# mapillary/OpenSfM

Hardware: NVIDIA H100
Metric: BA observations/sec (higher is better)
Workload: dtype f64

## Files before the change

### include/opensfm_b200.h

```cpp
#ifndef OPENSFM_B200_H_
#define OPENSFM_B200_H_

#include <stddef.h>
#include <stdint.h>

#ifdef __cplusplus
extern "C" {
#endif

#define OSFM_OK 0
#define OSFM_ERR_CUDA 1
#define OSFM_ERR_ARG 2
#define OSFM_ERR_RUNTIME 3

const char* osfm_last_error(void);
int osfm_version(void);
int64_t osfm_kernel_launch_count(void);

typedef struct osfm_matcher osfm_matcher;

int osfm_matcher_create(int device, osfm_matcher** out);
int osfm_matcher_destroy(osfm_matcher* m);

int osfm_bf_match_f32(osfm_matcher* m, const float* f1, int n1, const float* f2, int n2, int dim,
// ... 42 lines not shown

enum {
  OSFM_PERSPECTIVE = 0, OSFM_BROWN = 1, OSFM_FISHEYE = 2, OSFM_FISHEYE_OPENCV = 3, OSFM_FISHEYE62 = 4,
  OSFM_FISHEYE624 = 5, OSFM_SPHERICAL = 6, OSFM_DUAL = 7, OSFM_RADIAL = 8, OSFM_SIMPLE_RADIAL = 9
};
enum { OSFM_LOSS_TRIVIAL = 0, OSFM_LOSS_HUBER = 1, OSFM_LOSS_SOFTLONE = 2, OSFM_LOSS_CAUCHY = 3, OSFM_LOSS_ARCTAN = 4,
       OSFM_LOSS_TUKEY = 5  };

int osfm_ba_create(int device, osfm_ba** out);
int osfm_ba_destroy(osfm_ba* ba);
int osfm_camera_num_params(int projection_type);

int osfm_ba_set_cameras(osfm_ba* ba, int n, const int32_t* type, const double* params ,
                        const int32_t* constant, const double* prior , const double* prior_sigma ,
                        const int32_t* prior_log );
int osfm_ba_set_rig_instances(osfm_ba* ba, int n, const double* pose6, const int32_t* constant,
                              const int32_t* has_position_prior, const double* prior_position3,
                              const double* prior_std3);
int osfm_ba_set_rig_cameras(osfm_ba* ba, int n, const double* pose6, const int32_t* constant);
int osfm_ba_set_shots(osfm_ba* ba, int n, const int32_t* rig_instance, const int32_t* camera,
                      const int32_t* rig_camera, const int32_t* use_rig_camera);
int osfm_ba_set_points(osfm_ba* ba, int n, const double* xyz, const int32_t* constant);
int osfm_ba_set_observations(osfm_ba* ba, int64_t n, const int32_t* shot, const int32_t* point,
                             const double* xy, const double* std_deviation);
int osfm_ba_set_observations_async(osfm_ba* ba, int64_t n, const int32_t* shot, const int32_t* point,
                                   const double* xy, const double* std_deviation);

int osfm_ba_set_rig_camera_priors(osfm_ba* ba, const double* prior6, const double* sigma6);
int osfm_ba_set_point_priors(osfm_ba* ba, int n, const int32_t* point, const double* prior3, const double* sigma3,
                             const int32_t* has_altitude);
int osfm_ba_set_ext_blocks(osfm_ba* ba, int n, const int32_t* size, const double* values, const int32_t* constant,
                           const double* lower_bound);
int osfm_ba_get_ext_blocks(osfm_ba* ba, double* values);

enum {
  OSFM_SIDE_UP_VECTOR = 0, OSFM_SIDE_PAN = 1, OSFM_SIDE_TILT = 2, OSFM_SIDE_ROLL = 3, OSFM_SIDE_RELATIVE_MOTION = 4,
  OSFM_SIDE_RELATIVE_ROTATION = 5, OSFM_SIDE_COMMON_POSITION = 6, OSFM_SIDE_LINEAR_MOTION = 7,
  OSFM_SIDE_TRANSLATION_PRIOR = 8, OSFM_SIDE_PARAMETER_BARRIER = 9, OSFM_SIDE_STD_DEVIATION = 10,
  OSFM_SIDE_POSITION_PRIOR = 11,
  OSFM_SIDE_RA_RELATIVE_MOTION = 12, OSFM_SIDE_RA_ABSOLUTE_POSITION = 13, OSFM_SIDE_RA_RELATIVE_ABSOLUTE_POSITION = 14,
  OSFM_SIDE_RA_COMMON_POINT = 15, OSFM_SIDE_RA_COMMON_CAMERA = 16, OSFM_SIDE_NUM_TYPES = 17
};
typedef struct {
  int32_t type, nres, nblocks;
  int32_t kind[6], idx[6];
  int32_t loss;
  double loss_a;
  int32_t cofs;
  int32_t aux[4];
} osfm_side_term;
int osfm_ba_set_side_terms(osfm_ba* ba, int n, const osfm_side_term* terms, int64_t nconsts, const double* consts);
int osfm_ba_set_options(osfm_ba* ba, int loss, double loss_threshold, int max_iterations,
                        const char* linear_solver, int compute_reprojection_errors);
typedef int (*osfm_allreduce_fn)(void* device_buf, int64_t count, void* stream, void* user);
int osfm_ba_set_distributed(osfm_ba* ba, int rank, int world, osfm_allreduce_fn fn, void* user);
int osfm_nccl_unique_id(char* out128);
int osfm_ba_set_nccl(osfm_ba* ba, int rank, int world, const char* id128);
int osfm_ba_set_stream(osfm_ba* ba, void* cuda_stream);

int osfm_ba_run(osfm_ba* ba);

typedef struct {
  int iterations;
  int successful_steps;
  int linear_solves;
  int pcg_iterations;
  int termination;
  double initial_cost, final_cost;
  double time_run_s;
  double time_device_ms;
  double time_linearize_ms;
  int64_t linearize_launches;
  double time_schur_ms;
  int64_t schur_launches;
  double time_pcg_ms;
  double time_backsub_ms;
  int64_t num_observations_local;
  int reduced_dim;
  int reduced_blocks;
  int64_t reduced_nnz;
  int jac_planes;
  int64_t kernel_launches;
  char message[128];
} osfm_ba_summary;
int osfm_ba_get_summary(osfm_ba* ba, osfm_ba_summary* out);

int osfm_ba_get_cameras(osfm_ba* ba, double* params_flat);
int osfm_ba_get_rig_instances(osfm_ba* ba, double* pose6);
int osfm_ba_get_rig_cameras(osfm_ba* ba, double* pose6);
int osfm_ba_get_points(osfm_ba* ba, double* xyz);
int osfm_ba_get_reprojection_errors(osfm_ba* ba, double* out_n_by_3);

int osfm_ba_eval_observation(int device, int projection_type, const double* camera, const double* rig_instance,
                             const double* rig_camera, int use_rig_camera, const double* point,
                             const double* observed, double std_deviation, double* r, double* jac_camera,
                             double* jac_instance, double* jac_rig_camera, double* jac_point, int* num_residuals);

int osfm_ba_capture_linear_system(osfm_ba* ba, int iteration);
enum { OSFM_SCHUR_NONE = 0, OSFM_SCHUR_PIPE = 1, OSFM_SCHUR_MMA = 2, OSFM_SCHUR_SIMT_SEGMENT = 3 };
enum { OSFM_PCG_PIPELINED_DEFLATED = 1, OSFM_PCG_PIPELINED = 2, OSFM_PCG_CLASSIC_RESIDENT = 3,
       OSFM_PCG_CLASSIC_STREAMED = 4 };
typedef struct {
  int iteration;
  int nc, n, wc, nres;
  double radius;
  int nseg, p_fast, p_slow;
  int schur_kernel;
  int sp_nchunks;
  int pcg_kernel;
  int pcg_rescued;
  int pcg_iterations;
  double pcg_rr;
} osfm_ba_capture;
int osfm_ba_get_captured_system(osfm_ba* ba, osfm_ba_capture* info, double* S, double* rhs, double* y, double* scale,
                                double* diag, double* grad);
int osfm_ba_get_captured_parameters(osfm_ba* ba, double* cam_params, double* inst_pose6, double* rig_camera_pose6,
                                    double* points, double* ext_values);

int osfm_ba_set_compute_covariances(osfm_ba* ba, int enable);
enum {
  OSFM_COV_OK = 0,
  OSFM_COV_SOLVER_FAILURE = 1,
  OSFM_COV_POINT_RANK_DEFICIENT = 2,
  OSFM_COV_CAMERA_RANK_DEFICIENT = 3,
  OSFM_COV_NON_FINITE = 4
};
int osfm_ba_get_covariances(osfm_ba* ba, int* valid, int* status, double* out);
int osfm_ba_get_covariance_timing(osfm_ba* ba, double* pass_ms, double* cholesky_ms);

#ifdef __cplusplus
}
#endif
#endif
```

### opensfm_b200/_lib.py

```python
from __future__ import annotations

import ctypes
import os
from ctypes import POINTER, c_char_p, c_double, c_float, c_int, c_int32, c_int64, c_uint8, c_void_p

HERE = os.path.dirname(os.path.abspath(__file__))
LIB_PATH = os.path.join(HERE, "lib", "libopensfm_b200.so")

OSFM_OK = 0
PROJECTION_TYPES = dict(PERSPECTIVE=0, BROWN=1, FISHEYE=2, FISHEYE_OPENCV=3, FISHEYE62=4, FISHEYE624=5,
                        SPHERICAL=6, DUAL=7, RADIAL=8, SIMPLE_RADIAL=9)
LOSS_IDS = {"TrivialLoss": 0, "HuberLoss": 1, "SoftLOneLoss": 2, "CauchyLoss": 3, "ArctanLoss": 4}
LOSS_TUKEY = 5
SIDE_TYPES = dict(UP_VECTOR=0, PAN=1, TILT=2, ROLL=3, RELATIVE_MOTION=4, RELATIVE_ROTATION=5, COMMON_POSITION=6,
                  LINEAR_MOTION=7, TRANSLATION_PRIOR=8, PARAMETER_BARRIER=9, STD_DEVIATION=10, POSITION_PRIOR=11)
SB_CAM, SB_INST, SB_RIGCAM, SB_EXT = 0, 1, 2, 3


class SideTerm(ctypes.Structure):
    _fields_ = [("type", c_int32), ("nres", c_int32), ("nblocks", c_int32), ("kind", c_int32 * 6), ("idx", c_int32 * 6),
                ("loss", c_int32), ("loss_a", c_double), ("cofs", c_int32), ("aux", c_int32 * 4)]


class BASummary(ctypes.Structure):
    _fields_ = [
        ("iterations", c_int), ("successful_steps", c_int), ("linear_solves", c_int), ("pcg_iterations", c_int),
        ("termination", c_int), ("initial_cost", c_double), ("final_cost", c_double), ("time_run_s", c_double),
        ("time_device_ms", c_double), ("time_linearize_ms", c_double), ("linearize_launches", c_int64),
        ("time_schur_ms", c_double), ("schur_launches", c_int64), ("time_pcg_ms", c_double),
        ("time_backsub_ms", c_double), ("num_observations_local", c_int64), ("reduced_dim", c_int),
        ("reduced_blocks", c_int), ("reduced_nnz", c_int64), ("jac_planes", c_int), ("kernel_launches", c_int64), ("message", ctypes.c_char * 128),
    ]


class BACapture(ctypes.Structure):
    _fields_ = [("iteration", c_int), ("nc", c_int), ("n", c_int), ("wc", c_int), ("nres", c_int), ("radius", c_double),
                ("nseg", c_int), ("p_fast", c_int), ("p_slow", c_int), ("schur_kernel", c_int), ("sp_nchunks", c_int),
                ("pcg_kernel", c_int), ("pcg_rescued", c_int), ("pcg_iterations", c_int), ("pcg_rr", c_double)]


SCHUR_KERNELS = {0: "none", 1: "pipe", 2: "mma", 3: "simt_segment"}
PCG_KERNELS = {1: "pipelined_deflated", 2: "pipelined", 3: "classic_resident", 4: "classic_streamed"}
COVARIANCE_STATUS = {0: "ok", 1: "solver_failure", 2: "point_rank_deficient", 3: "camera_rank_deficient",
                     4: "non_finite"}

ALLREDUCE_FN = ctypes.CFUNCTYPE(c_int, c_void_p, c_int64, c_void_p, c_void_p)

SIGNATURES = {
    "osfm_last_error": (c_char_p, []),
    "osfm_version": (c_int, []),
    "osfm_kernel_launch_count": (c_int64, []),
    "osfm_matcher_create": (c_int, [c_int, POINTER(c_void_p)]),
    "osfm_matcher_destroy": (c_int, [c_void_p]),
    "osfm_bf_match_f32": (c_int, [c_void_p, c_void_p, c_int, c_void_p, c_int, c_int, c_double, c_void_p, c_int, c_void_p]),
    "osfm_bf_match_u8": (c_int, [c_void_p, c_void_p, c_int, c_void_p, c_int, c_int, c_double, c_void_p, c_int, c_void_p]),
    "osfm_matcher_add_f32": (c_int, [c_void_p, c_void_p, c_int, c_int, POINTER(c_int)]),
    "osfm_matcher_add_u8": (c_int, [c_void_p, c_void_p, c_int, c_int, POINTER(c_int)]),
    "osfm_matcher_add_batch_f32": (c_int, [c_void_p, c_int, c_void_p, c_void_p, c_int, c_void_p]),
    "osfm_matcher_add_batch_u8": (c_int, [c_void_p, c_int, c_void_p, c_void_p, c_int, c_void_p]),
    "osfm_matcher_add_u8_l2": (c_int, [c_void_p, c_void_p, c_int, c_int, POINTER(c_int)]),
    "osfm_matcher_add_batch_u8_l2": (c_int, [c_void_p, c_int, c_void_p, c_void_p, c_int, c_void_p]),
    "osfm_matcher_remove": (c_int, [c_void_p, c_int]),
    "osfm_matcher_clear": (c_int, [c_void_p]),
    "osfm_matcher_match_pairs_async": (c_int, [c_void_p, c_int, c_void_p, c_void_p, c_double, c_int]),
    "osfm_matcher_set_bearings": (c_int, [c_void_p, c_int, c_void_p]),
    "osfm_matcher_match_pairs_guided_async": (c_int, [c_void_p, c_int, c_void_p, c_void_p, c_void_p, c_double, c_double,
                                                       c_int]),
    "osfm_matcher_get_epipolar_masks": (c_int, [c_void_p, c_int, c_void_p, c_void_p]),
    "osfm_matcher_sync": (c_int, [c_void_p]),
    "osfm_matcher_fetch": (c_int, [c_void_p, c_void_p, c_int64]),
    "osfm_matcher_fetch_pairs": (c_int, [c_void_p, c_void_p, c_void_p, c_int64, POINTER(c_int64)]),
    "osfm_matcher_last_device_ms": (c_int, [c_void_p, POINTER(c_float), POINTER(c_float)]),
    "osfm_matcher_set_kernel": (c_int, [c_void_p, c_int]),
    "osfm_matcher_last_kernel": (c_int, [c_void_p]),
    "osfm_matcher_device_bytes": (c_int, [c_void_p, POINTER(c_int64), POINTER(c_int64)]),
    "osfm_match_words": (c_int, [c_void_p, c_void_p, c_int, c_void_p, c_int, c_void_p, c_int, c_void_p, c_int, c_float,
                                  c_int, c_void_p]),
    "osfm_vlad_distances": (c_int, [c_void_p, c_void_p, c_int, c_int, c_int, c_void_p]),
    "osfm_matcher_vlad_compute": (c_int, [c_void_p, c_int, c_void_p, c_void_p, c_int, c_int, c_void_p]),
    "osfm_matcher_vlad_get": (c_int, [c_void_p, c_int, c_int, c_void_p]),
    "osfm_matcher_vlad_select": (c_int, [c_void_p, c_int, c_void_p, c_int, c_void_p, c_void_p, c_void_p, c_int, c_void_p,
                                         c_void_p, c_void_p]),
    "osfm_ba_create": (c_int, [c_int, POINTER(c_void_p)]),
    "osfm_ba_destroy": (c_int, [c_void_p]),
    "osfm_camera_num_params": (c_int, [c_int]),
    "osfm_ba_set_cameras": (c_int, [c_void_p, c_int, c_void_p, c_void_p, c_void_p, c_void_p, c_void_p, c_void_p]),
    "osfm_ba_set_rig_instances": (c_int, [c_void_p, c_int, c_void_p, c_void_p, c_void_p, c_void_p, c_void_p]),
    "osfm_ba_set_rig_cameras": (c_int, [c_void_p, c_int, c_void_p, c_void_p]),
    "osfm_ba_set_shots": (c_int, [c_void_p, c_int, c_void_p, c_void_p, c_void_p, c_void_p]),
    "osfm_ba_set_points": (c_int, [c_void_p, c_int, c_void_p, c_void_p]),
    "osfm_ba_set_observations": (c_int, [c_void_p, c_int64, c_void_p, c_void_p, c_void_p, c_void_p]),
    "osfm_ba_set_observations_async": (c_int, [c_void_p, c_int64, c_void_p, c_void_p, c_void_p, c_void_p]),
    "osfm_ba_set_rig_camera_priors": (c_int, [c_void_p, c_void_p, c_void_p]),
    "osfm_ba_set_point_priors": (c_int, [c_void_p, c_int, c_void_p, c_void_p, c_void_p, c_void_p]),
    "osfm_ba_set_ext_blocks": (c_int, [c_void_p, c_int, c_void_p, c_void_p, c_void_p, c_void_p]),
    "osfm_ba_get_ext_blocks": (c_int, [c_void_p, c_void_p]),
    "osfm_ba_set_side_terms": (c_int, [c_void_p, c_int, c_void_p, c_int64, c_void_p]),
    "osfm_ba_set_options": (c_int, [c_void_p, c_int, c_double, c_int, c_char_p, c_int]),
    "osfm_ba_set_distributed": (c_int, [c_void_p, c_int, c_int, ALLREDUCE_FN, c_void_p]),
    "osfm_nccl_unique_id": (c_int, [c_void_p]),
    "osfm_ba_set_nccl": (c_int, [c_void_p, c_int, c_int, c_void_p]),
    "osfm_ba_set_stream": (c_int, [c_void_p, c_void_p]),
    "osfm_ba_run": (c_int, [c_void_p]),
    "osfm_ba_get_summary": (c_int, [c_void_p, POINTER(BASummary)]),
    "osfm_ba_get_cameras": (c_int, [c_void_p, c_void_p]),
    "osfm_ba_get_rig_instances": (c_int, [c_void_p, c_void_p]),
    "osfm_ba_get_rig_cameras": (c_int, [c_void_p, c_void_p]),
    "osfm_ba_get_points": (c_int, [c_void_p, c_void_p]),
    "osfm_ba_get_reprojection_errors": (c_int, [c_void_p, c_void_p]),
    "osfm_ba_eval_observation": (c_int, [c_int, c_int, c_void_p, c_void_p, c_void_p, c_int, c_void_p, c_void_p,
                                         c_double, c_void_p, c_void_p, c_void_p, c_void_p, c_void_p, POINTER(c_int)]),
    "osfm_ba_capture_linear_system": (c_int, [c_void_p, c_int]),
    "osfm_ba_get_captured_system": (c_int, [c_void_p, POINTER(BACapture), c_void_p, c_void_p, c_void_p, c_void_p,
                                            c_void_p, c_void_p]),
# ... 32 lines not shown
```

### opensfm_b200/csrc/ba.cu

```cuda
#include <algorithm>
#include <dlfcn.h>

#include <chrono>
#include <cstring>
#include <mutex>
#include <cmath>
#include <cstdlib>
#include <string>
#include <vector>

#include "ba_models.cuh"
#include "common.cuh"

struct OsfmNcclId { char internal[128]; };

namespace osfm {

struct BAView {
  int K, NI, NR, S, P;
  long long N;
  int nc, npf;
  int wc, nres;
  int loss;
  double loss_a;
  const int *cam_type, *cam_off, *cam_np, *cam_poff, *inst_poff, *rc_poff, *pt_poff;
  const int *shot_inst, *shot_cam, *shot_rc, *shot_use_rc;
  const int *obs_shot, *obs_point;
  const double *obs_x, *obs_y, *obs_isig;
  const long long* obs_orig;
  const long long* pt_start;
  double *r, *Jc, *Jp;
};

struct Params {
  double *cam, *inst, *rc, *pts, *ext;
};

struct Scalars {
  double cost;
  double model_change;
  double step_norm2;
  double x_norm2;
  double grad_max_bits;
  double gdot;
};

__device__ __forceinline__ double block_reduce_sum(double v) {
  __shared__ double sh[32];
  const int lane = threadIdx.x & 31, w = threadIdx.x >> 5;
#pragma unroll
  for (int o = 16; o; o >>= 1) v += __shfl_xor_sync(0xffffffffu, v, o);
  __syncthreads();
  if (lane == 0) sh[w] = v;
  __syncthreads();
  const int nw = (blockDim.x + 31) >> 5;
  v = threadIdx.x < nw ? sh[threadIdx.x] : 0.0;
  if (w == 0) {
#pragma unroll
    for (int o = 16; o; o >>= 1) v += __shfl_xor_sync(0xffffffffu, v, o);
  }
  return v;
}

__device__ __forceinline__ void atomic_max_nonneg(double* addr, double v) {
  atomicMax(reinterpret_cast<unsigned long long*>(addr), (unsigned long long)__double_as_longlong(v));
}

template <int MODE, int NB = 3, int TYPE = -1>
__global__ void __launch_bounds__(128, NB) ba_linearize(BAView v, Params p, Scalars* sc, double* reproj) {
  const long long i = (long long)blockIdx.x * blockDim.x + threadIdx.x;
  double cost = 0.0;
  if (i < v.N) {
    const int shot = v.obs_shot[i];
    const int cam = v.shot_cam[shot];
    const int type = TYPE >= 0 ? TYPE : v.cam_type[cam];
    const int C = TYPE >= 0 ? model_num_params(TYPE >= 0 ? TYPE : 0) : v.cam_np[cam];
    const bool use_rc = TYPE >= 0 ? false : v.shot_use_rc[shot] != 0;
    const int pt = v.obs_point[i];
    double camp[MAX_CAM_PARAMS], ri[6], rc[6], X[3];
#pragma unroll
    for (int j = 0; j < MAX_CAM_PARAMS; ++j)
      if (j < C) camp[j] = p.cam[v.cam_off[cam] + j];
#pragma unroll
    for (int j = 0; j < 6; ++j) ri[j] = p.inst[6 * (size_t)v.shot_inst[shot] + j];
    if (use_rc) {
#pragma unroll
      for (int j = 0; j < 6; ++j) rc[j] = p.rc[6 * (size_t)v.shot_rc[shot] + j];
    }
#pragma unroll
    for (int j = 0; j < 3; ++j) X[j] = p.pts[3 * (size_t)pt + j];
    const double ox = v.obs_x[i], oy = v.obs_y[i];
    if (MODE == 2) {
      double r[3] = {0.0, 0.0, 0.0};
      observation_eval(type, camp, ri, rc, use_rc, X, ox, oy, 1.0, r, nullptr, nullptr, nullptr, nullptr);
      const long long o = v.obs_orig[i];
      reproj[3 * o] = r[0]; reproj[3 * o + 1] = r[1]; reproj[3 * o + 2] = r[2];
    } else if (MODE == 0) {
      double r[3];
      const int nres = observation_eval(type, camp, ri, rc, use_rc, X, ox, oy, v.obs_isig[i], r, nullptr, nullptr,
                                        nullptr, nullptr);
      double s = r[0] * r[0] + r[1] * r[1];
      if (nres == 3) s += r[2] * r[2];
      double w;
      cost = 0.5 * robust_loss(v.loss, v.loss_a, s, &w);
      if (v.cam_poff[cam] < 0 && v.inst_poff[v.shot_inst[shot]] < 0 && (!use_rc || v.rc_poff[v.shot_rc[shot]] < 0) &&
          v.pt_poff[pt] < 0)
        cost = 0.0;
    } else {
      double r[3], jc[3 * MAX_CAM_PARAMS], jri[18], jrc[18], jp[9];
      const int nres = observation_eval(type, camp, ri, rc, use_rc, X, ox, oy, v.obs_isig[i], r, jc, jri, jrc, jp);
      double s = r[0] * r[0] + r[1] * r[1];
      if (nres == 3) s += r[2] * r[2];
      double w;
      cost = 0.5 * robust_loss(v.loss, v.loss_a, s, &w);
      const bool pfree = v.pt_poff[pt] >= 0;
      if (!pfree && v.cam_poff[cam] < 0 && v.inst_poff[v.shot_inst[shot]] < 0 && (!use_rc || v.rc_poff[v.shot_rc[shot]] < 0))
        cost = 0.0;
      const size_t N = (size_t)v.N;
      if (TYPE >= 0) {
        constexpr int CC = TYPE == PT_PERSPECTIVE ? 3 : TYPE == PT_FISHEYE ? 3 : TYPE == PT_BROWN ? 9 : 1;
        const int wcl = v.wc;
#pragma unroll
        for (int k = 0; k < 2; ++k) {
          v.r[k * N + i] = w * r[k];
          double* jcrow = v.Jc + (size_t)k * wcl * N + i;
#pragma unroll
          for (int j = 0; j < CC; ++j) jcrow[(size_t)j * N] = w * jc[k * CC + j];
#pragma unroll
// ... 187 lines not shown
    if (pf >= 0) {
#pragma unroll
      for (int j = 0; j < 3; ++j) {
        atomicAdd(&colnorm2[v.nc + 3 * pf + j], val[j]);
        atomicAdd(&grad[v.nc + 3 * pf + j], val[3 + j]);
      }
    }
  }
}

template <int WCT>
__global__ void __launch_bounds__(256, WCT ? 3 : 2) ba_colnorm_grad_seg(BAView v, const int* __restrict__ seg_start, int nseg,
                                                           double* colnorm2, double* grad) {
  const int s = blockIdx.x * (blockDim.x >> 5) + (threadIdx.x >> 5);
  if (s >= nseg) return;
  const int lane = threadIdx.x & 31;
  const int p0 = seg_start[s], np = seg_start[s + 1] - p0;
  const long long base = v.pt_start[p0];
  const int k = (int)(v.pt_start[p0 + 1] - base);
  const int G = 32 / k;
  const int g = lane / k, c = lane - g * k;
  const bool active = g < G;
  const size_t N = (size_t)v.N;
  const int wc = WCT ? WCT : v.wc;
  constexpr int WCU = WCT ? WCT : 16;
  double n2[WCU], gr[WCU];
#pragma unroll
  for (int j = 0; j < WCU; ++j) { n2[j] = 0.0; gr[j] = 0.0; }
  if (active) {
    for (int pi = g; pi < np; pi += G) {
      const size_t i = (size_t)(base + (long long)pi * k + c);
      for (int q = 0; q < v.nres; ++q) {
        const double rq = v.r[q * N + i];
#pragma unroll
        for (int j = 0; j < WCU; ++j) {
          if (j < wc) {
            const double a = v.Jc[((size_t)q * wc + j) * N + i];
            n2[j] += a * a;
            gr[j] += a * rq;
          }
        }
      }
    }
  }
  for (int gg = 1; gg < G; ++gg) {
#pragma unroll
    for (int j = 0; j < WCU; ++j) {
      if (j < wc) {
        const double a = __shfl_down_sync(0xffffffffu, n2[j], gg * k);
        const double b = __shfl_down_sync(0xffffffffu, gr[j], gg * k);
        if (lane < k) { n2[j] += a; gr[j] += b; }
      }
    }
  }
  if (lane < k) {
    const ObsCols oc = obs_cols(v, base + c);
#pragma unroll
    for (int j = 0; j < WCU; ++j) {
      if (j < wc) {
        const int col = oc.col(j);
        if (col >= 0) {
          atomicAdd(&colnorm2[col], n2[j]);
          atomicAdd(&grad[col], gr[j]);
        }
      }
    }
  }
}

__global__ void ba_prior_colnorm_grad(PriorView pv, Params p, double* colnorm2, double* grad) {
  const int row = blockIdx.x * blockDim.x + threadIdx.x;
  if (row >= pv.n_cam_rows + pv.n_pos_rows) return;
  double r, d;
  int col;
  prior_row(pv, p, row, &r, &col, &d);
  atomicAdd(&colnorm2[col], d * d);
  atomicAdd(&grad[col], d * r);
}

__global__ void ba_make_scale(const double* colnorm2, double* scale, int n) {
  const int i = blockIdx.x * blockDim.x + threadIdx.x;
  if (i < n) scale[i] = 1.0 / (1.0 + sqrt(colnorm2[i]));
}
__global__ void ba_make_diag(const double* colnorm2, const double* scale, double* diag, int n) {
  const int i = blockIdx.x * blockDim.x + threadIdx.x;
  if (i < n) diag[i] = fmin(fmax(colnorm2[i] * scale[i] * scale[i], 1e-6), 1e32);
}
__global__ void ba_pack_lin(const double* __restrict__ colnorm2, const double* __restrict__ grad, const Scalars* sc, int nc,
                            int rank, int world, double* __restrict__ pack) {
  const int i = blockIdx.x * blockDim.x + threadIdx.x;
  if (i < nc) { pack[i] = colnorm2[i]; pack[nc + i] = grad[i]; }
  if (i == 0) pack[2 * nc] = sc->cost;
  if (i < world) pack[2 * nc + 1 + i] = i == rank ? sc->grad_max_bits : 0.0;
}
__global__ void ba_unpack_lin(const double* __restrict__ pack, int nc, int world, double* __restrict__ colnorm2,
                              double* __restrict__ grad, Scalars* sc) {
  const int i = blockIdx.x * blockDim.x + threadIdx.x;
  double v = 0.0;
  if (i < nc) { colnorm2[i] = pack[i]; grad[i] = pack[nc + i]; v = fabs(pack[nc + i]); }
  if (i < world) v = fmax(v, pack[2 * nc + 1 + i]);
  if (i == 0) sc->cost = pack[2 * nc];
#pragma unroll
  for (int o = 16; o; o >>= 1) v = fmax(v, __shfl_xor_sync(0xffffffffu, v, o));
  if ((threadIdx.x & 31) == 0 && v > 0.0) atomic_max_nonneg(&sc->grad_max_bits, v);
}
__global__ void ba_grad_max(const double* grad, int n, Scalars* sc) {
  const int i = blockIdx.x * blockDim.x + threadIdx.x;
  double v = i < n ? fabs(grad[i]) : 0.0;
#pragma unroll
  for (int o = 16; o; o >>= 1) v = fmax(v, __shfl_xor_sync(0xffffffffu, v, o));
  if ((threadIdx.x & 31) == 0 && v > 0.0) atomic_max_nonneg(&sc->grad_max_bits, v);
}

}
#include "ba_reduced.cuh"
#include "ba_schur_pipe.cuh"

#include <tuple>
#include <utility>

namespace osfm {
template <typename... KArgs, size_t... I>
inline void launch_cooperative_impl(void (*kern)(KArgs...), int grid, int block, size_t smem, cudaStream_t st,
                                    std::tuple<KArgs...>& a, std::index_sequence<I...>) {
  void* ptrs[] = {static_cast<void*>(&std::get<I>(a))...};
  OSFM_CUDA(cudaLaunchCooperativeKernel(reinterpret_cast<const void*>(kern), dim3(grid), dim3(block), ptrs, smem, st));
}
template <typename... KArgs, typename... Args>
inline void launch_cooperative(void (*kern)(KArgs...), int grid, int block, size_t smem, cudaStream_t st, Args&&... args) {
  std::tuple<KArgs...> a(std::forward<Args>(args)...);
  launch_cooperative_impl(kern, grid, block, smem, st, a, std::index_sequence_for<KArgs...>{});
}
}
#include "ba_side.cuh"
#include "ba_order.cuh"
#include "ba_cov.cuh"
namespace osfm {

__global__ void __launch_bounds__(256) ba_backsub_rows(BAView v, const double* __restrict__ scale,
                                                       const double* __restrict__ y, double* __restrict__ t) {
  const long long i = (long long)blockIdx.x * blockDim.x + threadIdx.x;
  const size_t N = (size_t)v.N;
  const bool in = i < v.N;
  const int pt = in ? v.obs_point[i] : -1;
  const int pf = in ? v.pt_poff[pt] : -1;
  double val[3] = {0.0, 0.0, 0.0};
  if (pf >= 0) {
    const int wc = v.wc;
    const ObsCols oc = obs_cols(v, i);
    for (int q = 0; q < v.nres; ++q) {
      double e = v.r[q * N + i];
      for (int j = 0; j < wc; ++j) {
        const int g = oc.col(j);
        if (g >= 0) e -= v.Jc[((size_t)q * wc + j) * N + i] * scale[g] * y[g];
      }
#pragma unroll
      for (int j = 0; j < 3; ++j) val[j] += v.Jp[((size_t)q * 3 + j) * N + i] * e;
    }
  }
  seg_scan_by_point<3>(pt, val);
  const int next = __shfl_down_sync(0xffffffffu, pt, 1);
  const bool tail = (threadIdx.x & 31) == 31 || next != pt;
  if (pf >= 0 && tail) {
    const size_t NP = (size_t)v.npf;
#pragma unroll
    for (int j = 0; j < 3; ++j) atomicAdd(&t[j * NP + pf], val[j]);
  }
}
__global__ void __launch_bounds__(256) ba_backsub_points(BAView v, const double* __restrict__ scale,
                                                         const double* __restrict__ Vinv, const double* __restrict__ t,
                                                         double* __restrict__ y) {
  const int pf = blockIdx.x * blockDim.x + threadIdx.x;
  if (pf >= v.npf) return;
  const size_t NP = (size_t)v.npf;
  const int nc = v.nc;
  const double t0 = t[pf] * scale[nc + 3 * pf], t1 = t[NP + pf] * scale[nc + 3 * pf + 1],
               t2 = t[2 * NP + pf] * scale[nc + 3 * pf + 2];
  const double a = Vinv[0 * NP + pf], b = Vinv[1 * NP + pf], c = Vinv[2 * NP + pf];
  const double d = Vinv[3 * NP + pf], e = Vinv[4 * NP + pf], f = Vinv[5 * NP + pf];
  y[nc + 3 * pf + 0] = a * t0 + b * t1 + c * t2;
  y[nc + 3 * pf + 1] = b * t0 + d * t1 + e * t2;
  y[nc + 3 * pf + 2] = c * t0 + e * t1 + f * t2;
}

__global__ void ba_update(int which, int count, const int* __restrict__ poff, const int* __restrict__ off,
                          const int* __restrict__ np, int stride, int base, const double* __restrict__ src,
                          double* __restrict__ dst, const double* __restrict__ scale, const double* __restrict__ y,
                          Scalars* sc, int accumulate_norms, const double* __restrict__ lower = nullptr,
                          double alpha = 1.0) {
  const int b = blockIdx.x * blockDim.x + threadIdx.x;
  double sn = 0.0, xn = 0.0;
  if (b < count) {
    const int o = which == 0 ? off[b] : b * stride;
    const int n = which == 0 ? np[b] : stride;
    const int g = poff[b];
    for (int j = 0; j < n; ++j) {
      double val = src[o + j];
      if (g >= 0) {
        const int gi = which == 3 ? base + 3 * g + j : g + j;
        double d = -alpha * scale[gi] * y[gi];
        if (lower && val + d < lower[o + j]) d = lower[o + j] - val;
        xn += val * val;
        sn += d * d;
        val += d;
      }
      dst[o + j] = val;
    }
  }
  if (accumulate_norms) {
    const double t1 = block_reduce_sum(sn);
    const double t2 = block_reduce_sum(xn);
    if (threadIdx.x == 0) {
      if (t1 != 0.0) atomicAdd(&sc->step_norm2, t1);
      if (t2 != 0.0) atomicAdd(&sc->x_norm2, t2);
    }
  }
}

__global__ void ba_grad_dot(int n, int nc, int cam_side, const double* __restrict__ grad, const double* __restrict__ scale,
                            const double* __restrict__ y, Scalars* sc) {
  const int i = blockIdx.x * blockDim.x + threadIdx.x;
  double v = 0.0;
  if (i < n && (i >= nc || cam_side)) v = -grad[i] * scale[i] * y[i];
  const double t = block_reduce_sum(v);
  if (threadIdx.x == 0 && t != 0.0) atomicAdd(&sc->gdot, t);
}

__global__ void ba_model_change_alg(int n, int nc, int cam_side, const double* __restrict__ grad, const double* __restrict__ scale,
                                    const double* __restrict__ diag, double inv_radius, const double* __restrict__ y, Scalars* sc) {
  const int i = blockIdx.x * blockDim.x + threadIdx.x;
  double v = 0.0;
  if (i < n && (i >= nc || cam_side)) v = 0.5 * y[i] * (grad[i] * scale[i] + diag[i] * inv_radius * y[i]);
  const double t = block_reduce_sum(v);
  if (threadIdx.x == 0 && t != 0.0) atomicAdd(&sc->model_change, t);
}

__global__ void ba_eval_one(int type, const double* in, int use_rc, double* out, int* nres_out) {
  double r[3] = {0, 0, 0}, jc[3 * MAX_CAM_PARAMS], jri[18], jrc[18], jp[9];
  for (int i = 0; i < 18; ++i) jrc[i] = 0.0;
  const int nres = observation_eval(type, in, in + 16, in + 22, use_rc != 0, in + 28, in[31], in[32], in[33], r, jc,
                                    jri, jrc, jp);
  *nres_out = nres;
  for (int i = 0; i < 3; ++i) out[i] = r[i];
  for (int i = 0; i < 48; ++i) out[3 + i] = jc[i];
  for (int i = 0; i < 18; ++i) out[51 + i] = jri[i];
  for (int i = 0; i < 18; ++i) out[69 + i] = jrc[i];
  for (int i = 0; i < 9; ++i) out[87 + i] = jp[i];
}

struct EventTimer {
  cudaEvent_t a = nullptr, b = nullptr;
  double total_ms = 0.0;
  long long count = 0;
  bool pending = false;
  void init() { OSFM_CUDA(cudaEventCreate(&a)); OSFM_CUDA(cudaEventCreate(&b)); }
  void destroy() { if (a) cudaEventDestroy(a); if (b) cudaEventDestroy(b); a = b = nullptr; }
  void start(cudaStream_t st) { collect(); OSFM_CUDA(cudaEventRecord(a, st)); }
  void stop(cudaStream_t st) { OSFM_CUDA(cudaEventRecord(b, st)); pending = true; }
  void collect() {
    if (!pending) return;
    OSFM_CUDA(cudaEventSynchronize(b));
    float ms = 0.f;
    OSFM_CUDA(cudaEventElapsedTime(&ms, a, b));
    total_ms += ms; ++count; pending = false;
  }
};

template <class T>
static void upload(DevBuf<T>& d, const std::vector<T>& h, cudaStream_t st) {
  d.reserve(std::max<size_t>(h.size(), 1));
  if (!h.empty()) OSFM_CUDA(cudaMemcpyAsync(d.p, h.data(), h.size() * sizeof(T), cudaMemcpyHostToDevice, st));
}
template <class T>
static void download(std::vector<T>& h, const T* d, size_t count, cudaStream_t st) {
  h.resize(count);
  if (count) OSFM_CUDA(cudaMemcpyAsync(h.data(), d, count * sizeof(T), cudaMemcpyDeviceToHost, st));
}

struct NcclApi {
  void* lib = nullptr;
  int (*GetUniqueId)(void*) = nullptr;
  int (*CommInitRank)(void**, int, OsfmNcclId, int) = nullptr;
  int (*AllReduce)(const void*, void*, size_t, int, int, void*, cudaStream_t) = nullptr;
  int (*CommDestroy)(void*) = nullptr;
  const char* (*GetErrorString)(int) = nullptr;
};
static NcclApi& nccl_api() {
  static NcclApi api;
  static std::once_flag once;
  std::call_once(once, []() {
    void* h = dlopen("libnccl.so.2", RTLD_NOW | RTLD_NOLOAD);
    if (!h) h = dlopen("libnccl.so.2", RTLD_NOW);
    if (!h) h = dlopen("libnccl.so", RTLD_NOW);
    if (!h) return;
    api.lib = h;
    api.GetUniqueId = reinterpret_cast<int (*)(void*)>(dlsym(h, "ncclGetUniqueId"));
    api.CommInitRank = reinterpret_cast<int (*)(void**, int, OsfmNcclId, int)>(dlsym(h, "ncclCommInitRank"));
    api.AllReduce = reinterpret_cast<int (*)(const void*, void*, size_t, int, int, void*, cudaStream_t)>(dlsym(h, "ncclAllReduce"));
    api.CommDestroy = reinterpret_cast<int (*)(void*)>(dlsym(h, "ncclCommDestroy"));
    api.GetErrorString = reinterpret_cast<const char* (*)(int)>(dlsym(h, "ncclGetErrorString"));
  });
  if (!api.lib || !api.GetUniqueId || !api.CommInitRank || !api.AllReduce || !api.CommDestroy)
    throw std::runtime_error("NCCL (libnccl.so.2) is not available in this process");
  return api;
}
static void nccl_check(int rc, const char* what) {
  if (rc != 0) {
    NcclApi& a = nccl_api();
    throw std::runtime_error(std::string(what) + ": " + (a.GetErrorString ? a.GetErrorString(rc) : "NCCL error"));
  }
}

static int grid_for(long long n, int threads) { return (int)std::max<long long>(1, (n + threads - 1) / threads); }
static long long up16(long long x) { return (x + 15) / 16 * 16; }
static std::vector<int> balanced_cut(const std::vector<long long>& w, int G) {
  const int n = (int)w.size() - 1;
  std::vector<int> lo(G + 1, n);
  lo[0] = 0;
  for (int c = 1, i = 0; c < G; ++c) {
    const long long want = w[n] * c / G;
    while (i < n && w[i] < want) ++i;
    lo[c] = i;
  }
  return lo;
}
static bool env_starts_with(const char* name, char c) {
  const char* e = getenv(name);
  return e && e[0] == c;
}
struct BaSwitches {
  bool trace = env_starts_with("OSFM_BA_TRACE", '1');
  bool seg_schur = !env_starts_with("OSFM_BA_SEGMENT_SCHUR", '0');
  bool lin_special = !env_starts_with("OSFM_BA_LIN_SPECIAL", '0');
  bool schur_mma = !env_starts_with("OSFM_BA_SCHUR_MMA", '0');
  bool schur_pipe = !env_starts_with("OSFM_BA_SCHUR_PIPE", '0');
  bool pcg_resident = !env_starts_with("OSFM_BA_PCG_RESIDENT", '0');
  bool pcg_pipelined = !env_starts_with("OSFM_BA_PCG_PIPELINED", '0');
  bool pcg_deflate = !env_starts_with("OSFM_BA_PCG_DEFLATE", '0');
};
static const BaSwitches& switches() {
  static const BaSwitches s;
  return s;
}

enum LinPath {
  LIN_NONE,
  LIN_FUSED,
  LIN_CHUNKS,
  LIN_SEGMENTS,
};

struct RunState {
  std::chrono::high_resolution_clock::time_point t_start, t_prev;
  int64_t launches0 = 0;
  int K = 0, NI = 0, NR = 0, NE = 0, NT = 0, S = 0, P = 0, Pfull = 0;
  long long Nfull = 0, N = 0, n_fast_obs = 0, pair_bound = 0;
  int nc = 0, nc_pad = 0, n = 0, nblk = 0, npf = 0, ngroups = 0, wc = 0, nres = 2, nseg = 0, P_fast = 0;
  size_t nz = 1;
  int n_upper = 0, n_blocks_all = 0, pcg_grid = 1;
  long long s_upper_total = 0, s_total = 0, vb = 0;
  int uniform_type = -1;
  bool constrained = false;
  bool have_pp = false, add_priors = false;
  int cur = 0;
  int pcg_total = 0;
  std::vector<int> cam_off, cam_np, cam_poff, inst_poff, rc_poff, ext_off, ext_poff, blk_off, blk_sz;
  std::vector<int> cam_blk, inst_blk, rc_blk, ext_blk, side_jofs, side_rofs, grp_b1, grp_b2;
  std::vector<int> pr_cam_param, pr_cam_col, pr_cam_log, pr_pos_kind, pr_pos_inst, pr_pos_axis, pr_pos_col;
  std::vector<int> pr_blk, pr_local;
  std::vector<double> pr_cam_prior, pr_cam_scale, pr_pos_prior, pr_pos_scale;
  std::vector<int> row_M, cbase;
  std::vector<long long> rowbase;
  std::vector<int> cov_inst, cov_bstart;
  int cov_m = 0, cov_nb1 = 0;
  int schur = OSFM_SCHUR_NONE;
  LinPath lin = LIN_NONE;
  bool seg_tab = false;
  int sp_nchunks = 0;
  bool pcg_resident = false, pcg_pipe_ok = false;
  int pcg_smem = 0, pcg_pipe_smem = 0;
  PcgResident pcg_res{};
  PcgPipe pcg_pipe{};
  BAView v{}; PriorView pv{}; SideView sv{}; PointPriorView ppv{}; BlkMaps bm{}; BsrView bsr{}; PcgLayout lay{};
  double *d_rhs_p = nullptr, *d_S_p = nullptr;
  cudaEvent_t ev0 = nullptr, ev1 = nullptr;
  EventTimer tm_lin, tm_schur, tm_pcg, tm_back;
};

struct BA {
  int device = 0;
  cudaStream_t own_stream = nullptr, stream = nullptr;
  cudaStream_t copy_stream = nullptr;
  cudaEvent_t ev_obs = nullptr;
  bool obs_pending = false;
  std::vector<int> cam_type, cam_const, cam_prior_log;
  std::vector<double> cam_params, cam_prior, cam_prior_sigma;
  std::vector<double> inst, inst_prior_pos, inst_prior_std;
  std::vector<int> inst_const, inst_has_prior;
  std::vector<double> rc, rc_prior, rc_prior_sigma;
  std::vector<int> rc_const;
  std::vector<int> ext_size, ext_const;
  std::vector<double> ext_values, ext_lower;
  std::vector<osfm_side_term> side_terms;
  std::vector<double> side_consts;
  std::vector<int> pp_point, pp_alt;
  std::vector<double> pp_prior, pp_sigma;
  std::vector<int> shot_inst, shot_cam, shot_rc, shot_use_rc;
  std::vector<double> pts;
  std::vector<int> pt_const;
  long long n_obs_full = 0;
  int loss = OSFM_LOSS_CAUCHY;
  double loss_a = 1.0;
  int max_iterations = 500;
  bool compute_reproj = true;
  int rank = 0, world = 1;
  osfm_allreduce_fn allreduce = nullptr;
  void* allreduce_user = nullptr;
  void* nccl_comm = nullptr;
  int nccl_rank = -1, nccl_world = 0;
  bool reproj_valid = false;
  osfm_ba_summary summary{};
  bool has_run = false;
  int cap_iter = 0;
  bool cap_valid = false;
  osfm_ba_capture cap_info{};
  std::vector<double> cap_sbuf, cap_y, cap_scale, cap_diag, cap_grad;
  std::vector<double> cap_cam, cap_inst, cap_rc, cap_pts, cap_ext;
  std::vector<int4> cap_upper;
  std::vector<int> cap_blk_off, cap_blk_sz, cap_pt_poff, cap_global_of;
  int cap_nc_pad = 0;
  bool cov_on = false, cov_ran = false, cov_valid = false;
  int cov_status = OSFM_COV_OK;
  double cov_pass_ms = 0.0, cov_chol_ms = 0.0;
  std::vector<double> cov_out;
  DevBuf<double> d_cov;
  DevBuf<int> d_cov_perm, d_cov_inst, d_cov_flags;

  DevBuf<int> d_cam_type, d_cam_off, d_cam_np, d_cam_poff, d_inst_poff, d_rc_poff, d_pt_poff;
  DevBuf<int> d_shot_inst, d_shot_cam, d_shot_rc, d_shot_use_rc, d_obs_shot, d_obs_point;
  DevBuf<double> d_obs_x, d_obs_y, d_obs_isig;
  DevBuf<long long> d_obs_orig, d_pt_start;
  DevBuf<double> d_cam[2], d_inst[2], d_rc[2], d_pts[2];
  DevBuf<double> d_r, d_Jc, d_Jp, d_Sbuf, d_Vinv, d_gp, d_slots;
  DevBuf<double> d_scale, d_colnorm2, d_grad, d_diag, d_y, d_bs_t;
  DevBuf<double> d_px, d_pr, d_pz, d_pp, d_pAp, d_Minv, d_reproj, d_full_pts;
  DevBuf<double> d_Wdef;
  DevBuf<int> d_blk_off, d_blk_sz, d_cam_blk, d_inst_blk, d_rc_blk;
  DevBuf<unsigned long long> d_tkeys, d_skeys, d_skeys2, d_rkeys, d_rkeys2;
  DevBuf<int> d_tvals, d_area, d_offs, d_row_ptr, d_row_col, d_row_off, d_diag_off, d_prior_diag_off;
  DevBuf<int> d_pr_blk, d_pr_local, d_g_obs_shot, d_g_obs_point;
  DevBuf<long long> d_g_pt_start;
  DevBuf<int4> d_upper;
  DevBuf<unsigned> d_count;
  DevBuf<char> d_cub;
  DevBuf<PcgState> d_pcg;
  DevBuf<int> d_seg_start;
  DevBuf<int> d_raw_shot, d_raw_point, d_ptc_full;
  DevBuf<double> d_raw_xy, d_raw_sigma, d_pts_in;
  DevBuf<unsigned long long> d_okeys, d_okeys2, d_pkey, d_pkey2;
  DevBuf<int> d_ovals, d_ovals2, d_pval, d_order, d_inv_order, d_global_of, d_free_flag, d_free_scan, d_head, d_run_head, d_nsel;
  DevBuf<long long> d_kk;
  DevBuf<char> d_seg_flags;
  DevBuf<OrderCounts> d_oc;
  PinnedBuf<OrderCounts> h_oc;
  DevBuf<double> d_rowsJ, d_rowsW, d_rowsY, d_Vig;
  DevBuf<int> d_row_M, d_qoff, d_blk_row, d_cbase, d_colidx, d_row_of, d_grp_b1, d_grp_b2;
  DevBuf<long long> d_rowbase;
  DevBuf<double> d_Spcg, d_Ap;
  PinnedBuf<PcgState> h_pcg;
  DevBuf<int> d_pcg_rowlo;
  DevBuf<int> d_pcg_grplo;
  DevBuf<char> d_grp_shared;
  DevBuf<unsigned long long> d_prof;
  DevBuf<long long> d_tab_off, d_tab_sizes;
  DevBuf<int> d_sp_nch, d_sp_chunk0;
  DevBuf<SchurChunk> d_sp_chunks;
  DevBuf<int> d_sp_ftab;
  DevBuf<int> d_tab;
  DevBuf<double> d_ptsum;
  std::vector<const void*> smem_opted;
  int num_sms = 132;
  DevBuf<int> d_pr_cam_param, d_pr_cam_col, d_pr_cam_log, d_pr_pos_inst, d_pr_pos_axis, d_pr_pos_col;
  DevBuf<double> d_pr_cam_prior, d_pr_cam_scale, d_pr_pos_prior, d_pr_pos_scale;
  DevBuf<Scalars> d_sc;
  PinnedBuf<Scalars> h_sc;
  DevBuf<int> d_pr_pos_kind, d_ext_off, d_ext_np, d_ext_poff, d_ext_blk, d_side_jofs, d_side_rofs;
  DevBuf<double> d_ext[2], d_ext_lower, d_side_consts, d_side_J, d_side_r, d_pp_d, d_pp_x0;
  DevBuf<SideTerm> d_side_terms;

  explicit BA(int dev) : device(dev) {
    OSFM_CUDA(cudaSetDevice(device));
    OSFM_CUDA(cudaStreamCreateWithFlags(&own_stream, cudaStreamNonBlocking));
    stream = own_stream;
    OSFM_CUDA(cudaStreamCreateWithFlags(&copy_stream, cudaStreamNonBlocking));
    OSFM_CUDA(cudaEventCreateWithFlags(&ev_obs, cudaEventDisableTiming));
    h_sc.reserve(1);
    h_pcg.reserve(1);
    OSFM_CUDA(cudaDeviceGetAttribute(&num_sms, cudaDevAttrMultiProcessorCount, device));
  }
  ~BA() {
    cudaSetDevice(device);
    if (nccl_comm) { try { nccl_api().CommDestroy(nccl_comm); } catch (...) {} }
    if (copy_stream) { cudaStreamSynchronize(copy_stream); cudaStreamDestroy(copy_stream); }
    if (ev_obs) cudaEventDestroy(ev_obs);
    if (own_stream) cudaStreamDestroy(own_stream);
  }

  Scalars read_scalars() {
    OSFM_CUDA(cudaMemcpyAsync(h_sc.p, d_sc.p, sizeof(Scalars), cudaMemcpyDeviceToHost, stream));
    OSFM_CUDA(cudaStreamSynchronize(stream));
    return *h_sc.p;
  }
  int ar_calls = 0;
  double ar_host_ms = 0.0, ar_dev_ms = 0.0;
  void allreduce_dev(double* buf, long long count) {
    if (world > 1) {
      const auto t0 = std::chrono::high_resolution_clock::now();
      cudaEvent_t e0 = nullptr, e1 = nullptr;
      if (switches().trace) { cudaEventCreate(&e0); cudaEventCreate(&e1); cudaEventRecord(e0, stream); }
      struct Done {
        BA* self; std::chrono::high_resolution_clock::time_point t0; cudaEvent_t e0, e1;
        ~Done() {
          if (switches().trace) {
            cudaEventRecord(e1, self->stream); cudaEventSynchronize(e1);
            float ms = 0.f; cudaEventElapsedTime(&ms, e0, e1); self->ar_dev_ms += ms;
            cudaEventDestroy(e0); cudaEventDestroy(e1);
          }
          ++self->ar_calls;
          self->ar_host_ms += std::chrono::duration<double, std::milli>(std::chrono::high_resolution_clock::now() - t0).count();
        }
      } done{this, t0, e0, e1};
      if (allreduce) {
        if (allreduce(buf, count, stream, allreduce_user) != 0) throw std::runtime_error("all-reduce callback failed");
      } else if (nccl_comm && nccl_world == world && nccl_rank == rank) {
        nccl_check(nccl_api().AllReduce(buf, buf, (size_t)count,  8,  0, nccl_comm, stream), "ncclAllReduce");
      } else {
        throw ArgError("world > 1 but neither an all-reduce callback nor an NCCL communicator is set");
      }
    }
  }
  template <class Kernel>
  void opt_in_smem(Kernel* kernel, int bytes) {
    const void* k = (const void*)kernel;
    if (std::find(smem_opted.begin(), smem_opted.end(), k) != smem_opted.end()) return;
    OSFM_CUDA(cudaFuncSetAttribute(k, cudaFuncAttributeMaxDynamicSharedMemorySize, bytes));
    smem_opted.push_back(k);
  }
  void trace(const char* what) {
    if (!switches().trace) return;
    const auto now = std::chrono::high_resolution_clock::now();
    fprintf(stderr, "[osfm_ba] %-12s %8.3f ms\n", what, std::chrono::duration<double, std::milli>(now - rs.t_prev).count());
    rs.t_prev = now;
  }
  template <int MODE>
  void launch_linearize(int b) {
    const int grid = grid_for(rs.N, 128);
    switch (rs.uniform_type) {
      case PT_PERSPECTIVE: ba_linearize<MODE, MODE == 1 ? 5 : 3, PT_PERSPECTIVE><<<grid, 128, 0, stream>>>(rs.v, params_of(b), d_sc.p, nullptr); break;
      case PT_BROWN: ba_linearize<MODE, MODE == 1 ? 4 : 3, PT_BROWN><<<grid, 128, 0, stream>>>(rs.v, params_of(b), d_sc.p, nullptr); break;
      case PT_FISHEYE: ba_linearize<MODE, MODE == 1 ? 5 : 3, PT_FISHEYE><<<grid, 128, 0, stream>>>(rs.v, params_of(b), d_sc.p, nullptr); break;
      default: ba_linearize<MODE, 3><<<grid, 128, 0, stream>>>(rs.v, params_of(b), d_sc.p, nullptr); break;
    }
    OSFM_LAUNCH_CHECK();
  }
  void update_params(int src, int dst, double alpha, const double* lower) {
    const Params a = params_of(src), b = params_of(dst);
    const int K = rs.K, NI = rs.NI, NR = rs.NR, P = rs.P, NE = rs.NE;
    if (K) { ba_update<<<grid_for(K, 128), 128, 0, stream>>>(0, K, d_cam_poff.p, d_cam_off.p, d_cam_np.p, 0, 0, a.cam, b.cam, d_scale.p, d_y.p, d_sc.p, rank == 0, nullptr, alpha); OSFM_LAUNCH_CHECK(); }
    if (NI) { ba_update<<<grid_for(NI, 128), 128, 0, stream>>>(1, NI, d_inst_poff.p, nullptr, nullptr, 6, 0, a.inst, b.inst, d_scale.p, d_y.p, d_sc.p, rank == 0, nullptr, alpha); OSFM_LAUNCH_CHECK(); }
    if (NR) { ba_update<<<grid_for(NR, 128), 128, 0, stream>>>(2, NR, d_rc_poff.p, nullptr, nullptr, 6, 0, a.rc, b.rc, d_scale.p, d_y.p, d_sc.p, rank == 0, nullptr, alpha); OSFM_LAUNCH_CHECK(); }
    if (P) { ba_update<<<grid_for(P, 128), 128, 0, stream>>>(3, P, d_pt_poff.p, nullptr, nullptr, 3, rs.nc, a.pts, b.pts, d_scale.p, d_y.p, d_sc.p, 1, nullptr, alpha); OSFM_LAUNCH_CHECK(); }
    if (NE) { ba_update<<<grid_for(NE, 128), 128, 0, stream>>>(0, NE, d_ext_poff.p, d_ext_off.p, d_ext_np.p, 0, 0, a.ext, b.ext, d_scale.p, d_y.p, d_sc.p, rank == 0, lower, alpha); OSFM_LAUNCH_CHECK(); }
  }
  double x_norm_of(int b) {
    OSFM_CUDA(cudaMemsetAsync(&d_sc.p->x_norm2, 0, sizeof(double), stream));
    OSFM_CUDA(cudaMemsetAsync(d_y.p, 0, sizeof(double) * rs.nz, stream));
    update_params(b, b, 1.0, nullptr);
    allreduce_dev(&d_sc.p->x_norm2, 1);
    return std::sqrt(read_scalars().x_norm2);
  }
  Params params_of(int b) { return Params{d_cam[b].p, d_inst[b].p, d_rc[b].p, d_pts[b].p, d_ext[b].p}; }
  RunState rs;

  void run();
  void plan_layout(), order_observations(), plan_prior_rows(), upload_problem(), discover_structure(), plan_pcg(),
      reserve_covariance(), build_segment_tables(), segment_table_scales();
  double eval_cost(int b), linearize(int b, bool timed, double* grad_max);
  void build_system(double inv_radius, int* rank_flag, bool timed), back_substitute();
  int solve_reduced();
  void capture_linear_system(int it, double radius, int pcg_path), covariance_pass(int termination);
  void write_results(osfm_ba_summary sum);
};

void BA::plan_layout() {
  const int K = (int)cam_type.size(), NI = (int)inst_const.size(), NR = (int)rc_const.size(), S = (int)shot_inst.size();
  const int NE = (int)ext_size.size(), NT = (int)side_terms.size();
  rs.K = K; rs.NI = NI; rs.NR = NR; rs.NE = NE; rs.NT = NT; rs.S = S; rs.Pfull = (int)pt_const.size(); rs.Nfull = n_obs_full;
  for (int s = 0; s < S; ++s) {
    if (shot_inst[s] < 0 || shot_inst[s] >= NI) throw ArgError("shot references a rig instance that doesn't exist");
    if (shot_cam[s] < 0 || shot_cam[s] >= K) throw ArgError("shot references a camera that doesn't exist");
    if (shot_use_rc[s] && (shot_rc[s] < 0 || shot_rc[s] >= NR))
      throw ArgError("shot references a rig camera that doesn't exist");
  }
  trace("validate");

  rs.cam_off.assign(K + 1, 0); rs.cam_np.assign(K, 0); rs.cam_poff.assign(K, -1); rs.inst_poff.assign(NI, -1);
  rs.rc_poff.assign(std::max(NR, 1), -1); rs.ext_off.assign(NE + 1, 0); rs.ext_poff.assign(std::max(NE, 1), -1);
  rs.cam_blk.assign(std::max(K, 1), -1); rs.inst_blk.assign(std::max(NI, 1), -1); rs.rc_blk.assign(std::max(NR, 1), -1);
  rs.ext_blk.assign(std::max(NE, 1), -1);
  int nc = 0;
  auto add_block = [&](int size, int& poff, int& blk) {
    poff = nc; blk = (int)rs.blk_off.size();
    rs.blk_off.push_back(nc); rs.blk_sz.push_back(size); nc += size;
  };
  for (int k = 0; k < K; ++k) {
    rs.cam_np[k] = model_num_params(cam_type[k]);
    rs.cam_off[k + 1] = rs.cam_off[k] + rs.cam_np[k];
  }
  for (int k = 0; k < K; ++k) if (!cam_const[k]) add_block(rs.cam_np[k], rs.cam_poff[k], rs.cam_blk[k]);
  for (int i = 0; i < NI; ++i) if (!inst_const[i]) add_block(6, rs.inst_poff[i], rs.inst_blk[i]);
  for (int i = 0; i < NR; ++i) if (!rc_const[i]) add_block(6, rs.rc_poff[i], rs.rc_blk[i]);
  for (int i = 0; i < NE; ++i) {
    if (ext_size[i] < 1 || ext_size[i] > MAXB) throw ArgError("ext block size must be in [1, 16]");
    rs.ext_off[i + 1] = rs.ext_off[i] + ext_size[i];
    if (ext_const[i]) continue;
    add_block(ext_size[i], rs.ext_poff[i], rs.ext_blk[i]);
    for (int j = 0; j < ext_size[i]; ++j) rs.constrained |= std::isfinite(ext_lower[rs.ext_off[i] + j]);
  }
  rs.nc = nc;
  rs.nblk = (int)rs.blk_off.size();
  rs.nc_pad = (nc + 15) / 16 * 16;
  rs.side_jofs.assign(NT + 1, 0); rs.side_rofs.assign(NT + 1, 0);
  for (int t = 0; t < NT; ++t) {
    const osfm_side_term& st = side_terms[t];
    if (st.type < 0 || st.type >= OSFM_SIDE_NUM_TYPES) throw ArgError("unknown side term type");
    if (st.nblocks < 1 || st.nblocks > SIDE_MAX_BLOCKS || st.nres < 1 || st.nres > SIDE_MAX_RES)
      throw ArgError("side term with a bad block / residual count");
    int np = 0;
    for (int b = 0; b < st.nblocks; ++b) {
      const int kd = st.kind[b], ix = st.idx[b];
      const int cnt = kd == SB_CAM ? K : kd == SB_INST ? NI : kd == SB_RIGCAM ? NR : kd == SB_EXT ? NE : -1;
      if (ix < 0 || ix >= cnt) throw ArgError("side term references a parameter block that doesn't exist");
      np += kd == SB_CAM ? model_num_params(cam_type[ix]) : kd == SB_EXT ? ext_size[ix] : 6;
    }
    if (np > SIDE_MAX_PARAMS) throw ArgError("side term with too many parameters");
    if (st.cofs < 0 || (size_t)st.cofs > side_consts.size()) throw ArgError("side term constants out of range");
    rs.side_jofs[t + 1] = rs.side_jofs[t] + st.nres * np;
    rs.side_rofs[t + 1] = rs.side_rofs[t] + st.nres;
  }

  {
    std::vector<int> cam_user(std::max(K, 1), -1), inst_cam(std::max(NI, 1), -1);
    for (int s2 = 0; s2 < S; ++s2) {
      const int k = shot_cam[s2], i = shot_inst[s2];
      cam_user[k] = cam_user[k] == -1 || cam_user[k] == i ? i : -2;
      inst_cam[i] = inst_cam[i] == -1 || inst_cam[i] == k ? k : -2;
    }
    std::vector<char> inst_done(std::max(NI, 1), 0);
    for (int k = 0; k < K; ++k) {
      if (rs.cam_blk[k] < 0) continue;
      const int i = cam_user[k];
      if (i >= 0 && rs.inst_blk[i] >= 0 && inst_cam[i] == k && rs.cam_np[k] + 6 <= 16) {
        rs.grp_b1.push_back(rs.cam_blk[k]); rs.grp_b2.push_back(rs.inst_blk[i]); inst_done[i] = 1;
      } else {
        rs.grp_b1.push_back(rs.cam_blk[k]); rs.grp_b2.push_back(-1);
      }
    }
    for (int i = 0; i < NI; ++i)
      if (rs.inst_blk[i] >= 0 && !inst_done[i]) { rs.grp_b1.push_back(rs.inst_blk[i]); rs.grp_b2.push_back(-1); }
    for (int i = 0; i < NR; ++i)
      if (rs.rc_blk[i] >= 0) { rs.grp_b1.push_back(rs.rc_blk[i]); rs.grp_b2.push_back(-1); }
    for (int i = 0; i < NE; ++i)
      if (rs.ext_blk[i] >= 0) { rs.grp_b1.push_back(rs.ext_blk[i]); rs.grp_b2.push_back(-1); }
// ... 121 lines not shown
  rs.nseg = h_oc.p->nseg; rs.P_fast = h_oc.p->p_fast;
  rs.n_fast_obs = h_oc.p->n_fast; rs.pair_bound = (long long)h_oc.p->pair_bound;
  if (switches().trace)
    fprintf(stderr, "[osfm_ba] points %d (fast path %d in %d segments), observations %lld (fast path %lld), free points %d\n", P,
            rs.P_fast, rs.nseg, N, rs.n_fast_obs, rs.npf);
}

void BA::plan_prior_rows() {
  for (int k = 0; k < rs.K; ++k) {
    if (rs.cam_poff[k] < 0) continue;
    for (int j = 0; j < rs.cam_np[k]; ++j) {
      const int idx = rs.cam_off[k] + j;
      rs.pr_cam_param.push_back(idx);
      rs.pr_cam_col.push_back(rs.cam_poff[k] + j);
      rs.pr_cam_log.push_back(cam_prior_log[idx]);
      rs.pr_cam_prior.push_back(cam_prior[idx]);
      rs.pr_cam_scale.push_back(1.0 / std::max(cam_prior_sigma[idx], DBL_EPSILON));
      rs.pr_blk.push_back(rs.cam_blk[k]); rs.pr_local.push_back(j);
    }
  }
  auto pos_row = [&](int kind, int i, int axis, int poff, int blk, double prior, double sigma) {
    rs.pr_pos_kind.push_back(kind); rs.pr_pos_inst.push_back(i); rs.pr_pos_axis.push_back(axis); rs.pr_pos_col.push_back(poff + axis);
    rs.pr_pos_prior.push_back(prior);
    rs.pr_pos_scale.push_back(1.0 / std::max(sigma, DBL_EPSILON));
    rs.pr_blk.push_back(blk); rs.pr_local.push_back(axis);
  };
  for (int i = 0; i < rs.NI; ++i) {
    if (!inst_has_prior[i] || rs.inst_poff[i] < 0) continue;
    for (int j = 0; j < 3; ++j)
      pos_row(1, i, 3 + j, rs.inst_poff[i], rs.inst_blk[i], inst_prior_pos[3 * (size_t)i + j], inst_prior_std[3 * (size_t)i + j]);
  }
  for (int i = 0; i < rs.NR && !rc_prior.empty(); ++i) {
    if (rs.rc_poff[i] < 0) continue;
    for (int j = 0; j < 6; ++j)
      pos_row(2, i, j, rs.rc_poff[i], rs.rc_blk[i], rc_prior[6 * (size_t)i + j], rc_prior_sigma[6 * (size_t)i + j]);
  }
}

void BA::upload_problem() {
  const int NT = rs.NT, P = rs.P, Pfull = rs.Pfull, nc = rs.nc, npf = rs.npf, nres = rs.nres, wc = rs.wc;
  upload(d_cam_type, cam_type, stream); upload(d_cam_off, rs.cam_off, stream); upload(d_cam_np, rs.cam_np, stream);
  upload(d_cam_poff, rs.cam_poff, stream); upload(d_inst_poff, rs.inst_poff, stream); upload(d_rc_poff, rs.rc_poff, stream);
  upload(d_shot_inst, shot_inst, stream); upload(d_shot_cam, shot_cam, stream); upload(d_shot_rc, shot_rc, stream);
  upload(d_shot_use_rc, shot_use_rc, stream);
  std::vector<double> rc_h = rc;
  if (rc_h.empty()) rc_h.assign(6, 0.0);
  for (int b = 0; b < 2; ++b) {
    upload(d_cam[b], cam_params, stream); upload(d_inst[b], inst, stream); upload(d_rc[b], rc_h, stream);
  }
  upload(d_blk_off, rs.blk_off, stream); upload(d_blk_sz, rs.blk_sz, stream);
  upload(d_cam_blk, rs.cam_blk, stream); upload(d_inst_blk, rs.inst_blk, stream); upload(d_rc_blk, rs.rc_blk, stream);
  upload(d_pr_blk, rs.pr_blk, stream); upload(d_pr_local, rs.pr_local, stream);
  upload(d_grp_b1, rs.grp_b1, stream); upload(d_grp_b2, rs.grp_b2, stream);
  upload(d_pr_cam_param, rs.pr_cam_param, stream); upload(d_pr_cam_col, rs.pr_cam_col, stream);
  upload(d_pr_cam_log, rs.pr_cam_log, stream); upload(d_pr_cam_prior, rs.pr_cam_prior, stream);
  upload(d_pr_cam_scale, rs.pr_cam_scale, stream); upload(d_pr_pos_inst, rs.pr_pos_inst, stream);
  upload(d_pr_pos_axis, rs.pr_pos_axis, stream); upload(d_pr_pos_col, rs.pr_pos_col, stream);
  upload(d_pr_pos_kind, rs.pr_pos_kind, stream);
  std::vector<double> ev = ext_values, el = ext_lower;
  if (ev.empty()) { ev.assign(1, 0.0); el.assign(1, 0.0); }
  upload(d_ext[0], ev, stream); upload(d_ext[1], ev, stream); upload(d_ext_lower, el, stream);
  upload(d_ext_off, rs.ext_off, stream); upload(d_ext_np, ext_size, stream); upload(d_ext_poff, rs.ext_poff, stream);
  upload(d_ext_blk, rs.ext_blk, stream);
  upload(d_side_terms, side_terms, stream); upload(d_side_consts, side_consts, stream);
  upload(d_side_jofs, rs.side_jofs, stream); upload(d_side_rofs, rs.side_rofs, stream);
  d_side_J.reserve((size_t)rs.side_jofs[NT] + 1); d_side_r.reserve((size_t)rs.side_rofs[NT] + 1);
  std::vector<double> ppd, ppx;
  if (rs.have_pp) {
    ppd.assign(3 * (size_t)Pfull, 0.0); ppx.assign(3 * (size_t)Pfull, 0.0);
    for (size_t q = 0; q < pp_point.size(); ++q) {
      const size_t g = (size_t)pp_point[q];
      for (int j = 0; j < (pp_alt[q] ? 3 : 2); ++j) {
        ppd[3 * g + j] = 1.0 / std::max(pp_sigma[3 * q + j], DBL_EPSILON);
        ppx[3 * g + j] = pp_prior[3 * q + j];
      }
    }
    upload(d_pp_d, ppd, stream); upload(d_pp_x0, ppx, stream);
  }
  OSFM_CUDA(cudaStreamSynchronize(stream));
  upload(d_pr_pos_prior, rs.pr_pos_prior, stream); upload(d_pr_pos_scale, rs.pr_pos_scale, stream);
  const size_t Nz = (size_t)std::max<long long>(rs.N, 1);
  d_r.reserve(nres * Nz); d_Jc.reserve((size_t)nres * wc * Nz); d_Jp.reserve((size_t)nres * 3 * Nz);
  d_Vinv.reserve(6 * (size_t)std::max(npf, 1)); d_gp.reserve(3 * (size_t)std::max(npf, 1));
  const size_t nz = rs.nz;
  d_scale.reserve(nz); d_colnorm2.reserve(nz); d_grad.reserve(nz); d_diag.reserve(nz); d_y.reserve(nz);
  d_px.reserve(std::max(nc, 1)); d_pr.reserve(std::max(nc, 1)); d_pz.reserve(std::max(nc, 1));
  d_pp.reserve(std::max(nc, 1)); d_pAp.reserve(std::max(nc, 1));
  d_pcg.reserve(1);
  d_Minv.reserve((size_t)std::max(rs.ngroups, 1) * MAXB * MAXB);
  d_Ap.reserve(std::max(nc, 1));
  d_sc.reserve(1);

  BAView& v = rs.v;
  v.K = rs.K; v.NI = rs.NI; v.NR = rs.NR; v.S = rs.S; v.P = P; v.N = rs.N; v.nc = nc; v.npf = npf; v.wc = wc; v.nres = nres;
  v.loss = loss; v.loss_a = loss_a;
  v.cam_type = d_cam_type.p; v.cam_off = d_cam_off.p; v.cam_np = d_cam_np.p; v.cam_poff = d_cam_poff.p;
  v.inst_poff = d_inst_poff.p; v.rc_poff = d_rc_poff.p; v.pt_poff = d_pt_poff.p;
  v.shot_inst = d_shot_inst.p; v.shot_cam = d_shot_cam.p; v.shot_rc = d_shot_rc.p; v.shot_use_rc = d_shot_use_rc.p;
  v.obs_shot = d_obs_shot.p; v.obs_point = d_obs_point.p; v.obs_x = d_obs_x.p; v.obs_y = d_obs_y.p;
  v.obs_isig = d_obs_isig.p; v.obs_orig = d_obs_orig.p; v.pt_start = d_pt_start.p;
  v.r = d_r.p; v.Jc = d_Jc.p; v.Jp = d_Jp.p;
  PriorView& pv = rs.pv;
  pv.n_cam_rows = rs.add_priors ? (int)rs.pr_cam_param.size() : 0;
  pv.n_pos_rows = rs.add_priors ? (int)rs.pr_pos_inst.size() : 0;
  pv.cam_row_param = d_pr_cam_param.p; pv.cam_row_col = d_pr_cam_col.p; pv.cam_row_log = d_pr_cam_log.p;
  pv.cam_row_prior = d_pr_cam_prior.p; pv.cam_row_scale = d_pr_cam_scale.p;
  pv.pos_row_kind = d_pr_pos_kind.p;
  pv.pos_row_inst = d_pr_pos_inst.p; pv.pos_row_axis = d_pr_pos_axis.p; pv.pos_row_col = d_pr_pos_col.p;
  pv.pos_row_prior = d_pr_pos_prior.p; pv.pos_row_scale = d_pr_pos_scale.p;
  SideView& sv = rs.sv;
  sv.n = NT; sv.terms = d_side_terms.p; sv.consts = d_side_consts.p; sv.jofs = d_side_jofs.p; sv.rofs = d_side_rofs.p;
  sv.J = d_side_J.p; sv.r = d_side_r.p;
  sv.ext_off = d_ext_off.p; sv.ext_np = d_ext_np.p; sv.ext_poff = d_ext_poff.p; sv.ext_blk = d_ext_blk.p;
  rs.ppv = PointPriorView{rs.have_pp ? d_pp_d.p : nullptr, d_pp_x0.p, d_global_of.p};
  rs.bm = BlkMaps{d_cam_blk.p, d_inst_blk.p, d_rc_blk.p};
}

void BA::discover_structure() {
  const int nblk = rs.nblk, nc = rs.nc, NT = rs.NT;
  if (nblk > 0) {
    const int* g_shot = d_obs_shot.p;
    const int* g_point = d_obs_point.p;
    const long long* g_start = d_pt_start.p;
    if (world > 1) { g_shot = d_g_obs_shot.p; g_point = d_g_obs_point.p; g_start = d_g_pt_start.p; }
    const long long bound = std::min<long long>((long long)nblk * (nblk + 1) / 2, 9 * rs.pair_bound + nblk + 21LL * NT);
    unsigned tsize = 1024;
    while ((long long)tsize < 4 * bound) {
      if (tsize >= (1u << 28)) throw std::runtime_error("reduced camera system has too many block pairs");
      tsize <<= 1;
    }
    d_tkeys.reserve(tsize); d_tvals.reserve(tsize);
    OSFM_CUDA(cudaMemsetAsync(d_tkeys.p, 0xff, sizeof(unsigned long long) * tsize, stream));
    const long long n_enum = world > 1 ? rs.Nfull : rs.N;
    if (n_enum > 0) {
      bsr_enum_pairs<<<grid_for(n_enum, 128), 128, 0, stream>>>(rs.v, rs.bm, g_shot, g_start, g_point, n_enum, d_tkeys.p,
                                                              tsize - 1, nblk);
      OSFM_LAUNCH_CHECK();
    }
    if (NT > 0) {
      side_enum_pairs<<<grid_for(NT, 128), 128, 0, stream>>>(rs.sv, rs.v, rs.bm, params_of(0), d_tkeys.p, tsize - 1, nblk);
      OSFM_LAUNCH_CHECK();
    }
    bsr_insert_diagonal<<<grid_for(nblk, 128), 128, 0, stream>>>(d_tkeys.p, tsize - 1, nblk);
    OSFM_LAUNCH_CHECK();
    const size_t cap = (size_t)(2 * bound + 16);
    d_skeys.reserve(cap); d_skeys2.reserve(cap); d_rkeys.reserve(cap); d_rkeys2.reserve(cap);
    d_area.reserve(cap); d_offs.reserve(cap); d_count.reserve(4);
    OSFM_CUDA(cudaMemsetAsync(d_count.p, 0, sizeof(unsigned), stream));
    bsr_compact<<<grid_for(tsize, 256), 256, 0, stream>>>(d_tkeys.p, tsize, nblk, d_skeys.p, d_count.p);
    OSFM_LAUNCH_CHECK();
    unsigned n_all_u = 0;
    OSFM_CUDA(cudaMemcpyAsync(&n_all_u, d_count.p, sizeof(unsigned), cudaMemcpyDeviceToHost, stream));
    OSFM_CUDA(cudaStreamSynchronize(stream));
    const int n_all = (int)n_all_u;
    rs.n_blocks_all = n_all;
    const int n_upper = rs.n_upper = nblk + (n_all - nblk) / 2;
    size_t tmp1 = 0, tmp2 = 0;
    cub::DeviceRadixSort::SortKeys(nullptr, tmp1, d_skeys.p, d_skeys2.p, n_all, 0, 64, stream);
    cub::DeviceScan::ExclusiveSum(nullptr, tmp2, d_area.p, d_offs.p, n_all, stream);
    d_cub.reserve(std::max(tmp1, tmp2) + 256);
    size_t tmp = d_cub.cap;
    OSFM_CUDA(cub::DeviceRadixSort::SortKeys(d_cub.p, tmp, d_skeys.p, d_skeys2.p, n_all, 0, 64, stream));
    g_kernel_launches.fetch_add(1);
    bsr_block_areas<<<grid_for(n_all, 256), 256, 0, stream>>>(d_skeys2.p, n_all, nblk, d_blk_sz.p, d_area.p);
    OSFM_LAUNCH_CHECK();
    tmp = d_cub.cap;
    OSFM_CUDA(cub::DeviceScan::ExclusiveSum(d_cub.p, tmp, d_area.p, d_offs.p, n_all, stream));
    g_kernel_launches.fetch_add(1);
// ... 133 lines not shown
    OSFM_CUDA(cudaStreamSynchronize(stream));
  }
  PcgLayout& lay = rs.lay;
  lay.row_of = d_row_of.p; lay.row_M = d_row_M.p; lay.rowbase = d_rowbase.p; lay.cbase = d_cbase.p;
  lay.colidx = d_colidx.p; lay.ngroups = ngroups; lay.grp_b1 = d_grp_b1.p; lay.grp_b2 = d_grp_b2.p;
}

void BA::reserve_covariance() {
  const int nc = rs.nc;
  for (int i = 0; i < rs.NI; ++i)
    if (rs.inst_poff[i] >= 0) rs.cov_inst.push_back(i);
  rs.cov_m = 6 * (int)rs.cov_inst.size();
  for (int k = 0; k < nc - rs.cov_m; k += COV_NB) rs.cov_bstart.push_back(k);
  rs.cov_nb1 = (int)rs.cov_bstart.size();
  for (int k = nc - rs.cov_m; k < nc; k += COV_NB) rs.cov_bstart.push_back(k);
  const size_t nblocks = rs.cov_bstart.size();
  rs.cov_bstart.push_back(nc);
  const size_t total = (size_t)nc * nc + (size_t)rs.cov_m * rs.cov_m + nblocks * COV_NB * COV_NB + (size_t)nc +
                       (size_t)rs.NI * 36 + 1;
  if (total > d_cov.cap) {
    size_t free_b = 0, total_b = 0;
    OSFM_CUDA(cudaMemGetInfo(&free_b, &total_b));
    if (total * sizeof(double) > free_b + d_cov.cap * sizeof(double)) {
      char msg[256];
      snprintf(msg, sizeof(msg),
               "covariance estimation needs %zu bytes of device memory for the dense reduced camera system "
               "(n_c = %d) and its workspace; %zu bytes are free", total * sizeof(double), nc, free_b);
      throw ArgError(msg);
    }
    d_cov.release();
    OSFM_CUDA(cudaMalloc(&d_cov.p, total * sizeof(double)));
    d_cov.cap = total;
  }
  d_cov_flags.reserve(COV_F_COUNT);
}

void BA::build_segment_tables() {
  const int nseg = rs.nseg, wc = rs.wc;
  if (nseg > 0 && rs.nblk > 0 && wc <= 9) {
    d_tab_off.reserve((size_t)nseg + 1); d_tab_sizes.reserve((size_t)nseg + 1);
    ba_seg_table_sizes<<<grid_for(nseg + 1, 256), 256, 0, stream>>>(rs.v, d_seg_start.p, nseg, d_tab_sizes.p);
    OSFM_LAUNCH_CHECK();
    size_t tb = 0;
    cub::DeviceScan::ExclusiveSum(nullptr, tb, d_tab_sizes.p, d_tab_off.p, nseg + 1, stream);
    d_cub.reserve(tb + 256);
    tb = d_cub.cap;
    OSFM_CUDA(cub::DeviceScan::ExclusiveSum(d_cub.p, tb, d_tab_sizes.p, d_tab_off.p, nseg + 1, stream));
    long long total_ints = 0;
    OSFM_CUDA(cudaMemcpyAsync(&total_ints, d_tab_off.p + nseg, sizeof(long long), cudaMemcpyDeviceToHost, stream));
    OSFM_CUDA(cudaStreamSynchronize(stream));
    d_tab.reserve((size_t)total_ints + 2);
    ba_seg_tables<<<nseg, 128, 0, stream>>>(rs.v, rs.bm, rs.bsr, d_seg_start.p, nullptr, d_tab_off.p, d_tab.p);
    OSFM_LAUNCH_CHECK();
    rs.seg_tab = true;
  }
  if (rs.seg_tab && wc == 9 && rs.nres == 2) {
    d_sp_nch.reserve((size_t)nseg + 1); d_sp_chunk0.reserve((size_t)nseg + 1);
    sp_chunk_counts<<<grid_for(nseg + 1, 256), 256, 0, stream>>>(rs.v, d_seg_start.p, nseg, d_sp_nch.p);
    OSFM_LAUNCH_CHECK();
    size_t tb = 0;
    cub::DeviceScan::ExclusiveSum(nullptr, tb, d_sp_nch.p, d_sp_chunk0.p, nseg + 1, stream);
    d_cub.reserve(tb + 256);
    tb = d_cub.cap;
    OSFM_CUDA(cub::DeviceScan::ExclusiveSum(d_cub.p, tb, d_sp_nch.p, d_sp_chunk0.p, nseg + 1, stream));
    OSFM_CUDA(cudaMemcpyAsync(&rs.sp_nchunks, d_sp_chunk0.p + nseg, sizeof(int), cudaMemcpyDeviceToHost, stream));
    OSFM_CUDA(cudaStreamSynchronize(stream));
    d_sp_chunks.reserve((size_t)rs.sp_nchunks + 1);
    sp_fill_chunks<<<grid_for((long long)nseg * 32, 256), 256, 0, stream>>>(rs.v, d_seg_start.p, nseg, d_sp_chunk0.p,
                                                                          d_tab_off.p, d_sp_chunks.p);
    OSFM_LAUNCH_CHECK();
  }
  const bool use_mma = switches().schur_mma && wc <= 9;
  const bool use_pipe = use_mma && switches().schur_pipe && rs.sp_nchunks > 0 &&
                        rs.s_upper_total + (long long)rs.nc_pad < (1LL << 29) &&
                        (long long)nseg * SP_FT_SEG * (long long)sizeof(int) <= (8LL << 30);
  if (use_pipe) {
    d_sp_ftab.reserve((size_t)nseg * SP_FT_SEG);
    sp_flush_tables<<<nseg, SP_CONS_THREADS, 0, stream>>>(rs.v, d_seg_start.p, d_tab_off.p, d_tab.p, d_sp_ftab.p);
    OSFM_LAUNCH_CHECK();
  }
  rs.schur = nseg == 0 ? OSFM_SCHUR_NONE
             : !use_mma ? OSFM_SCHUR_SIMT_SEGMENT
             : use_pipe ? OSFM_SCHUR_PIPE : OSFM_SCHUR_MMA;
  rs.lin = nseg == 0 ? LIN_NONE
           : rs.sp_nchunks == 0 ? LIN_SEGMENTS
           : rs.uniform_type == PT_PERSPECTIVE ? LIN_FUSED : LIN_CHUNKS;
}

void BA::segment_table_scales() {
  if (!rs.seg_tab) return;
  ba_seg_scales<<<rs.nseg, 128, 0, stream>>>(rs.v, d_seg_start.p, d_scale.p, d_tab_off.p, d_tab.p);
  OSFM_LAUNCH_CHECK();
}

double BA::eval_cost(int b) {
  OSFM_CUDA(cudaMemsetAsync(&d_sc.p->cost, 0, sizeof(double), stream));
  if (rs.N > 0) launch_linearize<0>(b);
  const int npr_local = rs.pv.n_cam_rows + rs.pv.n_pos_rows;
  if (npr_local > 0) {
    ba_prior_cost<<<grid_for(npr_local, 128), 128, 0, stream>>>(rs.pv, params_of(b), d_sc.p);
    OSFM_LAUNCH_CHECK();
  }
  if (rs.NT > 0 && rs.add_priors) {
    side_cost<<<grid_for(rs.NT, 128), 128, 0, stream>>>(rs.sv, rs.v, rs.bm, params_of(b), d_sc.p);
    OSFM_LAUNCH_CHECK();
  }
  if (rs.have_pp && rs.P > 0) {
    ba_point_prior<0><<<grid_for(rs.P, 128), 128, 0, stream>>>(rs.ppv, rs.v, params_of(b), nullptr, nullptr, nullptr, d_sc.p);
    OSFM_LAUNCH_CHECK();
  }
  allreduce_dev(&d_sc.p->cost, 1);
  return read_scalars().cost;
}


double BA::linearize(int b, bool timed, double* grad_max) {
  const long long N = rs.N, n_fast_obs = rs.n_fast_obs;
  const int nc = rs.nc, n = rs.n, nseg = rs.nseg, wc = rs.wc, NT = rs.NT;
  OSFM_CUDA(cudaMemsetAsync(d_sc.p, 0, sizeof(Scalars), stream));
  OSFM_CUDA(cudaMemsetAsync(d_colnorm2.p, 0, sizeof(double) * rs.nz, stream));
  OSFM_CUDA(cudaMemsetAsync(d_grad.p, 0, sizeof(double) * rs.nz, stream));
  if (N > 0 && rs.lin == LIN_FUSED) {
    d_ptsum.reserve(9 * (size_t)std::max(rs.npf, 1));
    const int grid = (int)((n_fast_obs + FL_WIN - 1) / FL_WIN + (N - n_fast_obs + FL_THREADS - 1) / FL_THREADS);
    if (timed) rs.tm_lin.start(stream);
    ba_linearize_fused<PT_PERSPECTIVE><<<grid, FL_THREADS, 0, stream>>>(rs.v, params_of(b), d_sc.p, d_sp_chunks.p, rs.sp_nchunks,
                                                                        n_fast_obs, d_tab.p, d_colnorm2.p, d_grad.p, d_ptsum.p);
    OSFM_LAUNCH_CHECK();
    if (timed) rs.tm_lin.stop(stream);
    if (N > n_fast_obs) {
      ba_colnorm_grad_points<<<grid_for(N - n_fast_obs, 256), 256, 0, stream>>>(rs.v, n_fast_obs, d_colnorm2.p, d_grad.p);
      OSFM_LAUNCH_CHECK();
      ba_colnorm_grad<<<grid_for(N - n_fast_obs, 256), 256, 0, stream>>>(rs.v, n_fast_obs, d_colnorm2.p, d_grad.p);
      OSFM_LAUNCH_CHECK();
    }
  } else if (N > 0) {
    if (timed) rs.tm_lin.start(stream);
    launch_linearize<1>(b);
    if (timed) rs.tm_lin.stop(stream);
    ba_colnorm_grad_points<<<grid_for(N, 256), 256, 0, stream>>>(rs.v, 0, d_colnorm2.p, d_grad.p);
    OSFM_LAUNCH_CHECK();
    if (rs.lin == LIN_CHUNKS) {
      opt_in_smem(ba_colnorm_grad_chunks, CC_SMEM);
      const int grid = std::max(1, std::min(num_sms, (rs.sp_nchunks + CC_WARPS - 1) / CC_WARPS));
      ba_colnorm_grad_chunks<<<grid, 32 * CC_WARPS, CC_SMEM, stream>>>(rs.v, d_sp_chunks.p, rs.sp_nchunks, d_tab.p,
                                                                        d_colnorm2.p, d_grad.p);
      OSFM_LAUNCH_CHECK();
    } else if (rs.lin == LIN_SEGMENTS) {
      auto kern = wc == 9 ? ba_colnorm_grad_seg<9> : ba_colnorm_grad_seg<0>;
      kern<<<grid_for((long long)nseg * 32, 256), 256, 0, stream>>>(rs.v, d_seg_start.p, nseg, d_colnorm2.p, d_grad.p);
      OSFM_LAUNCH_CHECK();
    }
    if (N > n_fast_obs) {
      ba_colnorm_grad<<<grid_for(N - n_fast_obs, 256), 256, 0, stream>>>(rs.v, n_fast_obs, d_colnorm2.p, d_grad.p);
      OSFM_LAUNCH_CHECK();
    }
  }
  const int npr_local = rs.pv.n_cam_rows + rs.pv.n_pos_rows;
  if (npr_local > 0) {
    ba_prior_cost<<<grid_for(npr_local, 128), 128, 0, stream>>>(rs.pv, params_of(b), d_sc.p);
    OSFM_LAUNCH_CHECK();
    ba_prior_colnorm_grad<<<grid_for(npr_local, 128), 128, 0, stream>>>(rs.pv, params_of(b), d_colnorm2.p, d_grad.p);
    OSFM_LAUNCH_CHECK();
  }
  if (NT > 0) {
    side_linearize<<<NT, SIDE_THREADS, 0, stream>>>(rs.sv, rs.v, rs.bm, params_of(b), d_sc.p, rs.add_priors ? 1 : 0);
    OSFM_LAUNCH_CHECK();
    if (rs.add_priors) {
      side_colnorm_grad<<<NT, SIDE_THREADS, 0, stream>>>(rs.sv, rs.v, rs.bm, params_of(b), d_colnorm2.p, d_grad.p);
      OSFM_LAUNCH_CHECK();
    }
  }
  if (rs.have_pp && rs.P > 0) {
    ba_point_prior<1><<<grid_for(rs.P, 128), 128, 0, stream>>>(rs.ppv, rs.v, params_of(b), d_colnorm2.p, d_grad.p, nullptr, d_sc.p);
    OSFM_LAUNCH_CHECK();
  }
  if (world > 1) {
    if (n > nc) {
      ba_grad_max<<<grid_for(n - nc, 256), 256, 0, stream>>>(d_grad.p + nc, n - nc, d_sc.p);
      OSFM_LAUNCH_CHECK();
    }
    const int npack = 2 * nc + 1 + world;
    d_slots.reserve(npack);
    const int gsz = std::max(nc, world);
    ba_pack_lin<<<grid_for(gsz, 256), 256, 0, stream>>>(d_colnorm2.p, d_grad.p, d_sc.p, nc, rank, world, d_slots.p);
    OSFM_LAUNCH_CHECK();
    allreduce_dev(d_slots.p, npack);
    ba_unpack_lin<<<grid_for(gsz, 256), 256, 0, stream>>>(d_slots.p, nc, world, d_colnorm2.p, d_grad.p, d_sc.p);
    OSFM_LAUNCH_CHECK();
  } else if (n > 0) {
    ba_grad_max<<<grid_for(n, 256), 256, 0, stream>>>(d_grad.p, n, d_sc.p);
    OSFM_LAUNCH_CHECK();
  }
  const Scalars s = read_scalars();
  *grad_max = s.grad_max_bits;
  return s.cost;
}

void BA::build_system(double inv_radius, int* rank_flag, bool timed) {
  const int nc = rs.nc, P = rs.P, P_fast = rs.P_fast, nseg = rs.nseg, wc = rs.wc;
  const bool trace_on = switches().trace;
  double *const d_rhs_p = rs.d_rhs_p, *const d_S_p = rs.d_S_p;
  if (nc > 0) OSFM_CUDA(cudaMemsetAsync(d_Sbuf.p, 0, sizeof(double) * ((size_t)rs.nc_pad + (size_t)rs.s_upper_total), stream));
  if (P > 0) {
    const size_t smem = (size_t)SCHUR_KC * wc * (2 * 3 * sizeof(double) + 2 * sizeof(int)) +
                        (size_t)SCHUR_KC * 8 * sizeof(int) + (size_t)SCHUR_KC * SCHUR_KC * 9 * sizeof(int);
    if (timed) rs.tm_schur.start(stream);
    if (rs.schur != OSFM_SCHUR_NONE) {
      d_Vig.reserve(3 * (size_t)std::max(rs.npf, 1));
      if (rs.lin == LIN_FUSED)
        ba_point_blocks_sums<<<grid_for(P_fast, PB_THREADS), PB_THREADS, 0, stream>>>(
            rs.v, P_fast, d_ptsum.p, d_scale.p, d_diag.p, inv_radius, d_Vinv.p, d_gp.p, d_Vig.p, rank_flag);
      else
        ba_point_blocks<<<grid_for(P_fast, PB_THREADS), PB_THREADS, 0, stream>>>(rs.v, P_fast, d_scale.p, d_diag.p, inv_radius,
                                                                               d_Vinv.p, d_gp.p, d_Vig.p, rank_flag);
      OSFM_LAUNCH_CHECK();
    }
    if (rs.schur == OSFM_SCHUR_PIPE || rs.schur == OSFM_SCHUR_MMA) {
      unsigned long long* prof = nullptr;
      if (trace_on) {
        d_prof.reserve(16);
        OSFM_CUDA(cudaMemsetAsync(d_prof.p, 0, 16 * sizeof(unsigned long long), stream));
        prof = d_prof.p;
      }
      if (rs.schur == OSFM_SCHUR_PIPE) {
        auto kern = prof ? ba_schur_pipe<true> : ba_schur_pipe<false>;
        opt_in_smem(kern, (int)sizeof(SpSmem));
        const int grid = std::max(1, std::min(num_sms, rs.sp_nchunks));
        kern<<<grid, SP_THREADS, sizeof(SpSmem), stream>>>(rs.v, d_sp_chunks.p, rs.sp_nchunks, d_tab.p, d_scale.p, d_Vinv.p,
                                                          d_Vig.p, d_sp_ftab.p, d_S_p, d_rhs_p, prof);
        if (trace_on) {
          OSFM_LAUNCH_CHECK();
          unsigned long long hp[16];
          OSFM_CUDA(cudaMemcpyAsync(hp, d_prof.p, sizeof(hp), cudaMemcpyDeviceToHost, stream));
          OSFM_CUDA(cudaStreamSynchronize(stream));
          const unsigned long long nch = std::max<unsigned long long>(hp[3], 1);
          fprintf(stderr, "[osfm_ba] ba_schur_pipe (%d CTAs, %llu chunks) producer clocks / chunk: copy wait %llu buffer wait %llu build %llu\n",
                  grid, hp[3], hp[0] / nch, hp[1] / nch, hp[2] / nch);
          for (int gI = 0; gI < 2; ++gI) {
            const unsigned long long ns = std::max<unsigned long long>(hp[8 + 5 * gI], 1);
            fprintf(stderr, "[osfm_ba]   consumer group %d clocks / segment (%llu segments): tables %llu operand wait %llu mma %llu flush %llu\n",
                    gI, hp[8 + 5 * gI], hp[4 + 5 * gI] / ns, hp[5 + 5 * gI] / ns, hp[6 + 5 * gI] / ns, hp[7 + 5 * gI] / ns);
          }
        }
      } else {
        auto kern = wc == 9 ? ba_schur_mma<9> : ba_schur_mma<0>;
        opt_in_smem(kern, (int)sizeof(SegMmaSmem));
        kern<<<nseg, SM_THREADS, sizeof(SegMmaSmem), stream>>>(rs.v, d_seg_start.p, d_tab_off.p, d_tab.p, d_scale.p, d_Vinv.p,
                                                               d_Vig.p, d_S_p, d_rhs_p, prof);
      }
      OSFM_LAUNCH_CHECK();
      if (trace_on && rs.schur == OSFM_SCHUR_MMA) {
        unsigned long long hp[8];
        OSFM_CUDA(cudaMemcpyAsync(hp, d_prof.p, sizeof(hp), cudaMemcpyDeviceToHost, stream));
        OSFM_CUDA(cudaStreamSynchronize(stream));
        fprintf(stderr, "[osfm_ba] ba_schur_mma clocks / segment (thread 0): structure %llu offsets %llu loads %llu rows %llu mma %llu flush %llu\n",
                hp[0] / nseg, hp[1] / nseg, hp[2] / nseg, hp[3] / nseg, hp[4] / nseg, hp[5] / nseg);
      }
    } else if (rs.schur == OSFM_SCHUR_SIMT_SEGMENT) {
      const long long n_fast = rs.n_fast_obs;
      d_rowsJ.reserve((size_t)n_fast * wc * 3 + 8); d_rowsW.reserve((size_t)n_fast * wc * 3 + 8);
      d_rowsY.reserve((size_t)n_fast * wc * 3 + 8);
      ba_obs_rows<<<grid_for(n_fast * wc, 256), 256, 0, stream>>>(rs.v, rs.bm, rs.bsr, n_fast, d_scale.p, d_Vinv.p, d_Vig.p,
                                                                d_rowsJ.p, d_rowsW.p, d_rowsY.p, d_rhs_p);
      OSFM_LAUNCH_CHECK();
      auto kern = wc == 9 ? ba_schur_seg<9> : ba_schur_seg<0>;
      opt_in_smem(kern, (int)sizeof(SegSmem));
      kern<<<nseg, SEG_THREADS, sizeof(SegSmem), stream>>>(rs.v, rs.bm, rs.bsr, d_seg_start.p, n_fast, d_rowsJ.p, d_rowsW.p,
                                                           d_rowsY.p, d_S_p);
      OSFM_LAUNCH_CHECK();
    }
    if (P > P_fast) {
      ba_schur<<<P - P_fast, SCHUR_THREADS, smem, stream>>>(rs.v, rs.bm, rs.bsr, d_scale.p, d_diag.p, inv_radius, d_S_p,
                                                           d_rhs_p, d_Vinv.p, d_gp.p, P_fast, rs.ppv, d_pts[rs.cur].p, rank_flag);
      OSFM_LAUNCH_CHECK();
    }
    if (timed) rs.tm_schur.stop(stream);
  }
  if (nc > 0) {
    if (world > 1) allreduce_dev(d_Sbuf.p, (long long)rs.nc_pad + rs.s_upper_total);
    PriorView pall = rs.pv;
    pall.n_cam_rows = (int)rs.pr_cam_param.size();
    pall.n_pos_rows = (int)rs.pr_pos_inst.size();
    const int nall = pall.n_cam_rows + pall.n_pos_rows;
    if (nall > 0) {
      ba_prior_system<<<grid_for(nall, 128), 128, 0, stream>>>(pall, params_of(rs.cur), d_scale.p, d_prior_diag_off.p,
                                                              d_S_p, d_rhs_p);
      OSFM_LAUNCH_CHECK();
    }
    if (rs.NT > 0) {
      side_system<<<rs.NT, SIDE_THREADS, 0, stream>>>(rs.sv, rs.v, rs.bm, params_of(rs.cur), rs.bsr, d_scale.p, d_S_p, d_rhs_p);
      OSFM_LAUNCH_CHECK();
    }
    ba_finish_system<<<grid_for((long long)rs.n_upper * 32, 256), 256, 0, stream>>>(d_upper.p, rs.n_upper, rs.bsr, d_S_p,
                                                                                  d_diag.p, inv_radius);
    OSFM_LAUNCH_CHECK();
  }
}

int BA::solve_reduced() {
  const int nc = rs.nc;
  rs.tm_pcg.start(stream);
  pcg_convert<<<grid_for((long long)rs.n_blocks_all * 32, 256), 256, 0, stream>>>(
      rs.d_S_p, d_row_col.p, d_row_off.p, d_qoff.p, d_blk_row.p, rs.n_blocks_all, rs.bsr, d_row_M.p, d_rowbase.p, d_Spcg.p);
  OSFM_LAUNCH_CHECK();
  pcg_factor_groups<<<grid_for(rs.ngroups, 64), 64, 0, stream>>>(rs.d_S_p, rs.bsr, d_diag_off.p, d_grp_b1.p, d_grp_b2.p,
                                                                rs.ngroups, d_Minv.p);
  OSFM_LAUNCH_CHECK();
  OSFM_CUDA(cudaMemsetAsync(d_pcg.p, 0, sizeof(PcgState), stream));
  const int max_pcg = std::min(2 * nc + 100, 5000);
  int path = 0;
  if (rs.pcg_pipe_ok) {
    launch_cooperative(pcg_pipelined, rs.pcg_grid, PCG_THREADS, rs.pcg_pipe_smem, stream, d_Spcg.p, rs.lay, rs.bsr, d_Minv.p,
                       rs.d_rhs_p, d_px.p, d_pz.p, d_pp.p, d_pcg.p, nc, max_pcg, 1e-16, rs.pcg_pipe);
    OSFM_LAUNCH_CHECK();
    OSFM_CUDA(cudaMemcpyAsync(h_pcg.p, d_pcg.p, PCG_STATE_HEADER, cudaMemcpyDeviceToHost, stream));
    OSFM_CUDA(cudaStreamSynchronize(stream));
    const PcgState& h = *h_pcg.p;
    const int its = std::max(h.iterations, 1);
    if (switches().trace)
      fprintf(stderr, "[osfm_ba] pipelined pcg %d its converged %d, CTA0 clocks/it: stage %lld matvec %lld reduce %lld update %lld"
              " | wide barrier (all calls / its): own sums %lld release %lld collect %lld column sums %lld\n",
              h.iterations, h.converged, h.prof[0] / its, h.prof[1] / its, h.prof[2] / its, h.prof[3] / its, h.prof[4] / its,
              h.prof[5] / its, h.prof[6] / its, h.prof[7] / its);
    if (h.converged) {
      path = h.deflated ? OSFM_PCG_PIPELINED_DEFLATED : OSFM_PCG_PIPELINED;
    } else {
      rs.pcg_total += h.iterations;
      OSFM_CUDA(cudaMemsetAsync(d_pcg.p, 0, sizeof(PcgState), stream));
    }
  }
  if (!path) {
    path = rs.pcg_resident ? OSFM_PCG_CLASSIC_RESIDENT : OSFM_PCG_CLASSIC_STREAMED;
    launch_cooperative(rs.pcg_resident ? pcg_persistent<true> : pcg_persistent<false>, rs.pcg_grid, PCG_THREADS, rs.pcg_smem,
                       stream, d_Spcg.p, rs.lay, rs.bsr, d_Minv.p, rs.d_rhs_p, d_px.p, d_pr.p, d_pz.p, d_pp.p, d_pAp.p, d_Ap.p,
                       d_pcg.p, nc, max_pcg, 1e-16, rs.pcg_res);
    OSFM_LAUNCH_CHECK();
  }
  OSFM_CUDA(cudaMemcpyAsync(d_y.p, d_px.p, sizeof(double) * nc, cudaMemcpyDeviceToDevice, stream));
  OSFM_CUDA(cudaMemcpyAsync(h_pcg.p, d_pcg.p, PCG_STATE_HEADER, cudaMemcpyDeviceToHost, stream));
  rs.tm_pcg.stop(stream);
  return path;
}

void BA::back_substitute() {
  const int P = rs.P, npf = rs.npf;
  if (P == 0 || npf == 0) return;
  rs.tm_back.start(stream);
  d_bs_t.reserve(3 * (size_t)npf);
  OSFM_CUDA(cudaMemsetAsync(d_bs_t.p, 0, sizeof(double) * 3 * (size_t)npf, stream));
  if (rs.N > 0) {
    ba_backsub_rows<<<grid_for(rs.N, 256), 256, 0, stream>>>(rs.v, d_scale.p, d_y.p, d_bs_t.p);
    OSFM_LAUNCH_CHECK();
  }
  if (rs.have_pp) {
    ba_point_prior<3><<<grid_for(P, 128), 128, 0, stream>>>(rs.ppv, rs.v, params_of(rs.cur), nullptr, nullptr, d_bs_t.p, d_sc.p);
    OSFM_LAUNCH_CHECK();
  }
  ba_backsub_points<<<grid_for(npf, 256), 256, 0, stream>>>(rs.v, d_scale.p, d_Vinv.p, d_bs_t.p, d_y.p);
  OSFM_LAUNCH_CHECK();
  rs.tm_back.stop(stream);
}

void BA::capture_linear_system(int it, double radius, int pcg_path) {
  const int nc = rs.nc, n = rs.n, P = rs.P;
  download(cap_sbuf, d_Sbuf.p, (size_t)rs.nc_pad + (size_t)rs.s_total, stream);
  download(cap_upper, d_upper.p, rs.n_upper, stream);
  download(cap_y, d_px.p, nc, stream);
  download(cap_scale, d_scale.p, n, stream); download(cap_diag, d_diag.p, n, stream); download(cap_grad, d_grad.p, n, stream);
  download(cap_pt_poff, d_pt_poff.p, P, stream); download(cap_global_of, d_global_of.p, P, stream);
  const Params xp = params_of(rs.cur);
  download(cap_cam, xp.cam, cam_params.size(), stream); download(cap_inst, xp.inst, inst.size(), stream);
  download(cap_rc, xp.rc, rc.size(), stream); download(cap_pts, xp.pts, 3 * (size_t)P, stream);
  download(cap_ext, xp.ext, ext_values.size(), stream);
  OSFM_CUDA(cudaStreamSynchronize(stream));
  cap_blk_off = rs.blk_off; cap_blk_sz = rs.blk_sz; cap_nc_pad = rs.nc_pad;
  cap_info = osfm_ba_capture{};
  cap_info.iteration = it; cap_info.nc = nc; cap_info.n = n; cap_info.wc = rs.wc; cap_info.nres = rs.nres;
  cap_info.radius = radius;
  cap_info.nseg = rs.nseg; cap_info.p_fast = rs.P_fast; cap_info.p_slow = P - rs.P_fast;
  cap_info.schur_kernel = rs.schur;
  cap_info.sp_nchunks = rs.sp_nchunks;
  cap_info.pcg_kernel = pcg_path;
  cap_info.pcg_rescued = rs.pcg_pipe_ok && pcg_path != OSFM_PCG_PIPELINED_DEFLATED && pcg_path != OSFM_PCG_PIPELINED;
  cap_info.pcg_iterations = h_pcg.p->iterations;
  cap_info.pcg_rr = h_pcg.p->rr_final;
  cap_valid = true;
}

void BA::covariance_pass(int termination) {
  const int nc = rs.nc, n = rs.n, NI = rs.NI;
  cov_out.assign((size_t)NI * 36, 0.0);
  cov_status = OSFM_COV_SOLVER_FAILURE;
  cov_pass_ms = cov_chol_ms = 0.0;
  if (termination != 2) {
    const std::vector<int>& cov_inst = rs.cov_inst;
    const std::vector<int>& cov_bstart = rs.cov_bstart;
    double* const A = d_cov.p;
    double* const X = A + (size_t)nc * nc;
    double* const W = X + (size_t)rs.cov_m * rs.cov_m;
    double* const d0 = W + (cov_bstart.size() - 1) * COV_NB * COV_NB;
    double* const out = d0 + nc;
    int* const flags = d_cov_flags.p;
    const int m = rs.cov_m, n1 = nc - rs.cov_m;
    std::vector<int> perm(std::max(nc, 1));
    {
      std::vector<char> is_inst(std::max(nc, 1), 0);
      for (size_t q = 0; q < cov_inst.size(); ++q)
        for (int j = 0; j < 6; ++j) {
          perm[rs.inst_poff[cov_inst[q]] + j] = n1 + 6 * (int)q + j;
          is_inst[rs.inst_poff[cov_inst[q]] + j] = 1;
        }
      for (int g = 0, lead = 0; g < nc; ++g)
        if (!is_inst[g]) perm[g] = lead++;
    }
    upload(d_cov_perm, perm, stream);
    std::vector<int> inst_list = cov_inst;
    if (inst_list.empty()) inst_list.push_back(0);
    upload(d_cov_inst, inst_list, stream);
    OSFM_CUDA(cudaMemsetAsync(flags, 0, sizeof(int) * COV_F_COUNT, stream));
    const int potrf_smem = 2 * COV_NB * (COV_NB + 1) * (int)sizeof(double);
    const int gemm_smem = 2 * COV_NB * COV_LDS * (int)sizeof(double);
    opt_in_smem(cov_potrf_diag, potrf_smem);
    for (auto k : {cov_gemm<COV_TRSM>, cov_gemm<COV_SYRK>, cov_gemm<COV_TRI_DIAG>, cov_gemm<COV_TRI_UPD>}) opt_in_smem(k, gemm_smem);
    cudaEvent_t ce[4];
    for (auto& e : ce) OSFM_CUDA(cudaEventCreate(&e));
    OSFM_CUDA(cudaEventRecord(ce[0], stream));
    double gm = 0.0;
    linearize(rs.cur, false, &gm);
    if (n > 0) {
      ba_make_scale<<<grid_for(n, 256), 256, 0, stream>>>(d_colnorm2.p, d_scale.p, n);
      OSFM_LAUNCH_CHECK();
      ba_make_diag<<<grid_for(n, 256), 256, 0, stream>>>(d_colnorm2.p, d_scale.p, d_diag.p, n);
      OSFM_LAUNCH_CHECK();
    }
    segment_table_scales();
    build_system(0.0, flags + COV_F_POINT_RANK, false);
    OSFM_CUDA(cudaEventRecord(ce[1], stream));
    auto tiles = [](int k) { return (k + COV_NB - 1) / COV_NB; };
    CovGemm g{A, nc, X, m, n1, nullptr, 0, 0, flags};
    if (nc > 0) {
      OSFM_CUDA(cudaMemsetAsync(A, 0, sizeof(double) * (size_t)nc * nc, stream));
      OSFM_CUDA(cudaMemsetAsync(d0, 0, sizeof(double) * (size_t)nc, stream));
      cov_densify<<<grid_for((long long)rs.n_upper * 32, 256), 256, 0, stream>>>(d_upper.p, rs.n_upper, rs.bsr, rs.d_S_p,
                                                                                d_cov_perm.p, nc, A, d0);
      OSFM_LAUNCH_CHECK();
      for (size_t b = 0; b + 1 < cov_bstart.size(); ++b) {
        const int k0 = cov_bstart[b], kb = cov_bstart[b + 1] - k0, rem = nc - k0 - kb;
        cov_potrf_diag<<<1, COV_THREADS, 2 * COV_NB * (COV_NB + 1) * sizeof(double), stream>>>(
            A, nc, k0, kb, d0, W + b * COV_NB * COV_NB, flags);
        OSFM_LAUNCH_CHECK();
        if (rem == 0) continue;
        g.W = W + b * COV_NB * COV_NB; g.k0 = k0; g.kb = kb;
        cov_gemm<COV_TRSM><<<dim3(tiles(rem), 1), COV_THREADS, gemm_smem, stream>>>(g);
        OSFM_LAUNCH_CHECK();
        cov_gemm<COV_SYRK><<<dim3(tiles(rem), tiles(rem)), COV_THREADS, gemm_smem, stream>>>(g);
        OSFM_LAUNCH_CHECK();
      }
    }
    OSFM_CUDA(cudaEventRecord(ce[2], stream));
    if (m > 0) {
      cov_identity<<<grid_for((long long)m * m, 256), 256, 0, stream>>>(X, m);
      OSFM_LAUNCH_CHECK();
      for (size_t b = rs.cov_nb1; b + 1 < cov_bstart.size(); ++b) {
        const int k0 = cov_bstart[b] - n1, kb = cov_bstart[b + 1] - cov_bstart[b], rem = m - k0 - kb;
        g.W = W + b * COV_NB * COV_NB; g.k0 = k0; g.kb = kb;
        cov_gemm<COV_TRI_DIAG><<<dim3(1, tiles(k0 + kb)), COV_THREADS, gemm_smem, stream>>>(g);
        OSFM_LAUNCH_CHECK();
        if (rem == 0) continue;
        cov_gemm<COV_TRI_UPD><<<dim3(tiles(rem), tiles(k0 + kb)), COV_THREADS, gemm_smem, stream>>>(g);
        OSFM_LAUNCH_CHECK();
      }
      OSFM_CUDA(cudaMemsetAsync(out, 0, sizeof(double) * (size_t)NI * 36, stream));
      cov_blocks<<<(int)cov_inst.size(), COV_THREADS, 0, stream>>>(X, m, d_cov_inst.p, d_inst_poff.p, d_scale.p, flags,
                                                                   out, flags);
      OSFM_LAUNCH_CHECK();
    }
    OSFM_CUDA(cudaEventRecord(ce[3], stream));
    int hf[COV_F_COUNT];
    OSFM_CUDA(cudaMemcpyAsync(hf, flags, sizeof(hf), cudaMemcpyDeviceToHost, stream));
    if (m > 0) OSFM_CUDA(cudaMemcpyAsync(cov_out.data(), out, sizeof(double) * cov_out.size(), cudaMemcpyDeviceToHost, stream));
    OSFM_CUDA(cudaStreamSynchronize(stream));
    float ms_pass = 0.f, ms_chol = 0.f;
    OSFM_CUDA(cudaEventElapsedTime(&ms_pass, ce[0], ce[3]));
    OSFM_CUDA(cudaEventElapsedTime(&ms_chol, ce[1], ce[2]));
    for (auto& e : ce) cudaEventDestroy(e);
    cov_pass_ms = ms_pass; cov_chol_ms = ms_chol;
    cov_status = hf[COV_F_POINT_RANK] ? OSFM_COV_POINT_RANK_DEFICIENT
                 : hf[COV_F_CHOL]     ? OSFM_COV_CAMERA_RANK_DEFICIENT
                 : hf[COV_F_NONFINITE] ? OSFM_COV_NON_FINITE : OSFM_COV_OK;
    if (switches().trace && hf[COV_F_CHOL])
      fprintf(stderr, "[osfm_ba] covariances: reduced system rank deficient at dense column %d\n", hf[COV_F_CHOL_COL]);
  }
  cov_valid = cov_status == OSFM_COV_OK;
  if (!cov_valid) {
    std::fill(cov_out.begin(), cov_out.end(), 0.0);
    for (int i = 0; i < NI; ++i)
      for (int j = 0; j < 6; ++j) cov_out[(size_t)i * 36 + j * 7] = j < 3 ? 1e-5 : 1e-2;
  }
  cov_ran = true;
  trace("covariances");
}

void BA::write_results(osfm_ba_summary sum) {
  const int cur = rs.cur, P = rs.P, Pfull = rs.Pfull;
  const long long Nfull = rs.Nfull;
  download(cam_params, d_cam[cur].p, cam_params.size(), stream); download(inst, d_inst[cur].p, inst.size(), stream);
  download(rc, d_rc[cur].p, rc.size(), stream); download(ext_values, d_ext[cur].p, ext_values.size(), stream);
  d_full_pts.reserve(3 * (size_t)std::max(Pfull, 1));
  if (world > 1) OSFM_CUDA(cudaMemsetAsync(d_full_pts.p, 0, sizeof(double) * 3 * (size_t)Pfull, stream));
  if (P > 0) {
    ord_scatter_points<<<grid_for(P, 256), 256, 0, stream>>>(P, d_pts[cur].p, d_global_of.p, d_full_pts.p);
    OSFM_LAUNCH_CHECK();
  }
  allreduce_dev(d_full_pts.p, 3 * (long long)Pfull);
  download(pts, d_full_pts.p, 3 * (size_t)Pfull, stream);
  reproj_valid = false;
  if (compute_reproj && Nfull > 0) {
    d_reproj.reserve(3 * (size_t)Nfull);
    OSFM_CUDA(cudaMemsetAsync(d_reproj.p, 0, sizeof(double) * 3 * (size_t)Nfull, stream));
    if (rs.N > 0) {
      ba_linearize<2><<<grid_for(rs.N, 128), 128, 0, stream>>>(rs.v, params_of(cur), d_sc.p, d_reproj.p);
      OSFM_LAUNCH_CHECK();
    }
    allreduce_dev(d_reproj.p, 3 * Nfull);
    reproj_valid = true;
  }
  OSFM_CUDA(cudaStreamSynchronize(stream));
  trace("results");
  if (switches().trace && world > 1)
    fprintf(stderr, "[osfm_ba] rank %d: %d all-reduces, host %.3f ms, device (traced, serialised) %.3f ms\n", rank, ar_calls,
            ar_host_ms, ar_dev_ms);
  float dev_ms = 0.f;
  OSFM_CUDA(cudaEventElapsedTime(&dev_ms, rs.ev0, rs.ev1));
  cudaEventDestroy(rs.ev0); cudaEventDestroy(rs.ev1);
  rs.tm_lin.collect(); rs.tm_schur.collect(); rs.tm_pcg.collect(); rs.tm_back.collect();
  sum.time_device_ms = dev_ms;
  sum.time_linearize_ms = rs.tm_lin.total_ms;
  sum.linearize_launches = rs.tm_lin.count;
  sum.time_schur_ms = rs.tm_schur.total_ms;
  sum.schur_launches = rs.tm_schur.count;
  sum.time_pcg_ms = rs.tm_pcg.total_ms;
  sum.time_backsub_ms = rs.tm_back.total_ms;
  sum.num_observations_local = rs.N;
  sum.reduced_dim = rs.nc;
  sum.reduced_blocks = rs.n_blocks_all;
  sum.reduced_nnz = rs.s_total;
  sum.jac_planes = rs.nres * (rs.wc + 3 + 1);
  rs.tm_lin.destroy(); rs.tm_schur.destroy(); rs.tm_pcg.destroy(); rs.tm_back.destroy();
  sum.kernel_launches = g_kernel_launches.load() - rs.launches0;
  sum.time_run_s = std::chrono::duration<double>(std::chrono::high_resolution_clock::now() - rs.t_start).count();
  summary = sum;
  has_run = true;
}

void BA::run() {
  OSFM_CUDA(cudaSetDevice(device));
  rs = RunState{};
  rs.t_start = rs.t_prev = std::chrono::high_resolution_clock::now();
  ar_calls = 0; ar_host_ms = 0.0; ar_dev_ms = 0.0;
  if (cam_type.empty() && n_obs_full > 0) throw ArgError("observations but no cameras");
  if (cap_iter > 0 && world > 1) throw ArgError("the linear-system capture supports world == 1 only");
  if (cov_on && world > 1) throw ArgError("covariance estimation supports world == 1 only");
  cap_valid = cov_ran = false;
  if (!cov_on) d_cov.release();
  rs.launches0 = g_kernel_launches.load();

  plan_layout();
  trace("layout");
  order_observations();
  trace("sort");
  plan_prior_rows();
  trace("priors");
  upload_problem();
  OSFM_CUDA(cudaEventCreate(&rs.ev0)); OSFM_CUDA(cudaEventCreate(&rs.ev1));
  trace("upload");
  rs.tm_lin.init(); rs.tm_schur.init(); rs.tm_pcg.init(); rs.tm_back.init();
  trace("pre-struct");
  discover_structure();
  plan_pcg();
  trace("structure");
  if (cov_on) reserve_covariance();

  const int n = rs.n, nc = rs.nc;
  int& cur = rs.cur;
  if (world > 1) {
    OSFM_CUDA(cudaMemsetAsync(d_sc.p, 0, sizeof(Scalars), stream));
    allreduce_dev(&d_sc.p->cost, 1);
    OSFM_CUDA(cudaStreamSynchronize(stream));
  }
  OSFM_CUDA(cudaEventRecord(rs.ev0, stream));
  double radius = 1e4;
  const double max_radius = 1e16, min_radius = 1e-32, min_rel_decrease = 1e-3;
  const double ftol = 1e-6, gtol = 1e-10, ptol = 1e-8;
  double decrease_factor = 2.0;
  bool reuse_diagonal = false;
  int n_invalid = 0, it = 0, n_success = 0, n_solves = 0;
  int termination = 1;
  std::string message = "Maximum number of iterations reached.";

  build_segment_tables();
  double grad_max = 0.0;
  double cost = linearize(cur, true, &grad_max);
  const double initial_cost = cost;
  if (n > 0) {
    ba_make_scale<<<grid_for(n, 256), 256, 0, stream>>>(d_colnorm2.p, d_scale.p, n);
    OSFM_LAUNCH_CHECK();
  }
  segment_table_scales();
  if (switches().pcg_deflate && rs.pcg_pipe_ok && rs.NI > 0 && nc > 0) {
    d_Wdef.reserve((size_t)PCG_ND * nc);
    OSFM_CUDA(cudaMemsetAsync(d_Wdef.p, 0, sizeof(double) * PCG_ND * (size_t)nc, stream));
    pcg_gauge_vectors<<<grid_for(rs.NI, 128), 128, 0, stream>>>(rs.NI, d_inst_poff.p, params_of(cur).inst, d_scale.p, nc, d_Wdef.p);
    OSFM_LAUNCH_CHECK();
    rs.pcg_pipe.Wdef = d_Wdef.p;
  }
  double x_norm = n > 0 ? x_norm_of(cur) : 0.0;

  if (grad_max <= gtol || n == 0) {
    termination = 0;
    message = n == 0 ? "No free parameters." : "Gradient tolerance reached.";
  }
  while (termination == 1) {
    if (it >= max_iterations) break;
    if (radius < min_radius) { termination = 0; message = "Minimum trust region radius reached."; break; }
    ++it;
    if (!reuse_diagonal) {
      ba_make_diag<<<grid_for(n, 256), 256, 0, stream>>>(d_colnorm2.p, d_scale.p, d_diag.p, n);
      OSFM_LAUNCH_CHECK();
    }
    const double inv_radius = 1.0 / radius;
    build_system(inv_radius, nullptr, true);
    OSFM_CUDA(cudaMemsetAsync(d_y.p, 0, sizeof(double) * rs.nz, stream));
    int pcg_path = 0;
    if (nc > 0) {
      pcg_path = solve_reduced();
      if (it == cap_iter) capture_linear_system(it, radius, pcg_path);
    }
    ++n_solves;
    back_substitute();
    OSFM_CUDA(cudaMemsetAsync(&d_sc.p->model_change, 0, sizeof(double) * 3, stream));
    if (n > 0) {
      ba_model_change_alg<<<grid_for(n, 256), 256, 0, stream>>>(n, nc, rank == 0, d_grad.p, d_scale.p, d_diag.p, inv_radius, d_y.p, d_sc.p);
      OSFM_LAUNCH_CHECK();
    }
    const int cand = cur ^ 1;
    update_params(cur, cand, 1.0, d_ext_lower.p);
    if (world > 1) allreduce_dev(&d_sc.p->model_change, 3);
    const Scalars sm = read_scalars();
    bool ok = true;
    if (nc > 0) {
      const PcgState& h = *h_pcg.p;
      const int pcg_it = h.iterations, its = std::max(pcg_it, 1);
      rs.pcg_total += pcg_it;
      if (switches().trace && (pcg_path == OSFM_PCG_CLASSIC_RESIDENT || pcg_path == OSFM_PCG_CLASSIC_STREAMED))
        fprintf(stderr, "[osfm_ba] pcg %d its, CTA0 clocks/it: stage %lld matvec %lld reduce1 %lld phaseB %lld reduce2 %lld (resident %d)\n",
                pcg_it, h.prof[0] / its, h.prof[1] / its, h.prof[2] / its, h.prof[3] / its, h.prof[4] / its, (int)rs.pcg_resident);
      if (!(h.rr_final == h.rr_final)) ok = false;
    }
    const double model_change = sm.model_change;
    double step_norm = std::sqrt(sm.step_norm2);
    if (!ok || !(model_change > 0.0) || !std::isfinite(step_norm)) {
      if (++n_invalid >= 5) { termination = 2; message = "Too many consecutive invalid steps."; break; }
      radius *= 0.5;
      reuse_diagonal = true;
      continue;
    }
    n_invalid = 0;
    double cand_cost = eval_cost(cand);
    if (rs.constrained) {
      auto step_to = [&](double alpha) {
        OSFM_CUDA(cudaMemsetAsync(&d_sc.p->step_norm2, 0, sizeof(double) * 2, stream));
        update_params(cur, cand, alpha, d_ext_lower.p);
        if (world > 1) allreduce_dev(&d_sc.p->step_norm2, 2);
        return std::sqrt(read_scalars().step_norm2);
      };
      OSFM_CUDA(cudaMemsetAsync(&d_sc.p->gdot, 0, sizeof(double), stream));
      ba_grad_dot<<<grid_for(n, 256), 256, 0, stream>>>(n, nc, rank == 0, d_grad.p, d_scale.p, d_y.p, d_sc.p);
      OSFM_LAUNCH_CHECK();
      if (world > 1) allreduce_dev(&d_sc.p->gdot, 1);
      const double g0 = read_scalars().gdot;
      double alpha = 1.0;
      bool ok_ls = false;
      for (int ls = 0; ls < 20; ++ls) {
        if (ls > 0) { step_norm = step_to(alpha); cand_cost = eval_cost(cand); }
        if (std::isfinite(cand_cost) && cand_cost <= cost + 1e-4 * g0 * alpha) { ok_ls = true; break; }
        alpha *= 0.5;
      }
      if (!ok_ls) { step_norm = step_to(1.0); cand_cost = eval_cost(cand); }
    }
    if (step_norm <= ptol * (x_norm + ptol)) { termination = 0; message = "Parameter tolerance reached."; break; }
    const double cost_change = cost - cand_cost;
    if (std::fabs(cost_change) <= ftol * cost) { termination = 0; message = "Function tolerance reached."; break; }
    const double rel = cost_change / model_change;
    if (rel > min_rel_decrease) {
      cur = cand;
      cost = linearize(cur, true, &grad_max);
      x_norm = x_norm_of(cur);
      radius = std::min(max_radius, radius / std::max(1.0 / 3.0, 1.0 - std::pow(2.0 * rel - 1.0, 3)));
      decrease_factor = 2.0;
      reuse_diagonal = false;
      ++n_success;
      if (grad_max <= gtol) { termination = 0; message = "Gradient tolerance reached."; break; }
    } else {
      radius /= decrease_factor;
      decrease_factor *= 2.0;
      reuse_diagonal = true;
    }
  }
  OSFM_CUDA(cudaEventRecord(rs.ev1, stream));
  osfm_ba_summary sum{};
  sum.iterations = it;
  sum.successful_steps = n_success;
  sum.linear_solves = n_solves;
  sum.pcg_iterations = rs.pcg_total;
  sum.termination = termination;
  sum.initial_cost = initial_cost;
  sum.final_cost = eval_cost(cur);
  snprintf(sum.message, sizeof(sum.message), "%s", message.c_str());
  trace("lm");

  if (cov_on) covariance_pass(termination);
  write_results(sum);
}

}

struct osfm_ba {
  osfm::BA impl;
  explicit osfm_ba(int dev) : impl(dev) {}
};
using osfm::ArgError;

extern "C" {

int osfm_camera_num_params(int projection_type) {
  if (projection_type < 0 || projection_type > 9) return -1;
  return osfm::model_num_params(projection_type);
}

int osfm_ba_create(int device, osfm_ba** out) {
  OSFM_API_BEGIN
  if (!out) throw ArgError("null out");
  int count = 0;
  OSFM_CUDA(cudaGetDeviceCount(&count));
  if (device < 0 || device >= count) throw ArgError("no such CUDA device");
  *out = new osfm_ba(device);
  OSFM_API_END
}
int osfm_ba_destroy(osfm_ba* ba) {
  OSFM_API_BEGIN
  delete ba;
  OSFM_API_END
}
#define OSFM_BA_CHECK if (!ba) throw ArgError("null ba handle");

int osfm_ba_set_cameras(osfm_ba* ba, int n, const int32_t* type, const double* params, const int32_t* constant,
                        const double* prior, const double* prior_sigma, const int32_t* prior_log) {
  OSFM_API_BEGIN
  OSFM_BA_CHECK
  auto& b = ba->impl;
  if (n < 0 || (n > 0 && (!type || !params || !constant || !prior || !prior_sigma || !prior_log)))
    throw ArgError("bad camera arrays");
  int total = 0;
  for (int k = 0; k < n; ++k) {
    if (type[k] < 0 || type[k] > 9) throw ArgError("Invalid ProjectionType");
    total += osfm::model_num_params(type[k]);
  }
  b.cam_type.assign(type, type + n);
  b.cam_const.assign(constant, constant + n);
  b.cam_params.assign(params, params + total);
  b.cam_prior.assign(prior, prior + total);
  b.cam_prior_sigma.assign(prior_sigma, prior_sigma + total);
  b.cam_prior_log.assign(prior_log, prior_log + total);
  OSFM_API_END
}
int osfm_ba_set_rig_instances(osfm_ba* ba, int n, const double* pose6, const int32_t* constant,
                              const int32_t* has_position_prior, const double* prior_position3,
                              const double* prior_std3) {
  OSFM_API_BEGIN
  OSFM_BA_CHECK
  auto& b = ba->impl;
  if (n < 0 || (n > 0 && (!pose6 || !constant))) throw ArgError("bad rig instance arrays");
  b.inst.assign(pose6, pose6 + 6 * (size_t)n);
  b.inst_const.assign(constant, constant + n);
  b.inst_has_prior.assign(n, 0);
  b.inst_prior_pos.assign(3 * (size_t)n, 0.0);
  b.inst_prior_std.assign(3 * (size_t)n, 1.0);
  if (has_position_prior) {
    if (!prior_position3 || !prior_std3) throw ArgError("position prior arrays missing");
    b.inst_has_prior.assign(has_position_prior, has_position_prior + n);
    b.inst_prior_pos.assign(prior_position3, prior_position3 + 3 * (size_t)n);
    b.inst_prior_std.assign(prior_std3, prior_std3 + 3 * (size_t)n);
  }
  OSFM_API_END
}
int osfm_ba_set_rig_cameras(osfm_ba* ba, int n, const double* pose6, const int32_t* constant) {
  OSFM_API_BEGIN
  OSFM_BA_CHECK
  if (n < 0 || (n > 0 && (!pose6 || !constant))) throw ArgError("bad rig camera arrays");
  ba->impl.rc.assign(pose6, pose6 + 6 * (size_t)n);
  ba->impl.rc_const.assign(constant, constant + n);
// ... 369 lines not shown
```

### opensfm_b200/csrc/ba_reduced.cuh

```cuda
#pragma once
#include <cub/cub.cuh>

#include "ba_pcg_plan.h"

namespace osfm {

constexpr unsigned long long BSR_EMPTY = ~0ull;

struct BsrView {
  const unsigned long long* tkeys;
  const int* tvals;
  unsigned tmask;
  int nblk;
  const int* blk_off;
  const int* blk_sz;
};

__device__ __forceinline__ unsigned bsr_hash(unsigned long long k) {
  k ^= k >> 33; k *= 0xff51afd7ed558ccdULL; k ^= k >> 33; k *= 0xc4ceb9fe1a85ec53ULL; k ^= k >> 33;
  return (unsigned)k;
}
__device__ __forceinline__ int bsr_lookup(const BsrView& h, int bi, int bj) {
  const unsigned long long key = (unsigned long long)bi * (unsigned)h.nblk + (unsigned)bj;
  unsigned slot = bsr_hash(key) & h.tmask;
// ... 991 lines not shown
  const double ds = d * scale[col];
  atomicAdd(&Sval[prior_diag_off[row]], ds * ds);
  atomicAdd(&rhs[col], ds * r);
}

__global__ void __launch_bounds__(256)
    ba_finish_system(const int4* __restrict__ upper, int n_upper, BsrView h, double* Sval,
                     const double* __restrict__ diag, double inv_radius) {
  const int w = blockIdx.x * (blockDim.x >> 5) + (threadIdx.x >> 5);
  const int lane = threadIdx.x & 31;
  if (w >= n_upper) return;
  const int4 u = upper[w];
  const int szi = h.blk_sz[u.x], szj = h.blk_sz[u.y];
  if (u.x == u.y) {
    const int g0 = h.blk_off[u.x];
    for (int e = lane; e < szi * szi; e += 32) {
      const int r = e / szi, c = e % szi;
      if (r == c) Sval[u.z + e] += diag[g0 + r] * inv_radius;
      else if (c < r) Sval[u.z + e] = Sval[u.z + c * szi + r];
    }
  } else {
    for (int e = lane; e < szi * szj; e += 32) {
      const int r = e / szj, c = e % szj;
      Sval[u.w + c * szi + r] = Sval[u.z + e];
    }
  }
}

constexpr int MAXB = 16;

struct PcgLayout {
  const int* row_of;
  const int* row_M;
  const long long* rowbase;
  const int* cbase;
  const int* colidx;
  int ngroups;
  const int* grp_b1;
  const int* grp_b2;
};

__global__ void pcg_row_sizes(const int* __restrict__ row_ptr, const int* __restrict__ row_col, BsrView h, int* row_M,
                              int* qoff, int* blk_row) {
  const int b = blockIdx.x * blockDim.x + threadIdx.x;
  if (b >= h.nblk) return;
  int acc = 0;
  for (int e = row_ptr[b]; e < row_ptr[b + 1]; ++e) {
    qoff[e] = acc;
    blk_row[e] = b;
    acc += h.blk_sz[row_col[e]];
  }
  row_M[b] = acc;
}
__global__ void pcg_fill_colidx(const int* __restrict__ row_col, const int* __restrict__ qoff,
                                const int* __restrict__ blk_row, int n_all, BsrView h, const int* __restrict__ cbase,
                                int* colidx, int* row_of) {
  const int e = blockIdx.x * blockDim.x + threadIdx.x;
  if (e >= n_all) return;
  const int b = blk_row[e], cb = row_col[e];
  const int m = h.blk_sz[cb], co = h.blk_off[cb];
  for (int j = 0; j < m; ++j) colidx[cbase[b] + qoff[e] + j] = co + j;
  if (cb == b) {
    const int n = h.blk_sz[b], o = h.blk_off[b];
    for (int r = 0; r < n; ++r) row_of[o + r] = b;
  }
}
__global__ void __launch_bounds__(256)
    pcg_convert(const double* __restrict__ Sval, const int* __restrict__ row_col, const int* __restrict__ row_off,
                const int* __restrict__ qoff, const int* __restrict__ blk_row, int n_all, BsrView h,
                const int* __restrict__ row_M, const long long* __restrict__ rowbase, double* __restrict__ Spcg) {
  const int e = blockIdx.x * (blockDim.x >> 5) + (threadIdx.x >> 5);
  const int lane = threadIdx.x & 31;
  if (e >= n_all) return;
  const int b = blk_row[e];
  const int n = h.blk_sz[b], m = h.blk_sz[row_col[e]], M = row_M[b];
  const double* src = Sval + row_off[e];
  double* dst = Spcg + rowbase[b] + qoff[e];
  for (int t = lane; t < n * m; t += 32) {
    const int r = t / m, j = t - r * m;
    dst[(size_t)r * M + j] = src[t];
  }
}

__global__ void pcg_factor_groups(const double* __restrict__ Sval, BsrView h, const int* __restrict__ diag_off,
                                  const int* __restrict__ grp_b1, const int* __restrict__ grp_b2, int ngroups,
                                  double* __restrict__ Minv) {
  const int g = blockIdx.x * blockDim.x + threadIdx.x;
  if (g >= ngroups) return;
  const int b1 = grp_b1[g], b2 = grp_b2[g];
  const int n1 = h.blk_sz[b1], n2 = b2 >= 0 ? h.blk_sz[b2] : 0;
  const int n = n1 + n2;
  double L[MAXB * MAXB];
  const double* D1 = Sval + diag_off[b1];
  for (int i = 0; i < n1; ++i)
    for (int j = 0; j <= i; ++j) L[i * MAXB + j] = D1[i * n1 + j];
  if (b2 >= 0) {
    const double* D2 = Sval + diag_off[b2];
    for (int i = 0; i < n2; ++i)
      for (int j = 0; j <= i; ++j) L[(n1 + i) * MAXB + n1 + j] = D2[i * n2 + j];
    const int o12 = bsr_lookup(h, min(b1, b2), max(b1, b2));
    for (int i = 0; i < n2; ++i)
      for (int j = 0; j < n1; ++j) {
        double v = 0.0;
        if (o12 >= 0) v = b1 < b2 ? Sval[o12 + j * n2 + i] : Sval[o12 + i * n1 + j];
        L[(n1 + i) * MAXB + j] = v;
      }
  }
  for (int j = 0; j < n; ++j) {
    double d = L[j * MAXB + j];
    for (int k = 0; k < j; ++k) d -= L[j * MAXB + k] * L[j * MAXB + k];
    d = sqrt(fmax(d, 1e-300));
    L[j * MAXB + j] = d;
    for (int i = j + 1; i < n; ++i) {
      double s = L[i * MAXB + j];
      for (int k = 0; k < j; ++k) s -= L[i * MAXB + k] * L[j * MAXB + k];
      L[i * MAXB + j] = s / d;
    }
  }
  double* out = Minv + (size_t)g * MAXB * MAXB;
  for (int c = 0; c < n; ++c) {
    double y[MAXB];
    for (int i = 0; i < n; ++i) {
      double s = (i == c) ? 1.0 : 0.0;
      for (int k = 0; k < i; ++k) s -= L[i * MAXB + k] * y[k];
      y[i] = s / L[i * MAXB + i];
    }
    for (int i = n - 1; i >= 0; --i) {
      double s = y[i];
      for (int k = i + 1; k < n; ++k) s -= L[k * MAXB + i] * y[k];
      y[i] = s / L[i * MAXB + i];
    }
    for (int i = 0; i < n; ++i) out[i * MAXB + c] = y[i];
  }
}

constexpr int PCG_MAX_CTAS = 256;
constexpr int PCG_FLAG_STRIDE = 32;
struct PcgState {
  int iterations;
  int converged;
  double rr_final;
  int deflated;
  long long prof[8];
  alignas(16) double slot[2][PCG_MAX_CTAS][4];
  double slotx[2][PCG_MAX_CTAS][12];
  unsigned flags[PCG_MAX_CTAS * PCG_FLAG_STRIDE];
};
constexpr size_t PCG_STATE_HEADER = offsetof(PcgState, slot);

struct PcgResident {
  const int* row_lo;
  int off_S, off_cols, off_rows;
  int max_rows;
};

__device__ __forceinline__ double ldcg_d(const double* p) { return __ldcg(p); }

template <int NV>
__device__ __forceinline__ void grid_reduce(PcgState* st, unsigned nblocks, unsigned& gen, double a, double b, double c,
                                            double& A, double& B, double& C, double (*red)[3]) {
  static_assert(NV == 2 || NV == 3, "two or three sums");
  ++gen;
  const int lane = threadIdx.x & 31, warp = threadIdx.x >> 5, nwarps = blockDim.x >> 5;
#pragma unroll
  for (int o = 16; o; o >>= 1) {
    a += __shfl_xor_sync(0xffffffffu, a, o);
    b += __shfl_xor_sync(0xffffffffu, b, o);
    if (NV == 3) c += __shfl_xor_sync(0xffffffffu, c, o);
  }
  if (lane == 0) { red[warp][0] = a; red[warp][1] = b; if (NV == 3) red[warp][2] = c; }
  __syncthreads();
  if (threadIdx.x == 0) {
    double sa = 0.0, sb = 0.0, sc = 0.0;
    for (int w = 0; w < nwarps; ++w) { sa += red[w][0]; sb += red[w][1]; if (NV == 3) sc += red[w][2]; }
    double* sl = st->slot[gen & 1][blockIdx.x];
    __stcg(reinterpret_cast<double2*>(sl), make_double2(sa, sb));
    if (NV == 3) __stcg(sl + 2, sc);
    asm volatile("st.release.gpu.global.u32 [%0], %1;" ::"l"(&st->flags[blockIdx.x * PCG_FLAG_STRIDE]), "r"(gen) : "memory");
  }
  double va = 0.0, vb = 0.0, vc = 0.0;
  if (threadIdx.x < nblocks) {
    const long long t0 = clock64();
    unsigned cur;
    do {
      asm volatile("ld.acquire.gpu.global.u32 %0, [%1];" : "=r"(cur) : "l"(&st->flags[threadIdx.x * PCG_FLAG_STRIDE]) : "memory");
      if (clock64() - t0 > 8000000000LL) __trap();
    } while ((int)(cur - gen) < 0);
    const double* sl = st->slot[gen & 1][threadIdx.x];
    const double2 ab = __ldcg(reinterpret_cast<const double2*>(sl));
    va = ab.x; vb = ab.y;
    if (NV == 3) vc = __ldcg(sl + 2);
  }
  __syncthreads();
#pragma unroll
  for (int o = 16; o; o >>= 1) {
    va += __shfl_xor_sync(0xffffffffu, va, o);
    vb += __shfl_xor_sync(0xffffffffu, vb, o);
    if (NV == 3) vc += __shfl_xor_sync(0xffffffffu, vc, o);
  }
  if (lane == 0) { red[warp][0] = va; red[warp][1] = vb; if (NV == 3) red[warp][2] = vc; }
  __syncthreads();
  double sa = 0.0, sb = 0.0, sc = 0.0;
  const int wmax = (int)((nblocks + 31) >> 5);
  for (int w = 0; w < wmax; ++w) { sa += red[w][0]; sb += red[w][1]; if (NV == 3) sc += red[w][2]; }
  A = sa; B = sb;
  if (NV == 3) C = sc;
  __syncthreads();
}

__device__ __forceinline__ void pcg_apply_group(const BsrView& h, const PcgLayout& L, const double* Minv, int g, int lane,
                                                double rn, double* z, double* a_rz, double* a_rr, int n, int o_lane) {
  const double* M = Minv + (size_t)g * MAXB * MAXB;
  double s = 0.0;
  for (int j = 0; j < n; ++j) {
    const double rj = __shfl_sync(0xffffffffu, rn, j);
    if (lane < n) s += M[lane * MAXB + j] * rj;
// ... 656 lines not shown
```

Measured before the change: 685.1 million.

## Move LM trust-region loop on device with CUDA graph conditional nodes

Moves the Levenberg-Marquardt control logic (radius updates, acceptance, termination checks, PCG fallback) into small device kernels that keep an LmState, and captures each iteration into a CUDA graph with conditional If nodes, so the host no longer reads scalars back and synchronises every iteration. A host-loop fallback remains behind an environment switch. It also warp-parallelises the per-group Cholesky and inverse in pcg_factor_groups using shared memory, and reduces grad_max atomics to one per block. The cost is added graph-capture complexity, device-side phase timing kernels, and a dependence on conditional-node support in the CUDA runtime.

```diff
diff --git a/include/opensfm_b200.h b/include/opensfm_b200.h
--- a/include/opensfm_b200.h
+++ b/include/opensfm_b200.h
@@ -148,6 +148,7 @@
   int jac_planes;
   int64_t kernel_launches;
   char message[128];
+  int device_loop;
 } osfm_ba_summary;
 int osfm_ba_get_summary(osfm_ba* ba, osfm_ba_summary* out);
 
diff --git a/opensfm_b200/_lib.py b/opensfm_b200/_lib.py
--- a/opensfm_b200/_lib.py
+++ b/opensfm_b200/_lib.py
@@ -30,6 +30,7 @@
         ("time_schur_ms", c_double), ("schur_launches", c_int64), ("time_pcg_ms", c_double),
         ("time_backsub_ms", c_double), ("num_observations_local", c_int64), ("reduced_dim", c_int),
         ("reduced_blocks", c_int), ("reduced_nnz", c_int64), ("jac_planes", c_int), ("kernel_launches", c_int64), ("message", ctypes.c_char * 128),
+        ("device_loop", c_int),
     ]
 
 
diff --git a/opensfm_b200/csrc/ba.cu b/opensfm_b200/csrc/ba.cu
--- a/opensfm_b200/csrc/ba.cu
+++ b/opensfm_b200/csrc/ba.cu
@@ -44,6 +44,24 @@
   double grad_max_bits;
   double gdot;
 };
+
+enum LmBranch { LM_EVAL = 1, LM_ACCEPT = 2, LM_PCG_CLASSIC = 4 };
+enum LmMessage { LM_MSG_MAX_ITERATIONS, LM_MSG_NO_FREE, LM_MSG_GTOL, LM_MSG_MIN_RADIUS, LM_MSG_INVALID, LM_MSG_PTOL,
+                 LM_MSG_FTOL };
+enum LmPhase { LM_PH_LIN, LM_PH_SCHUR, LM_PH_PCG, LM_PH_BACK, LM_PH_COUNT };
+struct LmState {
+  double radius, decrease_factor, cost, initial_cost, x_norm;
+  int reuse_diagonal;
+  int it, n_invalid, n_success, n_solves, n_eval, n_classic, pcg_total;
+  int termination, message;
+  int running;
+  int branch;
+  int pcg_path;
+  unsigned long long phase_t0[LM_PH_COUNT], phase_ns[LM_PH_COUNT];
+  int phase_count[LM_PH_COUNT];
+};
+constexpr double LM_RADIUS0 = 1e4, LM_MAX_RADIUS = 1e16, LM_MIN_RADIUS = 1e-32, LM_MIN_REL_DECREASE = 1e-3;
+constexpr double LM_FTOL = 1e-6, LM_GTOL = 1e-10, LM_PTOL = 1e-8;
 
 __device__ __forceinline__ double block_reduce_sum(double v) {
   __shared__ double sh[32];
@@ -397,9 +415,18 @@
   const int i = blockIdx.x * blockDim.x + threadIdx.x;
   if (i < n) scale[i] = 1.0 / (1.0 + sqrt(colnorm2[i]));
 }
-__global__ void ba_make_diag(const double* colnorm2, const double* scale, double* diag, int n) {
+__global__ void ba_make_diag(const double* colnorm2, const double* scale, double* diag, int n, const LmState* st = nullptr,
+                             double* diag_r = nullptr) {
   const int i = blockIdx.x * blockDim.x + threadIdx.x;
-  if (i < n) diag[i] = fmin(fmax(colnorm2[i] * scale[i] * scale[i], 1e-6), 1e32);
+  if (i >= n) return;
+  double d;
+  if (st && st->reuse_diagonal) {
+    d = diag[i];
+  } else {
+    d = fmin(fmax(colnorm2[i] * scale[i] * scale[i], 1e-6), 1e32);
+    diag[i] = d;
+  }
+  if (diag_r) diag_r[i] = d * (1.0 / st->radius);
 }
 __global__ void ba_pack_lin(const double* __restrict__ colnorm2, const double* __restrict__ grad, const Scalars* sc, int nc,
                             int rank, int world, double* __restrict__ pack) {
@@ -419,12 +446,18 @@
   for (int o = 16; o; o >>= 1) v = fmax(v, __shfl_xor_sync(0xffffffffu, v, o));
   if ((threadIdx.x & 31) == 0 && v > 0.0) atomic_max_nonneg(&sc->grad_max_bits, v);
 }
-__global__ void ba_grad_max(const double* grad, int n, Scalars* sc) {
+__global__ void __launch_bounds__(256) ba_grad_max(const double* grad, int n, Scalars* sc) {
+  __shared__ double wmax[8];
   const int i = blockIdx.x * blockDim.x + threadIdx.x;
   double v = i < n ? fabs(grad[i]) : 0.0;
 #pragma unroll
   for (int o = 16; o; o >>= 1) v = fmax(v, __shfl_xor_sync(0xffffffffu, v, o));
-  if ((threadIdx.x & 31) == 0 && v > 0.0) atomic_max_nonneg(&sc->grad_max_bits, v);
+  if ((threadIdx.x & 31) == 0) wmax[threadIdx.x >> 5] = v;
+  __syncthreads();
+  if (threadIdx.x == 0) {
+    for (int w = 1; w < (int)(blockDim.x >> 5); ++w) v = fmax(v, wmax[w]);
+    if (v > 0.0) atomic_max_nonneg(&sc->grad_max_bits, v);
+  }
 }
 
 }
@@ -515,9 +548,9 @@
         const int gi = which == 3 ? base + 3 * g + j : g + j;
         double d = -alpha * scale[gi] * y[gi];
         if (lower && val + d < lower[o + j]) d = lower[o + j] - val;
-        xn += val * val;
         sn += d * d;
         val += d;
+        xn += val * val;
       }
       dst[o + j] = val;
     }
@@ -548,6 +581,105 @@
   if (i < n && (i >= nc || cam_side)) v = 0.5 * y[i] * (grad[i] * scale[i] + diag[i] * inv_radius * y[i]);
   const double t = block_reduce_sum(v);
   if (threadIdx.x == 0 && t != 0.0) atomicAdd(&sc->model_change, t);
+}
+
+__global__ void ba_lm_init(LmState* st, const Scalars* sc, int n) {
+  st->radius = LM_RADIUS0;
+  st->decrease_factor = 2.0;
+  st->cost = st->initial_cost = sc->cost;
+  st->x_norm = n > 0 ? sqrt(sc->x_norm2) : 0.0;
+  st->termination = 1;
+  st->message = LM_MSG_MAX_ITERATIONS;
+  if (n == 0) { st->termination = 0; st->message = LM_MSG_NO_FREE; }
+  else if (sc->grad_max_bits <= LM_GTOL) { st->termination = 0; st->message = LM_MSG_GTOL; }
+}
+__global__ void ba_lm_next(LmState* st, int max_iterations, cudaGraphConditionalHandle cond, int set_cond) {
+  int run = 0;
+  if (st->termination == 1 && st->it < max_iterations) {
+    if (st->radius < LM_MIN_RADIUS) { st->termination = 0; st->message = LM_MSG_MIN_RADIUS; }
+    else { ++st->it; run = 1; }
+  }
+  st->running = run;
+  st->branch = 0;
+  if (set_cond) cudaGraphSetConditional(cond, run);
+}
+__global__ void ba_lm_pcg_check(LmState* st, const PcgState* pcg, int classic_path, cudaGraphConditionalHandle cond,
+                                int set_cond) {
+  const int fallback = pcg->converged ? 0 : 1;
+  if (fallback) {
+    st->pcg_total += pcg->iterations;
+    st->pcg_path = classic_path;
+    st->branch |= LM_PCG_CLASSIC;
+    ++st->n_classic;
+  } else {
+    st->pcg_path = pcg->deflated ? OSFM_PCG_PIPELINED_DEFLATED : OSFM_PCG_PIPELINED;
+  }
+  if (set_cond) cudaGraphSetConditional(cond, fallback);
+}
+__global__ void ba_lm_check(LmState* st, const Scalars* sc, const PcgState* pcg, int nc, cudaGraphConditionalHandle cond,
+                            int set_cond) {
+  ++st->n_solves;
+  bool ok = true;
+  if (nc > 0) {
+    st->pcg_total += pcg->iterations;
+    if (!(pcg->rr_final == pcg->rr_final)) ok = false;
+  }
+  const double step_norm = sqrt(sc->step_norm2);
+  int eval = 0;
+  if (!ok || !(sc->model_change > 0.0) || !isfinite(step_norm)) {
+    if (++st->n_invalid >= 5) {
+      st->termination = 2;
+      st->message = LM_MSG_INVALID;
+    } else {
+      st->radius *= 0.5;
+      st->reuse_diagonal = 1;
+    }
+  } else {
+    st->n_invalid = 0;
+    ++st->n_eval;
+    st->branch |= LM_EVAL;
+    eval = 1;
+  }
+  if (set_cond) cudaGraphSetConditional(cond, eval);
+}
+__global__ void ba_lm_step(LmState* st, const Scalars* sc, cudaGraphConditionalHandle cond, int set_cond) {
+  int accept = 0;
+  if (st->branch & LM_EVAL) {
+    const double step_norm = sqrt(sc->step_norm2), cost_change = st->cost - sc->cost;
+    if (step_norm <= LM_PTOL * (st->x_norm + LM_PTOL)) {
+      st->termination = 0;
+      st->message = LM_MSG_PTOL;
+    } else if (fabs(cost_change) <= LM_FTOL * st->cost) {
+      st->termination = 0;
+      st->message = LM_MSG_FTOL;
+    } else {
+      const double rel = cost_change / sc->model_change;
+      if (rel > LM_MIN_REL_DECREASE) {
+        st->x_norm = sqrt(sc->x_norm2);
+        st->radius = fmin(LM_MAX_RADIUS, st->radius / fmax(1.0 / 3.0, 1.0 - pow(2.0 * rel - 1.0, 3.0)));
+        st->decrease_factor = 2.0;
+        st->reuse_diagonal = 0;
+        ++st->n_success;
+        st->branch |= LM_ACCEPT;
+        accept = 1;
+      } else {
+        st->radius /= st->decrease_factor;
+        st->decrease_factor *= 2.0;
+        st->reuse_diagonal = 1;
+      }
+    }
+  }
+  if (set_cond) cudaGraphSetConditional(cond, accept);
+}
+__global__ void ba_lm_accepted(LmState* st, const Scalars* sc) {
+  st->cost = sc->cost;
+  if (sc->grad_max_bits <= LM_GTOL) { st->termination = 0; st->message = LM_MSG_GTOL; }
+}
+__global__ void ba_lm_phase(LmState* st, int stop, int start) {
+  unsigned long long t;
+  asm volatile("mov.u64 %0, %%globaltimer;" : "=l"(t));
+  if (stop >= 0) { st->phase_ns[stop] += t - st->phase_t0[stop]; ++st->phase_count[stop]; }
+  if (start >= 0) st->phase_t0[start] = t;
 }
 
 __global__ void ba_eval_one(int type, const double* in, int use_rc, double* out, int* nres_out) {
@@ -562,24 +694,6 @@
   for (int i = 0; i < 18; ++i) out[69 + i] = jrc[i];
   for (int i = 0; i < 9; ++i) out[87 + i] = jp[i];
 }
-
-struct EventTimer {
-  cudaEvent_t a = nullptr, b = nullptr;
-  double total_ms = 0.0;
-  long long count = 0;
-  bool pending = false;
-  void init() { OSFM_CUDA(cudaEventCreate(&a)); OSFM_CUDA(cudaEventCreate(&b)); }
-  void destroy() { if (a) cudaEventDestroy(a); if (b) cudaEventDestroy(b); a = b = nullptr; }
-  void start(cudaStream_t st) { collect(); OSFM_CUDA(cudaEventRecord(a, st)); }
-  void stop(cudaStream_t st) { OSFM_CUDA(cudaEventRecord(b, st)); pending = true; }
-  void collect() {
-    if (!pending) return;
-    OSFM_CUDA(cudaEventSynchronize(b));
-    float ms = 0.f;
-    OSFM_CUDA(cudaEventElapsedTime(&ms, a, b));
-    total_ms += ms; ++count; pending = false;
-  }
-};
 
 template <class T>
 static void upload(DevBuf<T>& d, const std::vector<T>& h, cudaStream_t st) {
@@ -652,6 +766,7 @@
   bool pcg_resident = !env_starts_with("OSFM_BA_PCG_RESIDENT", '0');
   bool pcg_pipelined = !env_starts_with("OSFM_BA_PCG_PIPELINED", '0');
   bool pcg_deflate = !env_starts_with("OSFM_BA_PCG_DEFLATE", '0');
+  bool host_loop = env_starts_with("OSFM_BA_HOST_LOOP", '1');
 };
 static const BaSwitches& switches() {
   static const BaSwitches s;
@@ -677,8 +792,6 @@
   int uniform_type = -1;
   bool constrained = false;
   bool have_pp = false, add_priors = false;
-  int cur = 0;
-  int pcg_total = 0;
   std::vector<int> cam_off, cam_np, cam_poff, inst_poff, rc_poff, ext_off, ext_poff, blk_off, blk_sz;
   std::vector<int> cam_blk, inst_blk, rc_blk, ext_blk, side_jofs, side_rofs, grp_b1, grp_b2;
   std::vector<int> pr_cam_param, pr_cam_col, pr_cam_log, pr_pos_kind, pr_pos_inst, pr_pos_axis, pr_pos_col;
@@ -699,7 +812,11 @@
   BAView v{}; PriorView pv{}; SideView sv{}; PointPriorView ppv{}; BlkMaps bm{}; BsrView bsr{}; PcgLayout lay{};
   double *d_rhs_p = nullptr, *d_S_p = nullptr;
   cudaEvent_t ev0 = nullptr, ev1 = nullptr;
-  EventTimer tm_lin, tm_schur, tm_pcg, tm_back;
+  cudaGraph_t cap_graph = nullptr;
+  std::vector<cudaGraphNode_t> cap_deps;
+  cudaGraphConditionalHandle h_pcg = 0, h_eval = 0, h_accept = 0;
+  int64_t k_body = 0, k_pcg = 0, k_eval = 0, k_accept = 0;
+  bool device_loop = false;
 };
 
 struct BA {
@@ -799,6 +916,9 @@
   DevBuf<double> d_pr_cam_prior, d_pr_cam_scale, d_pr_pos_prior, d_pr_pos_scale;
   DevBuf<Scalars> d_sc;
   PinnedBuf<Scalars> h_sc;
+  DevBuf<LmState> d_lm;
+  PinnedBuf<LmState> h_lm;
+  DevBuf<double> d_diag_r;
   DevBuf<int> d_pr_pos_kind, d_ext_off, d_ext_np, d_ext_poff, d_ext_blk, d_side_jofs, d_side_rofs;
   DevBuf<double> d_ext[2], d_ext_lower, d_side_consts, d_side_J, d_side_r, d_pp_d, d_pp_x0;
   DevBuf<SideTerm> d_side_terms;
@@ -811,6 +931,8 @@
     OSFM_CUDA(cudaEventCreateWithFlags(&ev_obs, cudaEventDisableTiming));
     h_sc.reserve(1);
     h_pcg.reserve(1);
+    d_lm.reserve(1);
+    h_lm.reserve(1);
     OSFM_CUDA(cudaDeviceGetAttribute(&num_sms, cudaDevAttrMultiProcessorCount, device));
   }
   ~BA() {
@@ -825,6 +947,59 @@
     OSFM_CUDA(cudaMemcpyAsync(h_sc.p, d_sc.p, sizeof(Scalars), cudaMemcpyDeviceToHost, stream));
     OSFM_CUDA(cudaStreamSynchronize(stream));
     return *h_sc.p;
+  }
+  const LmState& read_lm() {
+    OSFM_CUDA(cudaMemcpyAsync(h_lm.p, d_lm.p, sizeof(LmState), cudaMemcpyDeviceToHost, stream));
+    OSFM_CUDA(cudaStreamSynchronize(stream));
+    return *h_lm.p;
+  }
+  void lm_phase(int stop, int start) {
+    ba_lm_phase<<<1, 1, 0, stream>>>(d_lm.p, stop, start);
+    OSFM_LAUNCH_CHECK();
+  }
+  void capture_begin(cudaGraph_t g) {
+    rs.cap_graph = g;
+    OSFM_CUDA(cudaStreamBeginCaptureToGraph(stream, g, rs.cap_deps.data(), nullptr, rs.cap_deps.size(),
+                                            cudaStreamCaptureModeRelaxed));
+  }
+  void capture_end() {
+    cudaStreamCaptureStatus status;
+    const cudaGraphNode_t* deps = nullptr;
+    size_t ndeps = 0;
+    OSFM_CUDA(cudaStreamGetCaptureInfo(stream, &status, nullptr, nullptr, &deps, &ndeps));
+    rs.cap_deps.assign(deps, deps + ndeps);
+    cudaGraph_t g = nullptr;
+    OSFM_CUDA(cudaStreamEndCapture(stream, &g));
+  }
+  cudaGraph_t add_conditional(cudaGraph_t g, cudaGraphConditionalHandle handle, cudaGraphConditionalNodeType type) {
+    cudaGraphNodeParams p{};
+    p.type = cudaGraphNodeTypeConditional;
+    p.conditional.handle = handle;
+    p.conditional.type = type;
+    p.conditional.size = 1;
+    cudaGraphNode_t node;
+    OSFM_CUDA(cudaGraphAddNode(&node, g, rs.cap_deps.data(), rs.cap_deps.size(), &p));
+    rs.cap_deps.assign(1, node);
+    return p.conditional.phGraph_out[0];
+  }
+  template <class F>
+  int64_t lm_if(cudaGraphConditionalHandle handle, int bit, F fn) {
+    const int64_t k0 = g_kernel_launches.load();
+    if (!rs.cap_graph) {
+      if (read_lm().branch & bit) fn();
+      return 0;
+    }
+    cudaGraph_t outer = rs.cap_graph;
+    capture_end();
+    cudaGraph_t body = add_conditional(outer, handle, cudaGraphCondTypeIf);
+    std::vector<cudaGraphNode_t> after = rs.cap_deps;
+    rs.cap_deps.clear();
+    capture_begin(body);
+    fn();
+    capture_end();
+    rs.cap_deps = after;
+    capture_begin(outer);
+    return g_kernel_launches.load() - k0;
   }
   int ar_calls = 0;
   double ar_host_ms = 0.0, ar_dev_ms = 0.0;
@@ -887,12 +1062,11 @@
     if (P) { ba_update<<<grid_for(P, 128), 128, 0, stream>>>(3, P, d_pt_poff.p, nullptr, nullptr, 3, rs.nc, a.pts, b.pts, d_scale.p, d_y.p, d_sc.p, 1, nullptr, alpha); OSFM_LAUNCH_CHECK(); }
     if (NE) { ba_update<<<grid_for(NE, 128), 128, 0, stream>>>(0, NE, d_ext_poff.p, d_ext_off.p, d_ext_np.p, 0, 0, a.ext, b.ext, d_scale.p, d_y.p, d_sc.p, rank == 0, lower, alpha); OSFM_LAUNCH_CHECK(); }
   }
-  double x_norm_of(int b) {
+  void x_norm_pass(int b) {
     OSFM_CUDA(cudaMemsetAsync(&d_sc.p->x_norm2, 0, sizeof(double), stream));
     OSFM_CUDA(cudaMemsetAsync(d_y.p, 0, sizeof(double) * rs.nz, stream));
     update_params(b, b, 1.0, nullptr);
     allreduce_dev(&d_sc.p->x_norm2, 1);
-    return std::sqrt(read_scalars().x_norm2);
   }
   Params params_of(int b) { return Params{d_cam[b].p, d_inst[b].p, d_rc[b].p, d_pts[b].p, d_ext[b].p}; }
   RunState rs;
@@ -900,10 +1074,10 @@
   void run();
   void plan_layout(), order_observations(), plan_prior_rows(), upload_problem(), discover_structure(), plan_pcg(),
       reserve_covariance(), build_segment_tables(), segment_table_scales();
-  double eval_cost(int b), linearize(int b, bool timed, double* grad_max);
-  void build_system(double inv_radius, int* rank_flag, bool timed), back_substitute();
-  int solve_reduced();
-  void capture_linear_system(int it, double radius, int pcg_path), covariance_pass(int termination);
+  void eval_cost(int b), linearize(int b, bool timed);
+  void build_system(const double* diag, double inv_radius, int* rank_flag, bool timed), back_substitute();
+  void solve_reduced(), lm_iteration(), line_search(), accept_candidate(), run_lm_graph();
+  void capture_linear_system(int it, double radius), covariance_pass(int termination);
   void write_results(osfm_ba_summary sum);
 };
 
@@ -1191,8 +1365,9 @@
   const size_t Nz = (size_t)std::max<long long>(rs.N, 1);
   d_r.reserve(nres * Nz); d_Jc.reserve((size_t)nres * wc * Nz); d_Jp.reserve((size_t)nres * 3 * Nz);
   d_Vinv.reserve(6 * (size_t)std::max(npf, 1)); d_gp.reserve(3 * (size_t)std::max(npf, 1));
+  d_Vig.reserve(3 * (size_t)std::max(npf, 1)); d_bs_t.reserve(3 * (size_t)std::max(npf, 1));
   const size_t nz = rs.nz;
-  d_scale.reserve(nz); d_colnorm2.reserve(nz); d_grad.reserve(nz); d_diag.reserve(nz); d_y.reserve(nz);
+  d_scale.reserve(nz); d_colnorm2.reserve(nz); d_grad.reserve(nz); d_diag.reserve(nz); d_diag_r.reserve(nz); d_y.reserve(nz);
   d_px.reserve(std::max(nc, 1)); d_pr.reserve(std::max(nc, 1)); d_pz.reserve(std::max(nc, 1));
   d_pp.reserve(std::max(nc, 1)); d_pAp.reserve(std::max(nc, 1));
   d_pcg.reserve(1);
@@ -1492,6 +1667,10 @@
   rs.schur = nseg == 0 ? OSFM_SCHUR_NONE
              : !use_mma ? OSFM_SCHUR_SIMT_SEGMENT
              : use_pipe ? OSFM_SCHUR_PIPE : OSFM_SCHUR_MMA;
+  if (rs.schur == OSFM_SCHUR_SIMT_SEGMENT) {
+    const size_t rows = (size_t)rs.n_fast_obs * wc * 3 + 8;
+    d_rowsJ.reserve(rows); d_rowsW.reserve(rows); d_rowsY.reserve(rows);
+  }
   rs.lin = nseg == 0 ? LIN_NONE
            : rs.sp_nchunks == 0 ? LIN_SEGMENTS
            : rs.uniform_type == PT_PERSPECTIVE ? LIN_FUSED : LIN_CHUNKS;
@@ -1503,7 +1682,7 @@
   OSFM_LAUNCH_CHECK();
 }
 
-double BA::eval_cost(int b) {
+void BA::eval_cost(int b) {
   OSFM_CUDA(cudaMemsetAsync(&d_sc.p->cost, 0, sizeof(double), stream));
   if (rs.N > 0) launch_linearize<0>(b);
   const int npr_local = rs.pv.n_cam_rows + rs.pv.n_pos_rows;
@@ -1520,11 +1699,10 @@
     OSFM_LAUNCH_CHECK();
   }
   allreduce_dev(&d_sc.p->cost, 1);
-  return read_scalars().cost;
-}
-
-
-double BA::linearize(int b, bool timed, double* grad_max) {
+}
+
+
+void BA::linearize(int b, bool timed) {
   const long long N = rs.N, n_fast_obs = rs.n_fast_obs;
   const int nc = rs.nc, n = rs.n, nseg = rs.nseg, wc = rs.wc, NT = rs.NT;
   OSFM_CUDA(cudaMemsetAsync(d_sc.p, 0, sizeof(Scalars), stream));
@@ -1533,11 +1711,11 @@
   if (N > 0 && rs.lin == LIN_FUSED) {
     d_ptsum.reserve(9 * (size_t)std::max(rs.npf, 1));
     const int grid = (int)((n_fast_obs + FL_WIN - 1) / FL_WIN + (N - n_fast_obs + FL_THREADS - 1) / FL_THREADS);
-    if (timed) rs.tm_lin.start(stream);
+    if (timed) lm_phase(-1, LM_PH_LIN);
     ba_linearize_fused<PT_PERSPECTIVE><<<grid, FL_THREADS, 0, stream>>>(rs.v, params_of(b), d_sc.p, d_sp_chunks.p, rs.sp_nchunks,
                                                                         n_fast_obs, d_tab.p, d_colnorm2.p, d_grad.p, d_ptsum.p);
     OSFM_LAUNCH_CHECK();
-    if (timed) rs.tm_lin.stop(stream);
+    if (timed) lm_phase(LM_PH_LIN, -1);
     if (N > n_fast_obs) {
       ba_colnorm_grad_points<<<grid_for(N - n_fast_obs, 256), 256, 0, stream>>>(rs.v, n_fast_obs, d_colnorm2.p, d_grad.p);
       OSFM_LAUNCH_CHECK();
@@ -1545,9 +1723,9 @@
       OSFM_LAUNCH_CHECK();
     }
   } else if (N > 0) {
-    if (timed) rs.tm_lin.start(stream);
+    if (timed) lm_phase(-1, LM_PH_LIN);
     launch_linearize<1>(b);
-    if (timed) rs.tm_lin.stop(stream);
+    if (timed) lm_phase(LM_PH_LIN, -1);
     ba_colnorm_grad_points<<<grid_for(N, 256), 256, 0, stream>>>(rs.v, 0, d_colnorm2.p, d_grad.p);
     OSFM_LAUNCH_CHECK();
     if (rs.lin == LIN_CHUNKS) {
@@ -1602,12 +1780,9 @@
     ba_grad_max<<<grid_for(n, 256), 256, 0, stream>>>(d_grad.p, n, d_sc.p);
     OSFM_LAUNCH_CHECK();
   }
-  const Scalars s = read_scalars();
-  *grad_max = s.grad_max_bits;
-  return s.cost;
-}
-
-void BA::build_system(double inv_radius, int* rank_flag, bool timed) {
+}
+
+void BA::build_system(const double* diag, double inv_radius, int* rank_flag, bool timed) {
   const int nc = rs.nc, P = rs.P, P_fast = rs.P_fast, nseg = rs.nseg, wc = rs.wc;
   const bool trace_on = switches().trace;
   double *const d_rhs_p = rs.d_rhs_p, *const d_S_p = rs.d_S_p;
@@ -1615,14 +1790,13 @@
   if (P > 0) {
     const size_t smem = (size_t)SCHUR_KC * wc * (2 * 3 * sizeof(double) + 2 * sizeof(int)) +
                         (size_t)SCHUR_KC * 8 * sizeof(int) + (size_t)SCHUR_KC * SCHUR_KC * 9 * sizeof(int);
-    if (timed) rs.tm_schur.start(stream);
+    if (timed) lm_phase(-1, LM_PH_SCHUR);
     if (rs.schur != OSFM_SCHUR_NONE) {
-      d_Vig.reserve(3 * (size_t)std::max(rs.npf, 1));
       if (rs.lin == LIN_FUSED)
         ba_point_blocks_sums<<<grid_for(P_fast, PB_THREADS), PB_THREADS, 0, stream>>>(
-            rs.v, P_fast, d_ptsum.p, d_scale.p, d_diag.p, inv_radius, d_Vinv.p, d_gp.p, d_Vig.p, rank_flag);
+            rs.v, P_fast, d_ptsum.p, d_scale.p, diag, inv_radius, d_Vinv.p, d_gp.p, d_Vig.p, rank_flag);
       else
-        ba_point_blocks<<<grid_for(P_fast, PB_THREADS), PB_THREADS, 0, stream>>>(rs.v, P_fast, d_scale.p, d_diag.p, inv_radius,
+        ba_point_blocks<<<grid_for(P_fast, PB_THREADS), PB_THREADS, 0, stream>>>(rs.v, P_fast, d_scale.p, diag, inv_radius,
                                                                                d_Vinv.p, d_gp.p, d_Vig.p, rank_flag);
       OSFM_LAUNCH_CHECK();
     }
@@ -1669,8 +1843,6 @@
       }
     } else if (rs.schur == OSFM_SCHUR_SIMT_SEGMENT) {
       const long long n_fast = rs.n_fast_obs;
-      d_rowsJ.reserve((size_t)n_fast * wc * 3 + 8); d_rowsW.reserve((size_t)n_fast * wc * 3 + 8);
-      d_rowsY.reserve((size_t)n_fast * wc * 3 + 8);
       ba_obs_rows<<<grid_for(n_fast * wc, 256), 256, 0, stream>>>(rs.v, rs.bm, rs.bsr, n_fast, d_scale.p, d_Vinv.p, d_Vig.p,
                                                                 d_rowsJ.p, d_rowsW.p, d_rowsY.p, d_rhs_p);
       OSFM_LAUNCH_CHECK();
@@ -1681,11 +1853,11 @@
       OSFM_LAUNCH_CHECK();
     }
     if (P > P_fast) {
-      ba_schur<<<P - P_fast, SCHUR_THREADS, smem, stream>>>(rs.v, rs.bm, rs.bsr, d_scale.p, d_diag.p, inv_radius, d_S_p,
-                                                           d_rhs_p, d_Vinv.p, d_gp.p, P_fast, rs.ppv, d_pts[rs.cur].p, rank_flag);
+      ba_schur<<<P - P_fast, SCHUR_THREADS, smem, stream>>>(rs.v, rs.bm, rs.bsr, d_scale.p, diag, inv_radius, d_S_p,
+                                                           d_rhs_p, d_Vinv.p, d_gp.p, P_fast, rs.ppv, d_pts[0].p, rank_flag);
       OSFM_LAUNCH_CHECK();
     }
-    if (timed) rs.tm_schur.stop(stream);
+    if (timed) lm_phase(LM_PH_SCHUR, -1);
   }
   if (nc > 0) {
     if (world > 1) allreduce_dev(d_Sbuf.p, (long long)rs.nc_pad + rs.s_upper_total);
@@ -1694,92 +1866,101 @@
     pall.n_pos_rows = (int)rs.pr_pos_inst.size();
     const int nall = pall.n_cam_rows + pall.n_pos_rows;
     if (nall > 0) {
-      ba_prior_system<<<grid_for(nall, 128), 128, 0, stream>>>(pall, params_of(rs.cur), d_scale.p, d_prior_diag_off.p,
+      ba_prior_system<<<grid_for(nall, 128), 128, 0, stream>>>(pall, params_of(0), d_scale.p, d_prior_diag_off.p,
                                                               d_S_p, d_rhs_p);
       OSFM_LAUNCH_CHECK();
     }
     if (rs.NT > 0) {
-      side_system<<<rs.NT, SIDE_THREADS, 0, stream>>>(rs.sv, rs.v, rs.bm, params_of(rs.cur), rs.bsr, d_scale.p, d_S_p, d_rhs_p);
+      side_system<<<rs.NT, SIDE_THREADS, 0, stream>>>(rs.sv, rs.v, rs.bm, params_of(0), rs.bsr, d_scale.p, d_S_p, d_rhs_p);
       OSFM_LAUNCH_CHECK();
     }
     ba_finish_system<<<grid_for((long long)rs.n_upper * 32, 256), 256, 0, stream>>>(d_upper.p, rs.n_upper, rs.bsr, d_S_p,
-                                                                                  d_diag.p, inv_radius);
-    OSFM_LAUNCH_CHECK();
-  }
-}
-
-int BA::solve_reduced() {
+                                                                                  diag, inv_radius);
+    OSFM_LAUNCH_CHECK();
+  }
+}
+
+void BA::solve_reduced() {
   const int nc = rs.nc;
-  rs.tm_pcg.start(stream);
+  lm_phase(-1, LM_PH_PCG);
   pcg_convert<<<grid_for((long long)rs.n_blocks_all * 32, 256), 256, 0, stream>>>(
       rs.d_S_p, d_row_col.p, d_row_off.p, d_qoff.p, d_blk_row.p, rs.n_blocks_all, rs.bsr, d_row_M.p, d_rowbase.p, d_Spcg.p);
   OSFM_LAUNCH_CHECK();
-  pcg_factor_groups<<<grid_for(rs.ngroups, 64), 64, 0, stream>>>(rs.d_S_p, rs.bsr, d_diag_off.p, d_grp_b1.p, d_grp_b2.p,
+  pcg_factor_groups<<<grid_for((long long)rs.ngroups * 32, 32 * PFG_WARPS), 32 * PFG_WARPS, 0, stream>>>(rs.d_S_p, rs.bsr, d_diag_off.p, d_grp_b1.p, d_grp_b2.p,
                                                                 rs.ngroups, d_Minv.p);
   OSFM_LAUNCH_CHECK();
   OSFM_CUDA(cudaMemsetAsync(d_pcg.p, 0, sizeof(PcgState), stream));
   const int max_pcg = std::min(2 * nc + 100, 5000);
-  int path = 0;
+  const int classic_path = rs.pcg_resident ? OSFM_PCG_CLASSIC_RESIDENT : OSFM_PCG_CLASSIC_STREAMED;
+  auto classic = [&]() {
+    launch_cooperative(rs.pcg_resident ? pcg_persistent<true> : pcg_persistent<false>, rs.pcg_grid, PCG_THREADS, rs.pcg_smem,
+                       stream, d_Spcg.p, rs.lay, rs.bsr, d_Minv.p, rs.d_rhs_p, d_px.p, d_pr.p, d_pz.p, d_pp.p, d_pAp.p, d_Ap.p,
+                       d_pcg.p, nc, max_pcg, 1e-16, rs.pcg_res);
+    OSFM_LAUNCH_CHECK();
+    if (switches().trace) {
+      OSFM_CUDA(cudaMemcpyAsync(h_pcg.p, d_pcg.p, PCG_STATE_HEADER, cudaMemcpyDeviceToHost, stream));
+      OSFM_CUDA(cudaStreamSynchronize(stream));
+      const PcgState& h = *h_pcg.p;
+      const int its = std::max(h.iterations, 1);
+      fprintf(stderr, "[osfm_ba] pcg %d its, CTA0 clocks/it: stage %lld matvec %lld reduce1 %lld phaseB %lld reduce2 %lld (resident %d)\n",
+              h.iterations, h.prof[0] / its, h.prof[1] / its, h.prof[2] / its, h.prof[3] / its, h.prof[4] / its, (int)rs.pcg_resident);
+    }
+  };
   if (rs.pcg_pipe_ok) {
     launch_cooperative(pcg_pipelined, rs.pcg_grid, PCG_THREADS, rs.pcg_pipe_smem, stream, d_Spcg.p, rs.lay, rs.bsr, d_Minv.p,
                        rs.d_rhs_p, d_px.p, d_pz.p, d_pp.p, d_pcg.p, nc, max_pcg, 1e-16, rs.pcg_pipe);
     OSFM_LAUNCH_CHECK();
-    OSFM_CUDA(cudaMemcpyAsync(h_pcg.p, d_pcg.p, PCG_STATE_HEADER, cudaMemcpyDeviceToHost, stream));
-    OSFM_CUDA(cudaStreamSynchronize(stream));
-    const PcgState& h = *h_pcg.p;
-    const int its = std::max(h.iterations, 1);
-    if (switches().trace)
+    if (switches().trace) {
+      OSFM_CUDA(cudaMemcpyAsync(h_pcg.p, d_pcg.p, PCG_STATE_HEADER, cudaMemcpyDeviceToHost, stream));
+      OSFM_CUDA(cudaStreamSynchronize(stream));
+      const PcgState& h = *h_pcg.p;
+      const int its = std::max(h.iterations, 1);
       fprintf(stderr, "[osfm_ba] pipelined pcg %d its converged %d, CTA0 clocks/it: stage %lld matvec %lld reduce %lld update %lld"
               " | wide barrier (all calls / its): own sums %lld release %lld collect %lld column sums %lld\n",
               h.iterations, h.converged, h.prof[0] / its, h.prof[1] / its, h.prof[2] / its, h.prof[3] / its, h.prof[4] / its,
               h.prof[5] / its, h.prof[6] / its, h.prof[7] / its);
-    if (h.converged) {
-      path = h.deflated ? OSFM_PCG_PIPELINED_DEFLATED : OSFM_PCG_PIPELINED;
-    } else {
-      rs.pcg_total += h.iterations;
+    }
+    ba_lm_pcg_check<<<1, 1, 0, stream>>>(d_lm.p, d_pcg.p, classic_path, rs.h_pcg, rs.cap_graph != nullptr);
+    OSFM_LAUNCH_CHECK();
+    rs.k_pcg = lm_if(rs.h_pcg, LM_PCG_CLASSIC, [&]() {
       OSFM_CUDA(cudaMemsetAsync(d_pcg.p, 0, sizeof(PcgState), stream));
-    }
-  }
-  if (!path) {
-    path = rs.pcg_resident ? OSFM_PCG_CLASSIC_RESIDENT : OSFM_PCG_CLASSIC_STREAMED;
-    launch_cooperative(rs.pcg_resident ? pcg_persistent<true> : pcg_persistent<false>, rs.pcg_grid, PCG_THREADS, rs.pcg_smem,
-                       stream, d_Spcg.p, rs.lay, rs.bsr, d_Minv.p, rs.d_rhs_p, d_px.p, d_pr.p, d_pz.p, d_pp.p, d_pAp.p, d_Ap.p,
-                       d_pcg.p, nc, max_pcg, 1e-16, rs.pcg_res);
-    OSFM_LAUNCH_CHECK();
+      classic();
+    });
+  } else {
+    classic();
   }
   OSFM_CUDA(cudaMemcpyAsync(d_y.p, d_px.p, sizeof(double) * nc, cudaMemcpyDeviceToDevice, stream));
-  OSFM_CUDA(cudaMemcpyAsync(h_pcg.p, d_pcg.p, PCG_STATE_HEADER, cudaMemcpyDeviceToHost, stream));
-  rs.tm_pcg.stop(stream);
-  return path;
+  lm_phase(LM_PH_PCG, -1);
 }
 
 void BA::back_substitute() {
   const int P = rs.P, npf = rs.npf;
   if (P == 0 || npf == 0) return;
-  rs.tm_back.start(stream);
-  d_bs_t.reserve(3 * (size_t)npf);
+  lm_phase(-1, LM_PH_BACK);
   OSFM_CUDA(cudaMemsetAsync(d_bs_t.p, 0, sizeof(double) * 3 * (size_t)npf, stream));
   if (rs.N > 0) {
     ba_backsub_rows<<<grid_for(rs.N, 256), 256, 0, stream>>>(rs.v, d_scale.p, d_y.p, d_bs_t.p);
     OSFM_LAUNCH_CHECK();
   }
   if (rs.have_pp) {
-    ba_point_prior<3><<<grid_for(P, 128), 128, 0, stream>>>(rs.ppv, rs.v, params_of(rs.cur), nullptr, nullptr, d_bs_t.p, d_sc.p);
+    ba_point_prior<3><<<grid_for(P, 128), 128, 0, stream>>>(rs.ppv, rs.v, params_of(0), nullptr, nullptr, d_bs_t.p, d_sc.p);
     OSFM_LAUNCH_CHECK();
   }
   ba_backsub_points<<<grid_for(npf, 256), 256, 0, stream>>>(rs.v, d_scale.p, d_Vinv.p, d_bs_t.p, d_y.p);
   OSFM_LAUNCH_CHECK();
-  rs.tm_back.stop(stream);
-}
-
-void BA::capture_linear_system(int it, double radius, int pcg_path) {
+  lm_phase(LM_PH_BACK, -1);
+}
+
+void BA::capture_linear_system(int it, double radius) {
   const int nc = rs.nc, n = rs.n, P = rs.P;
+  const int pcg_path = rs.pcg_pipe_ok ? read_lm().pcg_path : rs.pcg_resident ? OSFM_PCG_CLASSIC_RESIDENT : OSFM_PCG_CLASSIC_STREAMED;
+  OSFM_CUDA(cudaMemcpyAsync(h_pcg.p, d_pcg.p, PCG_STATE_HEADER, cudaMemcpyDeviceToHost, stream));
   download(cap_sbuf, d_Sbuf.p, (size_t)rs.nc_pad + (size_t)rs.s_total, stream);
   download(cap_upper, d_upper.p, rs.n_upper, stream);
   download(cap_y, d_px.p, nc, stream);
   download(cap_scale, d_scale.p, n, stream); download(cap_diag, d_diag.p, n, stream); download(cap_grad, d_grad.p, n, stream);
   download(cap_pt_poff, d_pt_poff.p, P, stream); download(cap_global_of, d_global_of.p, P, stream);
-  const Params xp = params_of(rs.cur);
+  const Params xp = params_of(0);
   download(cap_cam, xp.cam, cam_params.size(), stream); download(cap_inst, xp.inst, inst.size(), stream);
   download(cap_rc, xp.rc, rc.size(), stream); download(cap_pts, xp.pts, 3 * (size_t)P, stream);
   download(cap_ext, xp.ext, ext_values.size(), stream);
@@ -1836,8 +2017,7 @@
     cudaEvent_t ce[4];
     for (auto& e : ce) OSFM_CUDA(cudaEventCreate(&e));
     OSFM_CUDA(cudaEventRecord(ce[0], stream));
-    double gm = 0.0;
-    linearize(rs.cur, false, &gm);
+    linearize(0, false);
     if (n > 0) {
       ba_make_scale<<<grid_for(n, 256), 256, 0, stream>>>(d_colnorm2.p, d_scale.p, n);
       OSFM_LAUNCH_CHECK();
@@ -1845,7 +2025,7 @@
       OSFM_LAUNCH_CHECK();
     }
     segment_table_scales();
-    build_system(0.0, flags + COV_F_POINT_RANK, false);
+    build_system(d_diag.p, 0.0, flags + COV_F_POINT_RANK, false);
     OSFM_CUDA(cudaEventRecord(ce[1], stream));
     auto tiles = [](int k) { return (k + COV_NB - 1) / COV_NB; };
     CovGemm g{A, nc, X, m, n1, nullptr, 0, 0, flags};
@@ -1913,7 +2093,7 @@
 }
 
 void BA::write_results(osfm_ba_summary sum) {
-  const int cur = rs.cur, P = rs.P, Pfull = rs.Pfull;
+  const int cur = 0, P = rs.P, Pfull = rs.Pfull;
   const long long Nfull = rs.Nfull;
   download(cam_params, d_cam[cur].p, cam_params.size(), stream); download(inst, d_inst[cur].p, inst.size(), stream);
   download(rc, d_rc[cur].p, rc.size(), stream); download(ext_values, d_ext[cur].p, ext_values.size(), stream);
@@ -1944,24 +2124,126 @@
   float dev_ms = 0.f;
   OSFM_CUDA(cudaEventElapsedTime(&dev_ms, rs.ev0, rs.ev1));
   cudaEventDestroy(rs.ev0); cudaEventDestroy(rs.ev1);
-  rs.tm_lin.collect(); rs.tm_schur.collect(); rs.tm_pcg.collect(); rs.tm_back.collect();
+  const LmState& lm = read_lm();
   sum.time_device_ms = dev_ms;
-  sum.time_linearize_ms = rs.tm_lin.total_ms;
-  sum.linearize_launches = rs.tm_lin.count;
-  sum.time_schur_ms = rs.tm_schur.total_ms;
-  sum.schur_launches = rs.tm_schur.count;
-  sum.time_pcg_ms = rs.tm_pcg.total_ms;
-  sum.time_backsub_ms = rs.tm_back.total_ms;
+  sum.time_linearize_ms = lm.phase_ns[LM_PH_LIN] * 1e-6;
+  sum.linearize_launches = lm.phase_count[LM_PH_LIN];
+  sum.time_schur_ms = lm.phase_ns[LM_PH_SCHUR] * 1e-6;
+  sum.schur_launches = lm.phase_count[LM_PH_SCHUR];
+  sum.time_pcg_ms = lm.phase_ns[LM_PH_PCG] * 1e-6;
+  sum.time_backsub_ms = lm.phase_ns[LM_PH_BACK] * 1e-6;
   sum.num_observations_local = rs.N;
   sum.reduced_dim = rs.nc;
   sum.reduced_blocks = rs.n_blocks_all;
   sum.reduced_nnz = rs.s_total;
   sum.jac_planes = rs.nres * (rs.wc + 3 + 1);
-  rs.tm_lin.destroy(); rs.tm_schur.destroy(); rs.tm_pcg.destroy(); rs.tm_back.destroy();
   sum.kernel_launches = g_kernel_launches.load() - rs.launches0;
+  if (rs.device_loop)
+    sum.kernel_launches += (int64_t)(lm.it - 1) * rs.k_body + (int64_t)(lm.n_classic - 1) * rs.k_pcg +
+                           (int64_t)(lm.n_eval - 1) * rs.k_eval + (int64_t)(lm.n_success - 1) * rs.k_accept;
+  sum.device_loop = rs.device_loop ? 1 : 0;
   sum.time_run_s = std::chrono::duration<double>(std::chrono::high_resolution_clock::now() - rs.t_start).count();
   summary = sum;
   has_run = true;
+}
+
+void BA::lm_iteration() {
+  const int n = rs.n, nc = rs.nc;
+  const int graph = rs.cap_graph != nullptr;
+  ba_make_diag<<<grid_for(n, 256), 256, 0, stream>>>(d_colnorm2.p, d_scale.p, d_diag.p, n, d_lm.p, d_diag_r.p);
+  OSFM_LAUNCH_CHECK();
+  build_system(d_diag_r.p, 1.0, nullptr, true);
+  OSFM_CUDA(cudaMemsetAsync(d_y.p, 0, sizeof(double) * rs.nz, stream));
+  if (nc > 0) {
+    solve_reduced();
+    if (cap_iter > 0 && read_lm().it == cap_iter) capture_linear_system(cap_iter, h_lm.p->radius);
+  }
+  back_substitute();
+  OSFM_CUDA(cudaMemsetAsync(&d_sc.p->model_change, 0, sizeof(double) * 3, stream));
+  if (n > 0) {
+    ba_model_change_alg<<<grid_for(n, 256), 256, 0, stream>>>(n, nc, rank == 0, d_grad.p, d_scale.p, d_diag_r.p, 1.0, d_y.p, d_sc.p);
+    OSFM_LAUNCH_CHECK();
+  }
+  update_params(0, 1, 1.0, d_ext_lower.p);
+  if (world > 1) allreduce_dev(&d_sc.p->model_change, 3);
+  ba_lm_check<<<1, 1, 0, stream>>>(d_lm.p, d_sc.p, d_pcg.p, nc, rs.h_eval, graph);
+  OSFM_LAUNCH_CHECK();
+  rs.k_eval = lm_if(rs.h_eval, LM_EVAL, [&]() {
+    eval_cost(1);
+    if (rs.constrained) line_search();
+  });
+  ba_lm_step<<<1, 1, 0, stream>>>(d_lm.p, d_sc.p, rs.h_accept, graph);
+  OSFM_LAUNCH_CHECK();
+  rs.k_accept = lm_if(rs.h_accept, LM_ACCEPT, [&]() { accept_candidate(); });
+}
+
+void BA::line_search() {
+  const int n = rs.n, nc = rs.nc;
+  const double cost = read_lm().cost;
+  double cand_cost = read_scalars().cost;
+  auto step_to = [&](double alpha) {
+    OSFM_CUDA(cudaMemsetAsync(&d_sc.p->step_norm2, 0, sizeof(double) * 2, stream));
+    update_params(0, 1, alpha, d_ext_lower.p);
+    if (world > 1) allreduce_dev(&d_sc.p->step_norm2, 2);
+    eval_cost(1);
+  };
+  OSFM_CUDA(cudaMemsetAsync(&d_sc.p->gdot, 0, sizeof(double), stream));
+  ba_grad_dot<<<grid_for(n, 256), 256, 0, stream>>>(n, nc, rank == 0, d_grad.p, d_scale.p, d_y.p, d_sc.p);
+  OSFM_LAUNCH_CHECK();
+  if (world > 1) allreduce_dev(&d_sc.p->gdot, 1);
+  const double g0 = read_scalars().gdot;
+  double alpha = 1.0;
+  for (int ls = 0; ls < 20; ++ls) {
+    if (ls > 0) { step_to(alpha); cand_cost = read_scalars().cost; }
+    if (std::isfinite(cand_cost) && cand_cost <= cost + 1e-4 * g0 * alpha) return;
+    alpha *= 0.5;
+  }
+  step_to(1.0);
+}
+
+void BA::accept_candidate() {
+  const Params a = params_of(0), c = params_of(1);
+  auto copy = [&](double* dst, const double* src, size_t count) {
+    if (count) OSFM_CUDA(cudaMemcpyAsync(dst, src, sizeof(double) * count, cudaMemcpyDeviceToDevice, stream));
+  };
+  copy(a.cam, c.cam, cam_params.size());
+  copy(a.inst, c.inst, inst.size());
+  copy(a.rc, c.rc, rc.size());
+  copy(a.pts, c.pts, 3 * (size_t)rs.P);
+  copy(a.ext, c.ext, ext_values.size());
+  linearize(0, true);
+  ba_lm_accepted<<<1, 1, 0, stream>>>(d_lm.p, d_sc.p);
+  OSFM_LAUNCH_CHECK();
+}
+
+void BA::run_lm_graph() {
+  cudaGraph_t g = nullptr;
+  OSFM_CUDA(cudaGraphCreate(&g, 0));
+  cudaGraphConditionalHandle h_while;
+  OSFM_CUDA(cudaGraphConditionalHandleCreate(&h_while, g, 0, 0));
+  rs.cap_deps.clear();
+  capture_begin(g);
+  ba_lm_next<<<1, 1, 0, stream>>>(d_lm.p, max_iterations, h_while, 1);
+  OSFM_LAUNCH_CHECK();
+  capture_end();
+  cudaGraph_t body = add_conditional(g, h_while, cudaGraphCondTypeWhile);
+  OSFM_CUDA(cudaGraphConditionalHandleCreate(&rs.h_pcg, body, 0, 0));
+  OSFM_CUDA(cudaGraphConditionalHandleCreate(&rs.h_eval, body, 0, 0));
+  OSFM_CUDA(cudaGraphConditionalHandleCreate(&rs.h_accept, body, 0, 0));
+  rs.cap_deps.clear();
+  const int64_t k0 = g_kernel_launches.load();
+  capture_begin(body);
+  lm_iteration();
+  ba_lm_next<<<1, 1, 0, stream>>>(d_lm.p, max_iterations, h_while, 1);
+  OSFM_LAUNCH_CHECK();
+  capture_end();
+  rs.cap_graph = nullptr;
+  rs.k_body = g_kernel_launches.load() - k0 - rs.k_pcg - rs.k_eval - rs.k_accept;
+  cudaGraphExec_t exec = nullptr;
+  OSFM_CUDA(cudaGraphInstantiate(&exec, g, 0));
+  OSFM_CUDA(cudaGraphLaunch(exec, stream));
+  OSFM_CUDA(cudaGraphExecDestroy(exec));
+  OSFM_CUDA(cudaGraphDestroy(g));
 }
 
 void BA::run() {
@@ -1985,7 +2267,6 @@
   upload_problem();
   OSFM_CUDA(cudaEventCreate(&rs.ev0)); OSFM_CUDA(cudaEventCreate(&rs.ev1));
   trace("upload");
-  rs.tm_lin.init(); rs.tm_schur.init(); rs.tm_pcg.init(); rs.tm_back.init();
   trace("pre-struct");
   discover_structure();
   plan_pcg();
@@ -1993,26 +2274,17 @@
   if (cov_on) reserve_covariance();
 
   const int n = rs.n, nc = rs.nc;
-  int& cur = rs.cur;
+  rs.device_loop = world == 1 && !rs.constrained && cap_iter == 0 && !switches().trace && !switches().host_loop &&
+                   rs.pcg_pipe_ok && stream != cudaStreamLegacy;
   if (world > 1) {
     OSFM_CUDA(cudaMemsetAsync(d_sc.p, 0, sizeof(Scalars), stream));
     allreduce_dev(&d_sc.p->cost, 1);
     OSFM_CUDA(cudaStreamSynchronize(stream));
   }
+  OSFM_CUDA(cudaMemsetAsync(d_lm.p, 0, sizeof(LmState), stream));
   OSFM_CUDA(cudaEventRecord(rs.ev0, stream));
-  double radius = 1e4;
-  const double max_radius = 1e16, min_radius = 1e-32, min_rel_decrease = 1e-3;
-  const double ftol = 1e-6, gtol = 1e-10, ptol = 1e-8;
-  double decrease_factor = 2.0;
-  bool reuse_diagonal = false;
-  int n_invalid = 0, it = 0, n_success = 0, n_solves = 0;
-  int termination = 1;
-  std::string message = "Maximum number of iterations reached.";
-
   build_segment_tables();
-  double grad_max = 0.0;
-  double cost = linearize(cur, true, &grad_max);
-  const double initial_cost = cost;
+  linearize(0, true);
   if (n > 0) {
     ba_make_scale<<<grid_for(n, 256), 256, 0, stream>>>(d_colnorm2.p, d_scale.p, n);
     OSFM_LAUNCH_CHECK();
@@ -2021,113 +2293,40 @@
   if (switches().pcg_deflate && rs.pcg_pipe_ok && rs.NI > 0 && nc > 0) {
     d_Wdef.reserve((size_t)PCG_ND * nc);
     OSFM_CUDA(cudaMemsetAsync(d_Wdef.p, 0, sizeof(double) * PCG_ND * (size_t)nc, stream));
-    pcg_gauge_vectors<<<grid_for(rs.NI, 128), 128, 0, stream>>>(rs.NI, d_inst_poff.p, params_of(cur).inst, d_scale.p, nc, d_Wdef.p);
+    pcg_gauge_vectors<<<grid_for(rs.NI, 128), 128, 0, stream>>>(rs.NI, d_inst_poff.p, params_of(0).inst, d_scale.p, nc, d_Wdef.p);
     OSFM_LAUNCH_CHECK();
     rs.pcg_pipe.Wdef = d_Wdef.p;
   }
-  double x_norm = n > 0 ? x_norm_of(cur) : 0.0;
-
-  if (grad_max <= gtol || n == 0) {
-    termination = 0;
-    message = n == 0 ? "No free parameters." : "Gradient tolerance reached.";
-  }
-  while (termination == 1) {
-    if (it >= max_iterations) break;
-    if (radius < min_radius) { termination = 0; message = "Minimum trust region radius reached."; break; }
-    ++it;
-    if (!reuse_diagonal) {
-      ba_make_diag<<<grid_for(n, 256), 256, 0, stream>>>(d_colnorm2.p, d_scale.p, d_diag.p, n);
+  if (n > 0) x_norm_pass(0);
+  ba_lm_init<<<1, 1, 0, stream>>>(d_lm.p, d_sc.p, n);
+  OSFM_LAUNCH_CHECK();
+  if (rs.device_loop) {
+    run_lm_graph();
+  } else {
+    for (;;) {
+      ba_lm_next<<<1, 1, 0, stream>>>(d_lm.p, max_iterations, 0, 0);
       OSFM_LAUNCH_CHECK();
-    }
-    const double inv_radius = 1.0 / radius;
-    build_system(inv_radius, nullptr, true);
-    OSFM_CUDA(cudaMemsetAsync(d_y.p, 0, sizeof(double) * rs.nz, stream));
-    int pcg_path = 0;
-    if (nc > 0) {
-      pcg_path = solve_reduced();
-      if (it == cap_iter) capture_linear_system(it, radius, pcg_path);
-    }
-    ++n_solves;
-    back_substitute();
-    OSFM_CUDA(cudaMemsetAsync(&d_sc.p->model_change, 0, sizeof(double) * 3, stream));
-    if (n > 0) {
-      ba_model_change_alg<<<grid_for(n, 256), 256, 0, stream>>>(n, nc, rank == 0, d_grad.p, d_scale.p, d_diag.p, inv_radius, d_y.p, d_sc.p);
-      OSFM_LAUNCH_CHECK();
-    }
-    const int cand = cur ^ 1;
-    update_params(cur, cand, 1.0, d_ext_lower.p);
-    if (world > 1) allreduce_dev(&d_sc.p->model_change, 3);
-    const Scalars sm = read_scalars();
-    bool ok = true;
-    if (nc > 0) {
-      const PcgState& h = *h_pcg.p;
-      const int pcg_it = h.iterations, its = std::max(pcg_it, 1);
-      rs.pcg_total += pcg_it;
-      if (switches().trace && (pcg_path == OSFM_PCG_CLASSIC_RESIDENT || pcg_path == OSFM_PCG_CLASSIC_STREAMED))
-        fprintf(stderr, "[osfm_ba] pcg %d its, CTA0 clocks/it: stage %lld matvec %lld reduce1 %lld phaseB %lld reduce2 %lld (resident %d)\n",
-                pcg_it, h.prof[0] / its, h.prof[1] / its, h.prof[2] / its, h.prof[3] / its, h.prof[4] / its, (int)rs.pcg_resident);
-      if (!(h.rr_final == h.rr_final)) ok = false;
-    }
-    const double model_change = sm.model_change;
-    double step_norm = std::sqrt(sm.step_norm2);
-    if (!ok || !(model_change > 0.0) || !std::isfinite(step_norm)) {
-      if (++n_invalid >= 5) { termination = 2; message = "Too many consecutive invalid steps."; break; }
-      radius *= 0.5;
-      reuse_diagonal = true;
-      continue;
-    }
-    n_invalid = 0;
-    double cand_cost = eval_cost(cand);
-    if (rs.constrained) {
-      auto step_to = [&](double alpha) {
-        OSFM_CUDA(cudaMemsetAsync(&d_sc.p->step_norm2, 0, sizeof(double) * 2, stream));
-        update_params(cur, cand, alpha, d_ext_lower.p);
-        if (world > 1) allreduce_dev(&d_sc.p->step_norm2, 2);
-        return std::sqrt(read_scalars().step_norm2);
-      };
-      OSFM_CUDA(cudaMemsetAsync(&d_sc.p->gdot, 0, sizeof(double), stream));
-      ba_grad_dot<<<grid_for(n, 256), 256, 0, stream>>>(n, nc, rank == 0, d_grad.p, d_scale.p, d_y.p, d_sc.p);
-      OSFM_LAUNCH_CHECK();
-      if (world > 1) allreduce_dev(&d_sc.p->gdot, 1);
-      const double g0 = read_scalars().gdot;
-      double alpha = 1.0;
-      bool ok_ls = false;
-      for (int ls = 0; ls < 20; ++ls) {
-        if (ls > 0) { step_norm = step_to(alpha); cand_cost = eval_cost(cand); }
-        if (std::isfinite(cand_cost) && cand_cost <= cost + 1e-4 * g0 * alpha) { ok_ls = true; break; }
-        alpha *= 0.5;
-      }
-      if (!ok_ls) { step_norm = step_to(1.0); cand_cost = eval_cost(cand); }
-    }
-    if (step_norm <= ptol * (x_norm + ptol)) { termination = 0; message = "Parameter tolerance reached."; break; }
-    const double cost_change = cost - cand_cost;
-    if (std::fabs(cost_change) <= ftol * cost) { termination = 0; message = "Function tolerance reached."; break; }
-    const double rel = cost_change / model_change;
-    if (rel > min_rel_decrease) {
-      cur = cand;
-      cost = linearize(cur, true, &grad_max);
-      x_norm = x_norm_of(cur);
-      radius = std::min(max_radius, radius / std::max(1.0 / 3.0, 1.0 - std::pow(2.0 * rel - 1.0, 3)));
-      decrease_factor = 2.0;
-      reuse_diagonal = false;
-      ++n_success;
-      if (grad_max <= gtol) { termination = 0; message = "Gradient tolerance reached."; break; }
-    } else {
-      radius /= decrease_factor;
-      decrease_factor *= 2.0;
-      reuse_diagonal = true;
+      if (!read_lm().running) break;
+      lm_iteration();
     }
   }
   OSFM_CUDA(cudaEventRecord(rs.ev1, stream));
+  static const char* const messages[] = {"Maximum number of iterations reached.", "No free parameters.",
+                                         "Gradient tolerance reached.", "Minimum trust region radius reached.",
+                                         "Too many consecutive invalid steps.", "Parameter tolerance reached.",
+                                         "Function tolerance reached."};
+  const LmState lm = read_lm();
+  const int termination = lm.termination;
   osfm_ba_summary sum{};
-  sum.iterations = it;
-  sum.successful_steps = n_success;
-  sum.linear_solves = n_solves;
-  sum.pcg_iterations = rs.pcg_total;
+  sum.iterations = lm.it;
+  sum.successful_steps = lm.n_success;
+  sum.linear_solves = lm.n_solves;
+  sum.pcg_iterations = lm.pcg_total;
   sum.termination = termination;
-  sum.initial_cost = initial_cost;
-  sum.final_cost = eval_cost(cur);
-  snprintf(sum.message, sizeof(sum.message), "%s", message.c_str());
+  sum.initial_cost = lm.initial_cost;
+  eval_cost(0);
+  sum.final_cost = read_scalars().cost;
+  snprintf(sum.message, sizeof(sum.message), "%s", messages[lm.message]);
   trace("lm");
 
   if (cov_on) covariance_pass(termination);
diff --git a/opensfm_b200/csrc/ba_reduced.cuh b/opensfm_b200/csrc/ba_reduced.cuh
--- a/opensfm_b200/csrc/ba_reduced.cuh
+++ b/opensfm_b200/csrc/ba_reduced.cuh
@@ -1097,56 +1097,69 @@
   }
 }
 
-__global__ void pcg_factor_groups(const double* __restrict__ Sval, BsrView h, const int* __restrict__ diag_off,
-                                  const int* __restrict__ grp_b1, const int* __restrict__ grp_b2, int ngroups,
-                                  double* __restrict__ Minv) {
-  const int g = blockIdx.x * blockDim.x + threadIdx.x;
+constexpr int PFG_WARPS = 4;
+__global__ void __launch_bounds__(32 * PFG_WARPS)
+    pcg_factor_groups(const double* __restrict__ Sval, BsrView h, const int* __restrict__ diag_off,
+                      const int* __restrict__ grp_b1, const int* __restrict__ grp_b2, int ngroups,
+                      double* __restrict__ Minv) {
+  __shared__ double Ls[PFG_WARPS][MAXB * MAXB];
+  const int w = threadIdx.x >> 5, lane = threadIdx.x & 31;
+  const int g = blockIdx.x * PFG_WARPS + w;
   if (g >= ngroups) return;
+  double* L = Ls[w];
   const int b1 = grp_b1[g], b2 = grp_b2[g];
   const int n1 = h.blk_sz[b1], n2 = b2 >= 0 ? h.blk_sz[b2] : 0;
   const int n = n1 + n2;
-  double L[MAXB * MAXB];
   const double* D1 = Sval + diag_off[b1];
-  for (int i = 0; i < n1; ++i)
-    for (int j = 0; j <= i; ++j) L[i * MAXB + j] = D1[i * n1 + j];
+  for (int t = lane; t < n1 * n1; t += 32) {
+    const int i = t / n1, j = t - i * n1;
+    if (j <= i) L[i * MAXB + j] = D1[t];
+  }
   if (b2 >= 0) {
     const double* D2 = Sval + diag_off[b2];
-    for (int i = 0; i < n2; ++i)
-      for (int j = 0; j <= i; ++j) L[(n1 + i) * MAXB + n1 + j] = D2[i * n2 + j];
+    for (int t = lane; t < n2 * n2; t += 32) {
+      const int i = t / n2, j = t - i * n2;
+      if (j <= i) L[(n1 + i) * MAXB + n1 + j] = D2[t];
+    }
     const int o12 = bsr_lookup(h, min(b1, b2), max(b1, b2));
-    for (int i = 0; i < n2; ++i)
-      for (int j = 0; j < n1; ++j) {
-        double v = 0.0;
-        if (o12 >= 0) v = b1 < b2 ? Sval[o12 + j * n2 + i] : Sval[o12 + i * n1 + j];
-        L[(n1 + i) * MAXB + j] = v;
-      }
-  }
+    for (int t = lane; t < n2 * n1; t += 32) {
+      const int i = t / n1, j = t - i * n1;
+      double v = 0.0;
+      if (o12 >= 0) v = b1 < b2 ? Sval[o12 + j * n2 + i] : Sval[o12 + i * n1 + j];
+      L[(n1 + i) * MAXB + j] = v;
+    }
+  }
+  __syncwarp();
   for (int j = 0; j < n; ++j) {
-    double d = L[j * MAXB + j];
-    for (int k = 0; k < j; ++k) d -= L[j * MAXB + k] * L[j * MAXB + k];
-    d = sqrt(fmax(d, 1e-300));
-    L[j * MAXB + j] = d;
-    for (int i = j + 1; i < n; ++i) {
+    if (lane == 0) {
+      double d = L[j * MAXB + j];
+      for (int k = 0; k < j; ++k) d -= L[j * MAXB + k] * L[j * MAXB + k];
+      L[j * MAXB + j] = sqrt(fmax(d, 1e-300));
+    }
+    __syncwarp();
+    const int i = j + 1 + lane;
+    if (i < n) {
       double s = L[i * MAXB + j];
       for (int k = 0; k < j; ++k) s -= L[i * MAXB + k] * L[j * MAXB + k];
-      L[i * MAXB + j] = s / d;
-    }
-  }
+      L[i * MAXB + j] = s / L[j * MAXB + j];
+    }
+    __syncwarp();
+  }
+  if (lane >= n) return;
+  const int c = lane;
   double* out = Minv + (size_t)g * MAXB * MAXB;
-  for (int c = 0; c < n; ++c) {
-    double y[MAXB];
-    for (int i = 0; i < n; ++i) {
-      double s = (i == c) ? 1.0 : 0.0;
-      for (int k = 0; k < i; ++k) s -= L[i * MAXB + k] * y[k];
-      y[i] = s / L[i * MAXB + i];
-    }
-    for (int i = n - 1; i >= 0; --i) {
-      double s = y[i];
-      for (int k = i + 1; k < n; ++k) s -= L[k * MAXB + i] * y[k];
-      y[i] = s / L[i * MAXB + i];
-    }
-    for (int i = 0; i < n; ++i) out[i * MAXB + c] = y[i];
-  }
+  double y[MAXB];
+  for (int i = 0; i < n; ++i) {
+    double s = (i == c) ? 1.0 : 0.0;
+    for (int k = 0; k < i; ++k) s -= L[i * MAXB + k] * y[k];
+    y[i] = s / L[i * MAXB + i];
+  }
+  for (int i = n - 1; i >= 0; --i) {
+    double s = y[i];
+    for (int k = i + 1; k < n; ++k) s -= L[k * MAXB + i] * y[k];
+    y[i] = s / L[i * MAXB + i];
+  }
+  for (int i = 0; i < n; ++i) out[i * MAXB + c] = y[i];
 }
 
 constexpr int PCG_MAX_CTAS = 256;
```

After: 716.1 million (median of 6 runs). 1.05x the previous value.
